# vadimkantorov/deepspeech.pytorch

Hardware: AMD Instinct MI355X
Metric: audio-seconds/sec training, DS2 5x BiGRU-800 bs32, at 1/2/4/8 MI355X (higher is better)
Workload: dtype f32

## Files before the change

### deepspeech.pytorch_amd/csrc/gru.hip

```cpp
#include "rnn_common.h"

#include <algorithm>

namespace ds2 {

constexpr int KC_FWD = 1024;
constexpr int KC_BWD = 2400;
constexpr int kTraceS0 = 100, kTraceSteps = 16;

template <int KSW>
__global__ __launch_bounds__(GT) void gru_fwd_step_kernel(
    int s, int T, int N, int H, int D, int UB, int BT, const float* __restrict__ xproj,
    const float* __restrict__ wp, const float* __restrict__ b_f, const float* __restrict__ b_r,
    const int* __restrict__ lens, float* __restrict__ h_all, float* __restrict__ gates) {
  constexpr int PITCH = KC_FWD + 2;
  __shared__ __attribute__((aligned(16))) float hs[GB * PITCH];
  int ub, d, bt;
  if (!map_work(UB * D, BT, UB, ub, d, bt)) return;
  const int n0 = bt * GB;
  const int lane = threadIdx.x & 63;
  const int wave = __builtin_amdgcn_readfirstlane(threadIdx.x >> 6);
  const int t = d == 0 ? s : T - 1 - s;
  const int tp = d == 0 ? t - 1 : t + 1;
  const int KS = (H + 3) / 4;
  const int per = (KS + GW - 1) / GW;
  const int a_ks = wave * per;
  const int b_ks = min(KS, a_ks + per);

  f32x4 acc[3];
#pragma unroll
  for (int g = 0; g < 3; ++g) acc[g] = f32x4{0.f, 0.f, 0.f, 0.f};

  if (s > 0) {
    float w[3][KSW];
    const float* wpd = wp + ((int64_t)d * UB + ub) * KS * 3 * 64 + lane;
#pragma unroll
    for (int i = 0; i < KSW; ++i) {
      const int ks = a_ks + i;
#pragma unroll
      for (int g = 0; g < 3; ++g) w[g][i] = ks < b_ks ? wpd[((int64_t)ks * 3 + g) * 64] : 0.f;
    }
    const float* hprev = h_all + ((int64_t)tp * N * D + d) * H;
    stage_rows(hprev, (int64_t)D * H, N, n0, 0, H, hs, PITCH);
    __syncthreads();
    const float* hrow = hs + (lane & 15) * PITCH + (lane >> 4);
#pragma unroll
    for (int i = 0; i < KSW; ++i) {
      const int ks = a_ks + i;
      if (ks < b_ks) {
        const int k = 4 * ks;
        const float a = (k + (lane >> 4) < H) ? hrow[k] : 0.f;
        acc[0] = __builtin_amdgcn_mfma_f32_16x16x4f32(a, w[0][i], acc[0], 0, 0, 0);
        acc[1] = __builtin_amdgcn_mfma_f32_16x16x4f32(a, w[1][i], acc[1], 0, 0, 0);
        acc[2] = __builtin_amdgcn_mfma_f32_16x16x4f32(a, w[2][i], acc[2], 0, 0, 0);
      }
    }
    __syncthreads();
  }
  float* red = hs;
  constexpr int RP = 3 * GU + 1;
#pragma unroll
  for (int g = 0; g < 3; ++g)
#pragma unroll
    for (int r = 0; r < 4; ++r)
      red[(wave * GB + (lane >> 4) * 4 + r) * RP + g * GU + (lane & 15)] = acc[g][r];
  __syncthreads();
  if (threadIdx.x >= GB * GU) return;

  const int m = threadIdx.x >> 4;
  const int u = threadIdx.x & 15;
  const int n = n0 + m;
  const int j = ub * GU + u;
  if (n >= N || j >= H) return;
  float gh[3];
#pragma unroll
  for (int g = 0; g < 3; ++g) {
    float v = 0.f;
#pragma unroll
    for (int w8 = 0; w8 < GW; ++w8) v += red[(w8 * GB + m) * RP + g * GU + u];
    gh[g] = v;
  }
  const float* bh = d == 0 ? b_f : b_r;
  const float ghr = gh[0] + bh[j];
  const float ghz = gh[1] + bh[H + j];
  float ghn = gh[2] + bh[2 * H + j];
  const int64_t row = ((int64_t)t * N + n) * D + d;
  const bool active = t < lens[n];
  float hout = 0.f, r = 0.f, z = 0.f, nn = 0.f;
  if (active) {
    const float* xp = xproj + row * 3 * H;
    const float hp = s > 0 ? h_all[(((int64_t)tp * N + n) * D + d) * H + j] : 0.f;
    r = sigmoidf_(ghr + xp[j]);
    z = sigmoidf_(ghz + xp[H + j]);
    nn = tanhf(xp[2 * H + j] + r * ghn);
    hout = (hp - nn) * z + nn;
  } else {
    ghn = 0.f;
  }
  h_all[row * H + j] = hout;
  if (gates != nullptr) {
    float* gp = gates + row * 4 * H;
    gp[j] = r;
    gp[H + j] = z;
    gp[2 * H + j] = nn;
    gp[3 * H + j] = ghn;
  }
}

template <int KSW>
__global__ __launch_bounds__(GT) void gru_bwd_step_kernel(
    int s, int T, int N, int H, int D, int UB, int BT, const float* __restrict__ dy, int dyd,
    const float* __restrict__ wpt, const float* __restrict__ h_all,
    const float* __restrict__ gates, const int* __restrict__ lens, float* __restrict__ dgx,
    float* __restrict__ dgh, float* __restrict__ dhs) {
  constexpr int PITCH = KC_BWD + 2;
  __shared__ __attribute__((aligned(16))) float hs[GB * PITCH];
  int ub, d, bt;
  if (!map_work(UB * D, BT, UB, ub, d, bt)) return;
  const int n0 = bt * GB;
  const int lane = threadIdx.x & 63;
  const int wave = __builtin_amdgcn_readfirstlane(threadIdx.x >> 6);
  const int t = d == 0 ? T - 1 - s : s;
  const int tq = d == 0 ? t + 1 : t - 1;
  const int H3 = 3 * H;
  const int KS = (H3 + 3) / 4;

  f32x4 acc0 = f32x4{0.f, 0.f, 0.f, 0.f};
  f32x4 acc1 = f32x4{0.f, 0.f, 0.f, 0.f};
  if (s > 0) {
    const float* dghq = dgh + ((int64_t)tq * N * D + d) * H3;
    const float* wpd = wpt + ((int64_t)d * UB + ub) * KS * 64 + lane;
    for (int kc0 = 0; kc0 < H3; kc0 += KC_BWD) {
      const int kc1 = min(H3, kc0 + KC_BWD);
      const int ks0 = kc0 / 4;
      const int ks1 = (kc1 + 3) / 4;
      const int per = (ks1 - ks0 + GW - 1) / GW;
      const int a_ks = ks0 + wave * per;
      const int b_ks = min(ks1, a_ks + per);
      float w[KSW];
#pragma unroll
      for (int i = 0; i < KSW; ++i) {
        const int ks = a_ks + i;
        w[i] = ks < b_ks ? wpd[(int64_t)ks * 64] : 0.f;
      }
      if (kc0 > 0) __syncthreads();
      stage_rows(dghq, (int64_t)D * H3, N, n0, kc0, kc1, hs, PITCH);
      __syncthreads();
      const float* hrow = hs + (lane & 15) * PITCH + (lane >> 4) - kc0;
#pragma unroll
      for (int i = 0; i < KSW; i += 2) {
        const int ks = a_ks + i;
        if (ks < b_ks) {
          const int k = 4 * ks;
          const float a0 = (k + (lane >> 4) < kc1) ? hrow[k] : 0.f;
          acc0 = __builtin_amdgcn_mfma_f32_16x16x4f32(a0, w[i], acc0, 0, 0, 0);
        }
        if (i + 1 < KSW && ks + 1 < b_ks) {
          const int k = 4 * (ks + 1);
          const float a1 = (k + (lane >> 4) < kc1) ? hrow[k] : 0.f;
          acc1 = __builtin_amdgcn_mfma_f32_16x16x4f32(a1, w[i + 1], acc1, 0, 0, 0);
        }
      }
    }
    __syncthreads();
  }
  float* red = hs;
  constexpr int RP = GU + 1;
#pragma unroll
  for (int r = 0; r < 4; ++r)
    red[(wave * GB + (lane >> 4) * 4 + r) * RP + (lane & 15)] = acc0[r] + acc1[r];
  __syncthreads();
  if (threadIdx.x >= GB * GU) return;

  const int m = threadIdx.x >> 4;
  const int u = threadIdx.x & 15;
  const int n = n0 + m;
  const int j = ub * GU + u;
  if (n >= N || j >= H) return;
  const int len = lens[n];
  const int64_t row = ((int64_t)t * N + n) * D + d;
  float* dhcur = dhs + ((int64_t)(s & 1) * N * D + (int64_t)n * D + d) * H;
  const float* dhprv = dhs + ((int64_t)((s + 1) & 1) * N * D + (int64_t)n * D + d) * H;
  float dh = 0.f;
  if (t < len) {
    float carry = 0.f;
    if (s > 0) {
      float rec = 0.f;
#pragma unroll
      for (int w8 = 0; w8 < GW; ++w8) rec += red[(w8 * GB + m) * RP + u];
      const float zq = gates[(((int64_t)tq * N + n) * D + d) * 4 * H + H + j];
      carry = dhprv[j] * zq + rec;
    }
    dh = dy[(((int64_t)t * N + n) * dyd + (dyd > 1 ? d : 0)) * H + j] + carry;
  }
  float dar = 0.f, daz = 0.f, dan = 0.f, dghn = 0.f;
  if (t < len) {
    const float* gp = gates + row * 4 * H;
    const float r = gp[j], z = gp[H + j], nn = gp[2 * H + j], ghn = gp[3 * H + j];
    float hp = 0.f;
    const int tp = d == 0 ? t - 1 : t + 1;
    if (tp >= 0 && tp < T) hp = h_all[(((int64_t)tp * N + n) * D + d) * H + j];
    dan = dh * (1.f - z) * (1.f - nn * nn);
    daz = dh * (hp - nn) * z * (1.f - z);
    dar = dan * ghn * r * (1.f - r);
    dghn = dan * r;
  }
  float* gx = dgx + row * H3;
  float* gh = dgh + row * H3;
  gx[j] = dar;
  gx[H + j] = daz;
  gx[2 * H + j] = dan;
  gh[j] = dar;
  gh[H + j] = daz;
  gh[2 * H + j] = dghn;
  dhcur[j] = dh;
}

template <int KSW>
__global__ __launch_bounds__(GT) void gru_fwd_persist_kernel(
    int T, int N, int H, int D, int UB, int BT, const float* __restrict__ xproj,
    const float* __restrict__ wp, const float* __restrict__ b_f, const float* __restrict__ b_r,
    const int* __restrict__ lens, float* __restrict__ h_all, float* __restrict__ gates,
    unsigned* __restrict__ counters, unsigned* __restrict__ err,
    unsigned long long* __restrict__ stamps, int trace) {
  constexpr int PITCH = KC_FWD + 4;
  __shared__ __attribute__((aligned(16))) float hs[GB * PITCH];
  __shared__ int flag;
  int ub, d, bt;
  if (!map_work(UB * D, BT, UB, ub, d, bt)) return;
  const int n0 = bt * GB;
  const int lane = threadIdx.x & 63;
  const int wave = __builtin_amdgcn_readfirstlane(threadIdx.x >> 6);
  const int KS = (H + 3) / 4;
  const int a_ks = wave * KSW;
  const int b_ks = min(KS, a_ks + KSW);
  unsigned* gflags = counters + (D * BT + 1) + (d * BT + bt) * UB;
  const __amdgpu_buffer_rsrc_t h_rs = __builtin_amdgcn_make_buffer_rsrc(
      h_all, (short)0, T * N * D * H * 4, 0x00020000);
  const bool stamping = stamps != nullptr && !trace && blockIdx.x == 0 && threadIdx.x == 0;
  const bool tracing = stamps != nullptr && trace && threadIdx.x == 0;
  auto trace_at = [&](int s, int p) {
    if (tracing && s >= kTraceS0 && s < kTraceS0 + kTraceSteps)
      stamps[((int64_t)(s - kTraceS0) * gridDim.x + blockIdx.x) * 5 + p] =
          __builtin_amdgcn_s_memrealtime();
  };
  unsigned long long acc_t[6] = {0, 0, 0, 0, 0, 0};
  unsigned long long t0 = 0, t1 = 0;

  float w[3][KSW];
  {
    const float* wpd = wp + ((int64_t)d * UB + ub) * KS * 3 * 64 + lane;
#pragma unroll
    for (int i = 0; i < KSW; ++i) {
      const int ks = a_ks + i;
#pragma unroll
      for (int g = 0; g < 3; ++g) w[g][i] = ks < b_ks ? wpd[((int64_t)ks * 3 + g) * 64] : 0.f;
    }
  }
  const float* bh = d == 0 ? b_f : b_r;
  const int m = threadIdx.x >> 4;
  const int u = threadIdx.x & 15;
  const int n = n0 + m;
  const int j = ub * GU + u;
  const bool owner = threadIdx.x < GB * GU && n < N && j < H;
  float bias_r = 0.f, bias_z = 0.f, bias_n = 0.f;
  int len = 0;
  if (owner) {
    bias_r = bh[j];
    bias_z = bh[H + j];
    bias_n = bh[2 * H + j];
    len = lens[n];
  }
  settle(bias_r);
  settle(bias_z);
  settle(bias_n);
  settle(len);
  constexpr int RP = 3 * GU + 1;
  __shared__ float red[GW * GB * RP];
  float g_r = 0.f, g_z = 0.f, g_n = 0.f, g_hn = 0.f;
  int64_t g_row = -1;
  for (int s = 0; s < T; ++s) {
    const int t = d == 0 ? s : T - 1 - s;
    const int tp = d == 0 ? t - 1 : t + 1;
    const int64_t row = ((int64_t)t * N + n) * D + d;
    float xr = 0.f, xz = 0.f, xn = 0.f;
    if (owner && t < len) {
      const float* xp = xproj + row * 3 * H;
      xr = xp[j];
      xz = xp[H + j];
      xn = xp[2 * H + j];
    }
    f32x4 acc[3];
#pragma unroll
    for (int g = 0; g < 3; ++g) acc[g] = f32x4{0.f, 0.f, 0.f, 0.f};
    float hp = 0.f;
    if (stamping) t0 = stamp_now();
    trace_at(s, 0);
    if (s > 0) {
      if (!flags_wait(gflags, UB, (unsigned)s, err, &flag)) {
        poison_rest(h_all, s, T, d != 0, N, D, n, d, H, j, H, 1, owner);
        return;
      }
      trace_at(s, 1);
      if (stamping) { t1 = stamp_now(); acc_t[0] += t1 - t0; t0 = t1; }
      const float* hprev = h_all + ((int64_t)tp * N * D + d) * H;
// ... 377 lines not shown
      const float* hrow = hs + (lane & 15) * PITCH + (lane >> 4) + 4 * a_ks;
#pragma unroll
      for (int i = 0; i < KSW; i += 2) {
        acc0 = __builtin_amdgcn_mfma_f32_16x16x4f32(hrow[4 * i], w[i], acc0, 0, 0, 0);
        if (i + 1 < KSW)
          acc1 = __builtin_amdgcn_mfma_f32_16x16x4f32(hrow[4 * i + 4], w[i + 1], acc1, 0, 0, 0);
      }
      __syncthreads();
    }
#pragma unroll
    for (int r = 0; r < 4; ++r)
      red[(wave * GB + (lane >> 4) * 4 + r) * RP + (lane & 15)] = acc0[r] + acc1[r];
    __syncthreads();
    trace_at(s, 3);
    if (owner) {
      float dh = 0.f;
      float dar = 0.f, daz = 0.f, dan = 0.f, dghn = 0.f, zc = 0.f;
      if (t < len) {
        float carry = 0.f;
        if (s > 0) {
          float rec = 0.f;
#pragma unroll
          for (int w8 = 0; w8 < GW; ++w8) rec += red[(w8 * GB + m) * RP + u];
          carry = dh_prev * z_prev + rec;
        }
        dh = dyv + carry;
        zc = g_z;
        dan = dh * (1.f - zc) * (1.f - g_n * g_n);
        daz = dh * (hp - g_n) * zc * (1.f - zc);
        dar = dan * g_hn * g_r * (1.f - g_r);
        dghn = dan * g_r;
      }
      const int go = static_cast<int>((row * H3 + j) * 4);
      __builtin_amdgcn_raw_buffer_store_b32(__builtin_bit_cast(unsigned, dar), g_rs, go, 0, kSc1);
      __builtin_amdgcn_raw_buffer_store_b32(__builtin_bit_cast(unsigned, daz), g_rs, go + 4 * H, 0,
                                            kSc1);
      __builtin_amdgcn_raw_buffer_store_b32(__builtin_bit_cast(unsigned, dghn), g_rs, go + 8 * H,
                                            0, kSc1);
      dh_prev = dh;
      z_prev = zc;
      px_dar = dar; px_daz = daz; px_dan = dan; px_row = row;
    }
    flags_arrive(gflags + ub, (unsigned)s + 1);
    trace_at(s, 4);
    if (owner) {
      float* gx = dgx + px_row * H3;
      gx[j] = px_dar;
      gx[H + j] = px_daz;
      gx[2 * H + j] = px_dan;
    }
  }
}

template <int NBW>
__global__ __launch_bounds__(GT) __attribute__((amdgpu_waves_per_eu(2, 2))) void gru_bwd_dop_kernel(
    int T, int N, int H, int D, int UB, int BT, const float* __restrict__ dy, int dyd,
    const float* __restrict__ w_f, const float* __restrict__ w_r,
    const float* __restrict__ h_all, const float* __restrict__ gates,
    const int* __restrict__ lens, float* __restrict__ dgx, float* __restrict__ dgh,
    float* __restrict__ gx, unsigned* __restrict__ counters, unsigned* __restrict__ err,
    unsigned long long* __restrict__ stamps, double* __restrict__ dbp) {
  constexpr int RP = GU + 1;
  __shared__ __attribute__((aligned(8))) float red[GW * GB * RP];
  __shared__ __attribute__((aligned(16))) float tile[3 * GB * GU];
  __shared__ int flag;
  int ub, d, bt;
  if (!map_work(UB * D, BT, UB, ub, d, bt)) return;
  const int n0 = bt * GB;
  const int lane = threadIdx.x & 63;
  const int wave = __builtin_amdgcn_readfirstlane(threadIdx.x >> 6);
  const int H3 = 3 * H;
  const int NB3 = 3 * UB;
  int b0, nb;
  simd_split(NB3, wave, b0, nb);
  const unsigned* gflags = counters + (D * BT + 1) + (d * BT + bt) * UB;
  unsigned* myflag = counters + (D * BT + 1) + (d * BT + bt) * UB + ub;
  const int slot_floats = D * BT * NB3 * 256;
  const __amdgpu_buffer_rsrc_t x_rs =
      __builtin_amdgcn_make_buffer_rsrc(gx, (short)0, 2 * slot_floats * 4, 0x00020000);
  const int grp_off = (d * BT + bt) * NB3 * 256;
  const bool tracing = stamps != nullptr && threadIdx.x == 0;
  auto trace_at = [&](int s, int p) {
    if (tracing && s >= kTraceS0 && s < kTraceS0 + kTraceSteps)
      stamps[((int64_t)(s - kTraceS0) * gridDim.x + blockIdx.x) * 5 + p] =
          __builtin_amdgcn_s_memrealtime();
  };

  f32x4 w[NBW];
  {
    const float* W = d == 0 ? w_f : w_r;
    const float* wc = W + (int64_t)(16 * b0 + 4 * (lane >> 4)) * H + ub * GU + (lane & 15);
#pragma unroll
    for (int i = 0; i < NBW; ++i)
#pragma unroll
      for (int c = 0; c < 4; ++c) w[i][c] = i < nb ? wc[(int64_t)(16 * i + c) * H] : 0.f;
#pragma unroll
    for (int i = 0; i < NBW; ++i) settle(w[i]);
  }
  const int m = threadIdx.x >> 4;
  const int u = threadIdx.x & 15;
  const int n = n0 + m;
  const int j = ub * GU + u;
  const bool owner = threadIdx.x < GB * GU && n < N;
  int len = owner ? lens[n] : 0;
  settle(len);
  const int tpos = ((u >> 2) * GB + m) * 4 + (u & 3);
  float dh_prev = 0.f, z_prev = 0.f;
  float px_dar = 0.f, px_daz = 0.f, px_dan = 0.f, px_dghn = 0.f;
  int64_t px_row = -1;
  double sb_r = 0.0, sb_z = 0.0, sb_n = 0.0, sb_hn = 0.0;
  for (int s = 0; s < T; ++s) {
    const int t = d == 0 ? T - 1 - s : s;
    f32x4 acc0 = f32x4{0.f, 0.f, 0.f, 0.f};
    f32x4 acc1 = f32x4{0.f, 0.f, 0.f, 0.f};
    trace_at(s, 0);
    float dyv = 0.f, g_r = 0.f, g_z = 0.f, g_n = 0.f, g_hn = 0.f, hp = 0.f;
    const int64_t row = ((int64_t)t * N + n) * D + d;
    if (owner && t < len) {
      dyv = dy[(((int64_t)t * N + n) * dyd + (dyd > 1 ? d : 0)) * H + j];
      const float* gp = gates + row * 4 * H;
      g_r = gp[j];
      g_z = gp[H + j];
      g_n = gp[2 * H + j];
      g_hn = gp[3 * H + j];
      const int tp = d == 0 ? t - 1 : t + 1;
      if (tp >= 0 && tp < T) hp = h_all[(((int64_t)tp * N + n) * D + d) * H + j];
    }
    if (s > 0) {
      if (!flags_wait(gflags, UB, (unsigned)s, err, &flag)) {
        poison_rest(dgx, s, T, d == 0, N, D, n, d, H, j, H3, 3, owner);
        return;
      }
      trace_at(s, 1);
      const int base = (((s - 1) & 1) * slot_floats + grp_off + b0 * 256 + lane * 4) * 4;
      f32x4 gv[NBW];
#pragma unroll
      for (int i = 0; i < NBW; ++i) {
        const int off = i < nb ? base + i * 1024 : 0x7ffffff0;
        gv[i] = __builtin_bit_cast(f32x4, __builtin_amdgcn_raw_buffer_load_b128(x_rs, off, 0, kSc1));
      }
      asm volatile("" ::: "memory");
      __builtin_amdgcn_sched_barrier(0);
#pragma unroll
      for (int i = 0; i < NBW; ++i) {
        acc0 = __builtin_amdgcn_mfma_f32_16x16x4f32(gv[i][0], w[i][0], acc0, 0, 0, 0);
        acc1 = __builtin_amdgcn_mfma_f32_16x16x4f32(gv[i][1], w[i][1], acc1, 0, 0, 0);
        acc0 = __builtin_amdgcn_mfma_f32_16x16x4f32(gv[i][2], w[i][2], acc0, 0, 0, 0);
        acc1 = __builtin_amdgcn_mfma_f32_16x16x4f32(gv[i][3], w[i][3], acc1, 0, 0, 0);
      }
      trace_at(s, 2);
    }
#pragma unroll
    for (int r = 0; r < 4; ++r)
      red[(wave * GB + (lane >> 4) * 4 + r) * RP + (lane & 15)] = acc0[r] + acc1[r];
    settle(dyv);
    settle(g_r);
    settle(g_z);
    settle(g_n);
    settle(g_hn);
    settle(hp);
    __syncthreads();
    trace_at(s, 3);
    if (threadIdx.x < GB * GU) {
      float dar = 0.f, daz = 0.f, dan = 0.f, dghn = 0.f;
      if (owner) {
        float dh = 0.f, zc = 0.f;
        if (t < len) {
          float carry = 0.f;
          if (s > 0) {
            float rec = 0.f;
#pragma unroll
            for (int w8 = 0; w8 < GW; ++w8) rec += red[(w8 * GB + m) * RP + u];
            carry = dh_prev * z_prev + rec;
          }
          dh = dyv + carry;
          zc = g_z;
          dan = dh * (1.f - zc) * (1.f - g_n * g_n);
          daz = dh * (hp - g_n) * zc * (1.f - zc);
          dar = dan * g_hn * g_r * (1.f - g_r);
          dghn = dan * g_r;
        }
        dh_prev = dh;
        z_prev = zc;
        px_dar = dar; px_daz = daz; px_dan = dan; px_dghn = dghn; px_row = row;
        sb_r += dar; sb_z += daz; sb_n += dan; sb_hn += dghn;
      }
      tile[tpos] = dar;
      tile[GB * GU + tpos] = daz;
      tile[2 * GB * GU + tpos] = dghn;
    }
    __syncthreads();
    if (wave == 0) {
      const int toff = (grp_off + ub * 256 + lane * 4) * 4;
      const int so = (s & 1) * slot_floats * 4 + toff;
#pragma unroll
      for (int g = 0; g < 3; ++g) {
        const u32x4 v = *reinterpret_cast<const u32x4*>(tile + g * GB * GU + lane * 4);
        __builtin_amdgcn_raw_buffer_store_b128(v, x_rs, so + g * UB * 1024, 0, kSc1);
      }
      asm volatile("s_waitcnt vmcnt(0)" ::: "memory");
      if (lane == 0)
        __hip_atomic_store(myflag, (unsigned)s + 1, __ATOMIC_RELAXED, __HIP_MEMORY_SCOPE_AGENT);
    }
    trace_at(s, 4);
    if (owner) {
      float* gxr = dgx + px_row * H3;
      gxr[j] = px_dar;
      gxr[H + j] = px_daz;
      gxr[2 * H + j] = px_dan;
      float* ghr = dgh + px_row * H3;
      ghr[j] = px_dar;
      ghr[H + j] = px_daz;
      ghr[2 * H + j] = px_dghn;
    }
  }
  if (dbp == nullptr) return;
  double* rd = reinterpret_cast<double*>(red);
  __syncthreads();
  if (threadIdx.x < GB * GU) {
    const bool mine = owner;
    rd[(0 * GB + m) * GU + u] = mine ? sb_r : 0.0;
    rd[(1 * GB + m) * GU + u] = mine ? sb_z : 0.0;
    rd[(2 * GB + m) * GU + u] = mine ? sb_n : 0.0;
    rd[(3 * GB + m) * GU + u] = mine ? sb_hn : 0.0;
  }
  __syncthreads();
  if (threadIdx.x < 4 * GU) {
    const int g = threadIdx.x / GU, uu = threadIdx.x - (threadIdx.x / GU) * GU;
    double acc = 0.0;
#pragma unroll
    for (int mm = 0; mm < GB; ++mm) acc += rd[(g * GB + mm) * GU + uu];
    dbp[(((int64_t)bt * D + d) * 4 + g) * H + ub * GU + uu] = acc;
  }
}

__global__ void gru_db_cols_kernel(const float* __restrict__ dgx, const float* __restrict__ dgh,
                                   int rows, int D, int H, double* __restrict__ dbp) {
  const int c = blockIdx.x;
  const int d = c / (4 * H), k = c - d * 4 * H;
  const int g = k / H, j = k - g * H;
  const float* src = g < 3 ? dgx + d * 3 * H + g * H + j : dgh + d * 3 * H + 2 * H + j;
  const int64_t stride = (int64_t)D * 3 * H;
  double acc = 0.0;
  for (int r = threadIdx.x; r < rows; r += blockDim.x) acc += src[r * stride];
  __shared__ double sh[256];
  sh[threadIdx.x] = acc;
  __syncthreads();
  for (int w = 128; w > 0; w >>= 1) {
    if ((int)threadIdx.x < w) sh[threadIdx.x] += sh[threadIdx.x + w];
    __syncthreads();
  }
  if (threadIdx.x == 0) dbp[c] = sh[0];
}

__global__ void gru_db_final_kernel(const double* __restrict__ dbp, int BT, int D, int H,
                                    float* __restrict__ dbi_f, float* __restrict__ dbh_f,
                                    float* __restrict__ dbi_r, float* __restrict__ dbh_r) {
  const int total = D * 4 * H;
  for (int i = blockIdx.x * blockDim.x + threadIdx.x; i < total; i += gridDim.x * blockDim.x) {
    const int d = i / (4 * H), k = i - d * 4 * H;
    double acc = 0.0;
    for (int b = 0; b < BT; ++b) acc += dbp[(int64_t)b * total + i];
    const float v = static_cast<float>(acc);
    float* dbi = d == 0 ? dbi_f : dbi_r;
    float* dbh = d == 0 ? dbh_f : dbh_r;
    if (k < 3 * H) dbi[k] = v;
    if (k < 2 * H) dbh[k] = v;
    if (k >= 3 * H) dbh[k - H] = v;
  }
}

}

namespace ds2 {
bool launch_gru_fwd_x6(int t_max, int n, int h, int num_dirs, const float* xproj,
                       const float* w_hh_f, const float* w_hh_r, const float* b_hh_f,
                       const float* b_hh_r, const int* lens, float* h_all, float* gates,
                       float* ring, unsigned* ctrs, unsigned* err, unsigned long long* stamps,
                       size_t lds_pad, hipStream_t st);
bool launch_gru_bwd_x6(int t_max, int n, int h, int num_dirs, const float* dy, int dy_dirs,
                       const float* w_hh_f, const float* w_hh_r, const float* h_all,
                       const float* gates, const int* lens, float* dgates_x, float* dgates_h,
                       float* ring, unsigned* ctrs, unsigned* err, unsigned long long* stamps,
                       double* dbp, size_t lds_pad, hipStream_t st, unsigned* camax,
                       bool* camax_done);
int gru_bwd_x6_grid(int n, int h, int num_dirs);
bool launch_rnn_fwd_h3(int t_max, int n, int h, int num_dirs, const float* xproj,
                       const float* w_hh_f, const float* w_hh_r, const float* b_hh_f,
                       const float* b_hh_r, const int* lens, float* h_all, float* ring,
                       unsigned* ctrs, unsigned* err, unsigned long long* stamps, size_t lds_pad,
                       hipStream_t st);
bool launch_rnn_bwd_h3(int t_max, int n, int h, int num_dirs, const float* dy, int dy_dirs,
                       const float* w_hh_f, const float* w_hh_r, const float* h_all,
                       const int* lens, float* dgates, float* ring, unsigned* ctrs, unsigned* err,
                       unsigned long long* stamps, size_t lds_pad, hipStream_t st,
                       unsigned* camax);
int rnn_h3_grid(int n, int h, int num_dirs);
int gru_xl_groups(int n, int h, int num_dirs);
int gru_xl_active(int n, int h, int num_dirs);
size_t gru_xl_ctr_words();
bool launch_gru_fwd_xl(int t_max, int n, int h, int num_dirs, const float* xproj,
                       const float* w_hh_f, const float* w_hh_r, const float* b_hh_f,
                       const float* b_hh_r, const int* lens, float* h_all, float* gates,
                       float* ring, unsigned* xl, unsigned* err, unsigned long long* stamps,
                       size_t lds_pad, hipStream_t st);
bool launch_gru_bwd_xl(int t_max, int n, int h, int num_dirs, const float* dy, int dy_dirs,
                       const float* w_hh_f, const float* w_hh_r, const float* h_all,
                       const float* gates, const int* lens, float* dgates_x, float* dgates_h,
                       float* ring, unsigned* xl, unsigned* err, unsigned long long* stamps,
                       double* dbp, size_t lds_pad, hipStream_t st, unsigned* camax);
}

using namespace ds2;

extern "C" {

static inline int stamp_mode() {
  const char* e = getenv("DS2_GRU_STAMPS");
  return e == nullptr ? 0 : (e[0] == '1' ? 1 : (e[0] == '2' ? 2 : 0));
}
constexpr unsigned kDopPadLds = 80 * 1024;
static const void* bwd_dop_fn(int need) {
#define DS2_BDOP(K) \
  if (need <= K) return reinterpret_cast<const void*>(gru_bwd_dop_kernel<K>);
  DS2_BDOP(1) DS2_BDOP(2) DS2_BDOP(3) DS2_BDOP(4) DS2_BDOP(6) DS2_BDOP(8) DS2_BDOP(10)
  DS2_BDOP(13) DS2_BDOP(16) DS2_BDOP(19) DS2_BDOP(22) DS2_BDOP(24)
#undef DS2_BDOP
  return nullptr;
}
static inline size_t ctr_words(int n, int num_dirs) {
  const int groups = num_dirs * ((n + GB - 1) / GB);
  const size_t a = (size_t)groups * 128, b = gru_xl_ctr_words();
  return (size_t)groups + 1 + (a > b ? a : b);
}
static inline size_t counter_bytes(int n, int num_dirs) {
  const size_t trace = stamp_mode() == 2 ? (size_t)kTraceSteps * 1024 * 5 : 16;
  return align256(ctr_words(n, num_dirs) * sizeof(unsigned)) + trace * sizeof(unsigned long long);
}
static inline unsigned long long* stamp_slots(unsigned* ctrs, int n, int num_dirs) {
  if (stamp_mode() == 0) return nullptr;
  return reinterpret_cast<unsigned long long*>(reinterpret_cast<char*>(ctrs) +
                                               align256(ctr_words(n, num_dirs) * sizeof(unsigned)));
}

static inline size_t ring_bytes(int n, int h, int num_dirs, int tiles) {
  const size_t UB = (h + GU - 1) / GU, BT = (n + GB - 1) / GB;
  const size_t tile_floats = tiles == 3 ? 384 : 256;
  const size_t slots = tiles == 3 ? 4 : 2 * kRingSlots;
  return align256(slots * (size_t)num_dirs * BT * UB * tiles * tile_floats * sizeof(float));
}
static inline hipError_t ring_reset(float* ring, int n, int h, int num_dirs, hipStream_t st) {
  return hipMemsetAsync(ring, 0xFF, ring_bytes(n, h, num_dirs, 1), st);
}

size_t ds2_gru_cache_floats(int t_max, int n, int h, int num_dirs) {
  if (t_max <= 0 || n <= 0 || h <= 0 || num_dirs <= 0) return 0;
  return (size_t)t_max * n * num_dirs * 4 * h;
}

size_t ds2_gru_fwd_workspace_size(int n, int h, int num_dirs) {
  const int64_t UB = (h + GU - 1) / GU;
  const int64_t KS = (h + 3) / 4;
  return align256((size_t)(num_dirs * UB * KS * 3 * 64) * sizeof(float)) +
         align256(counter_bytes(n, num_dirs)) + ring_bytes(n, h, num_dirs, 1) + 256;
}

#define DS2_FWD_CASE(K)                                                                    \
  case K:                                                                                  \
    hipLaunchKernelGGL(gru_fwd_step_kernel<K>, dim3(grid), dim3(GT), 0, st, s, t_max, n, h, \
                       num_dirs, UB, BT, xproj, wp, b_hh_f, b_hh_r, lens, h_all, gates);    \
    break;

static int pick_ksw(int per) {
  const int opts[] = {8, 16, 32, 48, 64, 80, 96};
  for (int k : opts)
    if (per <= k) return k;
  return -1;
}

ds2_status_t ds2_gru_fwd(int t_max, int n, int h, int num_dirs, const float* xproj,
                         const float* w_hh_f, const float* w_hh_r, const float* b_hh_f,
                         const float* b_hh_r, const int* lens, float* h_all, float* gates,
                         unsigned* err_out, void* ws, size_t ws_bytes, ds2_stream_t stream) {
  if (t_max < 0 || n < 0 || h < 1 || (num_dirs != 1 && num_dirs != 2)) return DS2_INVALID_VALUE;
  if (h > KC_FWD) return DS2_UNSUPPORTED_SHAPE;
  if (t_max == 0 || n == 0) return DS2_OK;
  if (ws == nullptr || ws_bytes < ds2_gru_fwd_workspace_size(n, h, num_dirs))
    return DS2_WORKSPACE_TOO_SMALL;
  if (num_dirs == 1) {
    w_hh_r = w_hh_f;
    b_hh_r = b_hh_f;
  }
  hipStream_t st = as_stream(stream);
  apply_spin_limit_env();
  apply_rnn_tune_env();
  const int UB = (h + GU - 1) / GU;
  const int KS = (h + 3) / 4;
  const int BT = (n + GB - 1) / GB;
  const int ksw = pick_ksw((KS + GW - 1) / GW);
  if (ksw < 0) return DS2_UNSUPPORTED_SHAPE;
  float* wp = static_cast<float*>(ws);
  const int grid = mapped_grid(UB * num_dirs, BT);
  const bool persistent = persistent_enabled() && grid <= num_cus() &&
                          (int64_t)t_max * n * num_dirs * h * 4 < (1ll << 31);
  unsigned* ctrs = reinterpret_cast<unsigned*>(
      static_cast<char*>(ws) + align256((size_t)num_dirs * UB * KS * 3 * 64 * sizeof(float)));
  unsigned* err = ctrs + num_dirs * BT;
  if (persistent && (h % GU) == 0 && UB <= 8 * GW) {
    if (hipMemsetAsync(ctrs, 0, counter_bytes(n, num_dirs), st) != hipSuccess)
      return launch_status("ds2_gru counters");
    int T_ = t_max, N_ = n, H_ = h, D_ = num_dirs, UB_ = UB, BT_ = BT;
    unsigned long long* stamps = stamp_mode() == 2 ? stamp_slots(ctrs, n, num_dirs) : nullptr;
    float* ring = reinterpret_cast<float*>(reinterpret_cast<char*>(ctrs) +
                                           align256(counter_bytes(n, num_dirs)));
    void* args[] = {&T_, &N_, &H_, &D_, &UB_, &BT_, &xproj, &w_hh_f, &w_hh_r, &b_hh_f,
                    &b_hh_r, &lens, &h_all, &gates, &ring, &ctrs, &err, &stamps};
    if (ring_reset(ring, n, h, num_dirs, st) != hipSuccess) return launch_status("ds2_gru ring");
    if (launch_gru_fwd_xl(t_max, n, h, num_dirs, xproj, w_hh_f, w_hh_r, b_hh_f, b_hh_r, lens,
                          h_all, gates, ring, err + 1, err, stamps, kDopPadLds, st)) {
      fold_err(err, err_out, st);
      return launch_status("ds2_gru_fwd");
    }
    (void)hipGetLastError();
    if (launch_gru_fwd_x6(t_max, n, h, num_dirs, xproj, w_hh_f, w_hh_r, b_hh_f, b_hh_r, lens,
                          h_all, gates, ring, ctrs, err, stamps, kDopPadLds, st)) {
      fold_err(err, err_out, st);
      return launch_status("ds2_gru_fwd");
    }
    (void)hipGetLastError();
    const void* fn = nullptr;
#define DS2_FDOP(K) \
  case K: fn = reinterpret_cast<const void*>(gru_fwd_dop_kernel<K>); break;
    switch ((UB + GW - 1) / GW) {
      DS2_FDOP(1) DS2_FDOP(2) DS2_FDOP(3) DS2_FDOP(4) DS2_FDOP(5) DS2_FDOP(6) DS2_FDOP(7)
      DS2_FDOP(8)
      default: break;
    }
#undef DS2_FDOP
    if (fn != nullptr &&
        rnn_launch(fn, dim3(grid), dim3(GT), args, kDopPadLds, st) == hipSuccess) {
      fold_err(err, err_out, st);
      return launch_status("ds2_gru_fwd");
    }
    (void)hipGetLastError();
  }
  hipLaunchKernelGGL(pack_fwd_kernel<3>, dim3(grid_cap((int64_t)num_dirs * UB * KS * 192)),
                     dim3(256), 0, st, w_hh_f, w_hh_r, h, num_dirs, UB, KS, wp);
  if (persistent && (h % 4) == 0) {
    if (hipMemsetAsync(ctrs, 0, counter_bytes(n, num_dirs), st) != hipSuccess)
      return launch_status("ds2_gru counters");
    int T_ = t_max, N_ = n, H_ = h, D_ = num_dirs, UB_ = UB, BT_ = BT;
    unsigned long long* stamps = stamp_slots(ctrs, n, num_dirs);
    int trace_ = stamp_mode() == 2 ? 1 : 0;
    void* args[] = {&T_, &N_, &H_, &D_, &UB_, &BT_, &xproj, &wp, &b_hh_f, &b_hh_r, &lens,
                    &h_all, &gates, &ctrs, &err, &stamps, &trace_};
    const void* fn = nullptr;
    const int kp = persist_ksw((KS + GW - 1) / GW, KC_FWD);
    switch (kp) {
      case 8: fn = reinterpret_cast<const void*>(gru_fwd_persist_kernel<8>); break;
      case 16: fn = reinterpret_cast<const void*>(gru_fwd_persist_kernel<16>); break;
      case 25: fn = reinterpret_cast<const void*>(gru_fwd_persist_kernel<25>); break;
      case 32: fn = reinterpret_cast<const void*>(gru_fwd_persist_kernel<32>); break;
      default: break;
    }
    if (fn != nullptr &&
        rnn_launch(fn, dim3(grid), dim3(GT), args, 0, st) == hipSuccess) {
      fold_err(err, err_out, st);
      return launch_status("ds2_gru_fwd");
    }
    (void)hipGetLastError();
  }
  for (int s = 0; s < t_max; ++s) {
    switch (ksw) {
      DS2_FWD_CASE(8) DS2_FWD_CASE(16) DS2_FWD_CASE(32) DS2_FWD_CASE(48) DS2_FWD_CASE(64)
      DS2_FWD_CASE(80) DS2_FWD_CASE(96)
    }
  }
  return launch_status("ds2_gru_fwd");
}

static size_t gru_bwd_ws_base(int n, int h, int num_dirs) {
  const int64_t UB = (h + GU - 1) / GU;
  const int64_t KS = (3 * h + 3) / 4;
  return align256((size_t)(num_dirs * UB * KS * 64) * sizeof(float)) +
         align256((size_t)2 * n * num_dirs * h * sizeof(float)) +
         align256(counter_bytes(n, num_dirs)) + ring_bytes(n, h, num_dirs, 3) + 512;
}

static size_t gru_db_bytes(int n, int h, int num_dirs) {
  return align256((size_t)((n + 7) / 8) * num_dirs * 4 * h * sizeof(double));
}

size_t ds2_gru_bwd_workspace_size(int n, int h, int num_dirs) {
  return gru_bwd_ws_base(n, h, num_dirs) + gru_db_bytes(n, h, num_dirs);
}

#define DS2_BWD_CASE(K)                                                                     \
  case K:                                                                                   \
    hipLaunchKernelGGL(gru_bwd_step_kernel<K>, dim3(grid), dim3(GT), 0, st, s, t_max, n, h,  \
                       num_dirs, UB, BT, dy, dy_dirs, wpt, h_all, gates, lens, dgates_x,     \
                       dgates_h, dhs);                                                       \
    break;

int ds2_gru_bwd_grid(int n, int h, int num_dirs) {
  if (n < 1 || h < 1 || (num_dirs != 1 && num_dirs != 2)) return 0;
  const int UB = (h + GU - 1) / GU, BT = (n + GB - 1) / GB;
  const int grid = mapped_grid(UB * num_dirs, BT);
  if (!persistent_enabled() || grid > num_cus()) return 0;
  if ((h % GU) == 0 && UB <= 8 * GW) {
    const int g = gru_bwd_x6_grid(n, h, num_dirs);
    const int x = gru_xl_active(n, h, num_dirs);
    const int m = g > x ? g : x;
    return m > grid ? m : grid;
  }
  return (3 * h <= KC_BWD && (h % 4) == 0) ? grid : 0;
}

ds2_status_t ds2_gru_bwd(int t_max, int n, int h, int num_dirs, const float* dy, int dy_dirs,
                         const float* w_hh_f, const float* w_hh_r, const float* h_all,
                         const float* gates, const int* lens, float* dgates_x, float* dgates_h,
                         unsigned* err_out, void* ws, size_t ws_bytes, ds2_stream_t stream) {
  return ds2_gru_bwd_bias(t_max, n, h, num_dirs, dy, dy_dirs, w_hh_f, w_hh_r, h_all, gates, lens,
                          dgates_x, dgates_h, nullptr, nullptr, nullptr, nullptr, err_out, ws,
                          ws_bytes, stream);
}

static ds2_status_t gru_bwd_run(int t_max, int n, int h, int num_dirs, const float* dy, int dy_dirs,
                                const float* w_hh_f, const float* w_hh_r, const float* h_all,
                                const float* gates, const int* lens, float* dgates_x,
                                float* dgates_h, unsigned* err_out, void* ws, hipStream_t st,
                                double* dbp, bool& summed, unsigned* camax, bool& camax_done,
                                int& db_tiles);

static ds2_status_t gru_bwd_bias_impl(int t_max, int n, int h, int num_dirs, const float* dy,
                                      int dy_dirs, const float* w_hh_f, const float* w_hh_r,
                                      const float* h_all, const float* gates, const int* lens,
                                      float* dgates_x, float* dgates_h, float* db_ih_f,
                                      float* db_hh_f, float* db_ih_r, float* db_hh_r,
                                      unsigned* err_out, void* ws, size_t ws_bytes,
                                      unsigned* camax, ds2_stream_t stream);

ds2_status_t ds2_gru_bwd_bias(int t_max, int n, int h, int num_dirs, const float* dy, int dy_dirs,
                              const float* w_hh_f, const float* w_hh_r, const float* h_all,
                              const float* gates, const int* lens, float* dgates_x,
                              float* dgates_h, float* db_ih_f, float* db_hh_f, float* db_ih_r,
                              float* db_hh_r, unsigned* err_out, void* ws, size_t ws_bytes,
                              ds2_stream_t stream) {
  return gru_bwd_bias_impl(t_max, n, h, num_dirs, dy, dy_dirs, w_hh_f, w_hh_r, h_all, gates, lens,
                           dgates_x, dgates_h, db_ih_f, db_hh_f, db_ih_r, db_hh_r, err_out, ws,
                           ws_bytes, nullptr, stream);
}

ds2_status_t ds2_gru_bwd_bias_amax(int t_max, int n, int h, int num_dirs, const float* dy,
                                   int dy_dirs, const float* w_hh_f, const float* w_hh_r,
                                   const float* h_all, const float* gates, const int* lens,
                                   float* dgates_x, float* dgates_h, float* db_ih_f,
                                   float* db_hh_f, float* db_ih_r, float* db_hh_r,
                                   unsigned* col_amax, unsigned* err_out, void* ws,
                                   size_t ws_bytes, ds2_stream_t stream) {
  if (col_amax == nullptr) return DS2_INVALID_VALUE;
  return gru_bwd_bias_impl(t_max, n, h, num_dirs, dy, dy_dirs, w_hh_f, w_hh_r, h_all, gates, lens,
                           dgates_x, dgates_h, db_ih_f, db_hh_f, db_ih_r, db_hh_r, err_out, ws,
                           ws_bytes, col_amax, stream);
}

static ds2_status_t gru_bwd_bias_impl(int t_max, int n, int h, int num_dirs, const float* dy,
                                      int dy_dirs, const float* w_hh_f, const float* w_hh_r,
                                      const float* h_all, const float* gates, const int* lens,
                                      float* dgates_x, float* dgates_h, float* db_ih_f,
                                      float* db_hh_f, float* db_ih_r, float* db_hh_r,
                                      unsigned* err_out, void* ws, size_t ws_bytes,
                                      unsigned* camax, ds2_stream_t stream) {
  if (t_max < 0 || n < 0 || h < 1 || (num_dirs != 1 && num_dirs != 2)) return DS2_INVALID_VALUE;
  if (gates == nullptr) return DS2_INVALID_VALUE;
  if (dy_dirs != 1 && dy_dirs != num_dirs) return DS2_INVALID_VALUE;
  const bool want_db = db_ih_f != nullptr;
  if (want_db && (db_hh_f == nullptr || (num_dirs == 2 && (db_ih_r == nullptr || db_hh_r == nullptr))))
    return DS2_INVALID_VALUE;
  if (ws == nullptr || ws_bytes < ds2_gru_bwd_workspace_size(n, h, num_dirs))
    return DS2_WORKSPACE_TOO_SMALL;
  hipStream_t st = as_stream(stream);
  double* dbp = reinterpret_cast<double*>(static_cast<char*>(ws) + gru_bwd_ws_base(n, h, num_dirs));
  const size_t camax_bytes = (size_t)2 * num_dirs * 3 * h * sizeof(unsigned);
  if (camax != nullptr && hipMemsetAsync(camax, 0, camax_bytes, st) != hipSuccess)
    return launch_status("ds2_gru_bwd_bias_amax");
  if (t_max == 0 || n == 0) {
    if (!want_db) return DS2_OK;
    if (hipMemsetAsync(dbp, 0, gru_db_bytes(n > 0 ? n : 1, h, num_dirs), st) != hipSuccess)
      return launch_status("ds2_gru_bwd_bias");
    hipLaunchKernelGGL(gru_db_final_kernel, dim3(cdiv(num_dirs * 4 * h, 256)), dim3(256), 0, st,
                       dbp, 1, num_dirs, h, db_ih_f, db_hh_f, db_ih_r, db_hh_r);
    return launch_status("ds2_gru_bwd_bias");
  }
  bool summed = false, camax_done = false;
  int db_tiles = (n + GB - 1) / GB;
  const ds2_status_t rc = gru_bwd_run(t_max, n, h, num_dirs, dy, dy_dirs, w_hh_f, w_hh_r, h_all,
                                      gates, lens, dgates_x, dgates_h, err_out, ws, st,
                                      want_db ? dbp : nullptr, summed, camax, camax_done, db_tiles);
  if (rc != DS2_OK) return rc;
  if (camax != nullptr && !camax_done) {
    const ds2_status_t ra = ds2_amax(dgates_x, t_max * n, num_dirs * 3 * h, num_dirs * 3 * h,
                                     nullptr, camax, stream);
    const ds2_status_t rb = ra != DS2_OK ? ra
        : ds2_amax(dgates_h, t_max * n, num_dirs * 3 * h, num_dirs * 3 * h, nullptr,
                   camax + num_dirs * 3 * h, stream);
    if (rb != DS2_OK) return rb;
  }
  if (!want_db) return DS2_OK;
  int bt = db_tiles;
  if (!summed) {
    hipLaunchKernelGGL(gru_db_cols_kernel, dim3(num_dirs * 4 * h), dim3(256), 0, st, dgates_x,
                       dgates_h, t_max * n, num_dirs, h, dbp);
    bt = 1;
  }
  hipLaunchKernelGGL(gru_db_final_kernel, dim3(cdiv(num_dirs * 4 * h, 256)), dim3(256), 0, st, dbp,
                     bt, num_dirs, h, db_ih_f, db_hh_f, db_ih_r, db_hh_r);
  return launch_status("ds2_gru_bwd_bias");
}

static ds2_status_t gru_bwd_run(int t_max, int n, int h, int num_dirs, const float* dy, int dy_dirs,
                                const float* w_hh_f, const float* w_hh_r, const float* h_all,
                                const float* gates, const int* lens, float* dgates_x,
                                float* dgates_h, unsigned* err_out, void* ws, hipStream_t st,
                                double* dbp, bool& summed, unsigned* camax, bool& camax_done,
                                int& db_tiles) {
  if (num_dirs == 1) w_hh_r = w_hh_f;
  apply_spin_limit_env();
  apply_rnn_tune_env();
  const int UB = (h + GU - 1) / GU;
  const int KS = (3 * h + 3) / 4;
  const int BT = (n + GB - 1) / GB;
  const int chunk_ks = (std::min(3 * h, KC_BWD) + 3) / 4;
  const int ksw = pick_ksw((chunk_ks + GW - 1) / GW + 1);
  if (ksw < 0) return DS2_UNSUPPORTED_SHAPE;
  float* wpt = static_cast<float*>(ws);
  size_t off = align256((size_t)num_dirs * UB * KS * 64 * sizeof(float));
  float* dhs = reinterpret_cast<float*>(static_cast<char*>(ws) + off);
  const int grid = mapped_grid(UB * num_dirs, BT);
  const bool persistent = persistent_enabled() && grid <= num_cus() &&
                          (int64_t)t_max * n * num_dirs * 3 * h * 4 < (1ll << 31);
  unsigned* ctrs = reinterpret_cast<unsigned*>(
      reinterpret_cast<char*>(dhs) + align256((size_t)2 * n * num_dirs * h * sizeof(float)));
  unsigned* err = ctrs + num_dirs * BT;
  if (persistent && (h % GU) == 0 && UB <= 8 * GW) {
    if (hipMemsetAsync(ctrs, 0, counter_bytes(n, num_dirs), st) != hipSuccess)
      return launch_status("ds2_gru counters");
    int T_ = t_max, N_ = n, H_ = h, D_ = num_dirs, UB_ = UB, BT_ = BT, DYD_ = dy_dirs;
    unsigned long long* stamps = stamp_mode() == 2 ? stamp_slots(ctrs, n, num_dirs) : nullptr;
    float* ring = reinterpret_cast<float*>(reinterpret_cast<char*>(ctrs) +
                                           align256(counter_bytes(n, num_dirs)));
    void* args[] = {&T_, &N_, &H_, &D_, &UB_, &BT_, &dy, &DYD_, &w_hh_f, &w_hh_r, &h_all,
                    &gates, &lens, &dgates_x, &dgates_h, &ring, &ctrs, &err, &stamps, &dbp};
    if (launch_gru_bwd_xl(t_max, n, h, num_dirs, dy, dy_dirs, w_hh_f, w_hh_r, h_all, gates,
                          lens, dgates_x, dgates_h, ring, err + 1, err, stamps, dbp, kDopPadLds,
                          st, camax)) {
      fold_err(err, err_out, st);
      summed = dbp != nullptr;
      camax_done = camax != nullptr;
      db_tiles = (n + 7) / 8;
      return launch_status("ds2_gru_bwd");
    }
    (void)hipGetLastError();
    if (launch_gru_bwd_x6(t_max, n, h, num_dirs, dy, dy_dirs, w_hh_f, w_hh_r, h_all, gates,
                          lens, dgates_x, dgates_h, ring, ctrs, err, stamps, dbp, kDopPadLds, st,
                          camax, &camax_done)) {
      fold_err(err, err_out, st);
      summed = dbp != nullptr;
      return launch_status("ds2_gru_bwd");
    }
    (void)hipGetLastError();
    const void* fn = bwd_dop_fn((3 * UB + GW - 1) / GW);
    if (fn != nullptr &&
        rnn_launch(fn, dim3(grid), dim3(GT), args, kDopPadLds, st) == hipSuccess) {
      fold_err(err, err_out, st);
      summed = dbp != nullptr;
      return launch_status("ds2_gru_bwd");
    }
    (void)hipGetLastError();
  }
  hipLaunchKernelGGL(pack_bwd_kernel<3>, dim3(grid_cap((int64_t)num_dirs * UB * KS * 64)),
                     dim3(256), 0, st, w_hh_f, w_hh_r, h, num_dirs, UB, KS, wpt);
  if (persistent && 3 * h <= KC_BWD && (h % 4) == 0) {
    if (hipMemsetAsync(ctrs, 0, counter_bytes(n, num_dirs), st) != hipSuccess)
      return launch_status("ds2_gru counters");
    int T_ = t_max, N_ = n, H_ = h, D_ = num_dirs, UB_ = UB, BT_ = BT, DYD_ = dy_dirs;
    unsigned long long* stamps = stamp_mode() == 2 ? stamp_slots(ctrs, n, num_dirs) : nullptr;
    void* args[] = {&T_, &N_, &H_, &D_, &UB_, &BT_, &dy, &DYD_, &wpt, &h_all, &gates, &lens,
                    &dgates_x, &dgates_h, &ctrs, &err, &stamps};
    const void* fn = nullptr;
    const int kp = persist_ksw((KS + GW - 1) / GW, KC_BWD);
    switch (kp) {
      case 8: fn = reinterpret_cast<const void*>(gru_bwd_persist_kernel<8>); break;
      case 16: fn = reinterpret_cast<const void*>(gru_bwd_persist_kernel<16>); break;
      case 25: fn = reinterpret_cast<const void*>(gru_bwd_persist_kernel<25>); break;
      case 32: fn = reinterpret_cast<const void*>(gru_bwd_persist_kernel<32>); break;
      case 48: fn = reinterpret_cast<const void*>(gru_bwd_persist_kernel<48>); break;
      case 64: fn = reinterpret_cast<const void*>(gru_bwd_persist_kernel<64>); break;
      case 75: fn = reinterpret_cast<const void*>(gru_bwd_persist_kernel<75>); break;
      default: break;
    }
    if (fn != nullptr &&
        rnn_launch(fn, dim3(grid), dim3(GT), args, 0, st) == hipSuccess) {
      fold_err(err, err_out, st);
      return launch_status("ds2_gru_bwd");
    }
    (void)hipGetLastError();
  }
  for (int s = 0; s < t_max; ++s) {
    switch (ksw) {
      DS2_BWD_CASE(8) DS2_BWD_CASE(16) DS2_BWD_CASE(32) DS2_BWD_CASE(48) DS2_BWD_CASE(64)
      DS2_BWD_CASE(80) DS2_BWD_CASE(96)
    }
  }
  return launch_status("ds2_gru_bwd");
}

static bool rnn_persistent_ok(int t_max, int n, int h, int num_dirs) {
  const int g = rnn_h3_grid(n, h, num_dirs);
  return persistent_enabled() && g > 0 && g <= num_cus() &&
         (int64_t)t_max * n * num_dirs * h * 4 < (1ll << 31);
}

size_t ds2_rnn_fwd_workspace_size(int n, int h, int num_dirs) {
  if (n < 1 || h < 1 || num_dirs < 1) return 256;
  return align256(counter_bytes(n, num_dirs)) + ring_bytes(n, h, num_dirs, 1) + 256;
}

ds2_status_t ds2_rnn_fwd_ws(int t_max, int n, int h, int num_dirs, const float* xproj,
                            const float* w_hh_f, const float* w_hh_r, const float* b_hh_f,
                            const float* b_hh_r, const int* lens, float* h_all, unsigned* err_out,
                            void* ws, size_t ws_bytes, ds2_stream_t stream) {
  if (t_max < 0 || n < 0 || h < 1 || (num_dirs != 1 && num_dirs != 2)) return DS2_INVALID_VALUE;
  if (t_max == 0 || n == 0) return DS2_OK;
  if (xproj == nullptr || w_hh_f == nullptr || b_hh_f == nullptr || lens == nullptr ||
      h_all == nullptr || (num_dirs == 2 && (w_hh_r == nullptr || b_hh_r == nullptr)))
    return DS2_INVALID_VALUE;
  if (ws == nullptr || ws_bytes < ds2_rnn_fwd_workspace_size(n, h, num_dirs))
    return DS2_WORKSPACE_TOO_SMALL;
  if (num_dirs == 1) {
    w_hh_r = w_hh_f;
    b_hh_r = b_hh_f;
  }
  hipStream_t st = as_stream(stream);
  if (rnn_persistent_ok(t_max, n, h, num_dirs)) {
    unsigned* ctrs = static_cast<unsigned*>(ws);
    unsigned* err = ctrs + num_dirs * ((n + GB - 1) / GB);
    float* ring = reinterpret_cast<float*>(static_cast<char*>(ws) + align256(counter_bytes(n, num_dirs)));
    if (hipMemsetAsync(ctrs, 0, counter_bytes(n, num_dirs), st) != hipSuccess)
      return launch_status("ds2_rnn counters");
    if (ring_reset(ring, n, h, num_dirs, st) != hipSuccess) return launch_status("ds2_rnn ring");
    unsigned long long* stamps = stamp_mode() == 2 ? stamp_slots(ctrs, n, num_dirs) : nullptr;
    if (launch_rnn_fwd_h3(t_max, n, h, num_dirs, xproj, w_hh_f, w_hh_r, b_hh_f, b_hh_r, lens,
                          h_all, ring, ctrs, err, stamps, kDopPadLds, st)) {
      fold_err(err, err_out, st);
      return launch_status("ds2_rnn_fwd");
    }
    (void)hipGetLastError();
  }
  return ds2_rnn_fwd(t_max, n, h, num_dirs, xproj, w_hh_f, w_hh_r, b_hh_f, b_hh_r, lens, h_all,
                     stream);
}

size_t ds2_rnn_bwd_workspace_size(int n, int h, int num_dirs) {
  if (n < 1 || h < 1 || num_dirs < 1) return 256;
  return align256(counter_bytes(n, num_dirs)) + ring_bytes(n, h, num_dirs, 3) + 256;
}

int ds2_rnn_bwd_grid(int n, int h, int num_dirs) {
  if (n < 1 || h < 1 || (num_dirs != 1 && num_dirs != 2)) return 0;
  const int g = rnn_h3_grid(n, h, num_dirs);
  return persistent_enabled() && g > 0 && g <= num_cus() ? g : 0;
}

ds2_status_t ds2_rnn_bwd_ws(int t_max, int n, int h, int num_dirs, const float* dy, int dy_dirs,
                            const float* w_hh_f, const float* w_hh_r, const float* h_all,
                            const int* lens, float* dgates, unsigned* col_amax, unsigned* err_out,
                            void* ws, size_t ws_bytes, ds2_stream_t stream) {
  if (t_max < 0 || n < 0 || h < 1 || (num_dirs != 1 && num_dirs != 2)) return DS2_INVALID_VALUE;
  if (dy_dirs != 1 && dy_dirs != num_dirs) return DS2_INVALID_VALUE;
  if (ws == nullptr || ws_bytes < ds2_rnn_bwd_workspace_size(n, h, num_dirs))
    return DS2_WORKSPACE_TOO_SMALL;
  hipStream_t st = as_stream(stream);
  if (col_amax != nullptr &&
      hipMemsetAsync(col_amax, 0, (size_t)num_dirs * h * sizeof(unsigned), st) != hipSuccess)
    return launch_status("ds2_rnn_bwd_ws");
  if (t_max == 0 || n == 0) return DS2_OK;
  if (dy == nullptr || w_hh_f == nullptr || h_all == nullptr || lens == nullptr ||
      dgates == nullptr || (num_dirs == 2 && w_hh_r == nullptr))
    return DS2_INVALID_VALUE;
  if (num_dirs == 1) w_hh_r = w_hh_f;
  if (rnn_persistent_ok(t_max, n, h, num_dirs)) {
    unsigned* ctrs = static_cast<unsigned*>(ws);
    unsigned* err = ctrs + num_dirs * ((n + GB - 1) / GB);
    float* ring = reinterpret_cast<float*>(static_cast<char*>(ws) + align256(counter_bytes(n, num_dirs)));
    if (hipMemsetAsync(ctrs, 0, counter_bytes(n, num_dirs), st) != hipSuccess)
      return launch_status("ds2_rnn counters");
    unsigned long long* stamps = stamp_mode() == 2 ? stamp_slots(ctrs, n, num_dirs) : nullptr;
    if (launch_rnn_bwd_h3(t_max, n, h, num_dirs, dy, dy_dirs, w_hh_f, w_hh_r, h_all, lens, dgates,
                          ring, ctrs, err, stamps, kDopPadLds, st, col_amax)) {
      fold_err(err, err_out, st);
      return launch_status("ds2_rnn_bwd");
    }
    (void)hipGetLastError();
  }
  const ds2_status_t rc = ds2_rnn_bwd(t_max, n, h, num_dirs, dy, dy_dirs, w_hh_f, w_hh_r, h_all,
                                      lens, dgates, stream);
  if (rc != DS2_OK || col_amax == nullptr) return rc;
  return ds2_amax(dgates, t_max * n, num_dirs * h, num_dirs * h, nullptr, col_amax, stream);
}

}
```

### deepspeech.pytorch_amd/csrc/gru_xl.hip

```cpp
#include "rnn_common.h"

namespace ds2 {

#ifndef DS2_XL_ABL
#define DS2_XL_ABL 0
#endif
constexpr bool kAblLoads = (DS2_XL_ABL & 1) != 0;
constexpr bool kAblStores = (DS2_XL_ABL & 2) != 0;
constexpr bool kAblWait = (DS2_XL_ABL & 4) != 0;
constexpr bool kAblFixT = (DS2_XL_ABL & 8) != 0;

constexpr int LB = 8;
constexpr int LU = 32;
constexpr int LW = 4;
constexpr int LT = LW * 64;
constexpr int LSLOTS = 4;
constexpr int LRB = 784;
constexpr int kXlTraceS0 = 100, kXlTraceSteps = 16;

__device__ __forceinline__ bool xl_map(int G, int UBX, int& g, int& ub) {
  g = blockIdx.x & 7;
  ub = blockIdx.x >> 3;
  return g < G && ub < UBX;
}

__device__ __forceinline__ bool xl_group_local(unsigned* xtab, int ub, int UBX, unsigned* err,
                                               int* lds_word, unsigned* mode, int force_global) {
  const unsigned mine = xcc_id() + 1u;
  if (threadIdx.x == 0) __hip_atomic_store(xtab + ub, mine, __ATOMIC_RELAXED, __HIP_MEMORY_SCOPE_AGENT);
  if ((threadIdx.x >> 6) == 0) {
    const int lane = threadIdx.x & 63;
    unsigned v = mine;
    bool ok = true;
    for (unsigned spins = 0;; ++spins) {
      v = lane < UBX ? __hip_atomic_load(xtab + lane, __ATOMIC_RELAXED, __HIP_MEMORY_SCOPE_AGENT)
                     : mine;
      if (__ballot(v == 0u) == 0ull) break;
      if (spins > g_spin_limit) {
        if (lane == 0) __hip_atomic_fetch_or(err, 1u, __ATOMIC_RELAXED, __HIP_MEMORY_SCOPE_AGENT);
        ok = false;
        break;
      }
      __builtin_amdgcn_s_sleep(1);
    }
    const bool loc = ok && __ballot(v != mine) == 0ull && force_global == 0;
    if (lane == 0) {
      *lds_word = loc ? 1 : 0;
      __hip_atomic_fetch_or(mode, loc ? 1u : 2u, __ATOMIC_RELAXED, __HIP_MEMORY_SCOPE_AGENT);
    }
  }
  __syncthreads();
  return *lds_word != 0;
}

__device__ __forceinline__ void xl_store(u32x4 v, __amdgpu_buffer_rsrc_t rs, int off, bool local) {
  if (local)
    __builtin_amdgcn_raw_buffer_store_b128(v, rs, off, 0, 0);
  else
    __builtin_amdgcn_raw_buffer_store_b128(v, rs, off, 0, kSc1);
}

__device__ __forceinline__ int xl_frag_hi(int m, int k) { return (((k >> 3) << 4) + m) * 8 + (k & 7); }

template <int NPW>
__global__ __launch_bounds__(LT) __attribute__((amdgpu_waves_per_eu(1, 1))) void gru_fwd_xl_kernel(
    int T, int N, int H, int D, int UBX, int BTX, const float* __restrict__ xproj,
    const float* __restrict__ w_f, const float* __restrict__ w_r, const float* __restrict__ b_f,
    const float* __restrict__ b_r, const int* __restrict__ lens, float* __restrict__ h_all,
    float* __restrict__ gates, float* __restrict__ ring, unsigned* __restrict__ xl,
    unsigned* __restrict__ err, unsigned long long* __restrict__ stamps, int force_global) {
  constexpr int NCT = 6;
  constexpr int RC = 3 * LU + 1;
  __shared__ float red[LW * 16 * RC];
  __shared__ __attribute__((aligned(16))) _Float16 stg[64 * 8];
  __shared__ float unsc[3 * LU];
  __shared__ __attribute__((aligned(16))) float pin[3 * 256];
  __shared__ __attribute__((aligned(16))) float pout[5 * 256];
  __shared__ int slen[LB];
  __shared__ int sh_local;
  __shared__ int failed;
  __shared__ u32x4 wx[LW * NCT * 2 * 64];
  const int G = D * BTX;
  int g, ub;
  if (!xl_map(G, UBX, g, ub)) return;
  const int d = g / BTX, bt = g - d * BTX;
  const int lane = threadIdx.x & 63;
  const int wave = __builtin_amdgcn_readfirstlane(threadIdx.x >> 6);
  const int p0 = wave * (UBX / LW) + min(wave, UBX % LW);
  const int np = UBX / LW + (wave < UBX % LW ? 1 : 0);
  if (threadIdx.x == 0) failed = 0;
  const bool local = xl_group_local(xl + g * 32, ub, UBX, err, &sh_local, xl + 512 + g, force_global);
  const int slot_floats = G * UBX * 256;
  const __amdgpu_buffer_rsrc_t x_rs =
      __builtin_amdgcn_make_buffer_rsrc(ring, (short)0, LSLOTS * slot_floats * 4, 0x00020000);
  const int grp_off = g * UBX * 256;
  const bool tracing = stamps != nullptr && lane == 0;
  auto trace_at = [&](int s, int p) __attribute__((always_inline)) {
    if (tracing && s >= kXlTraceS0 && s < kXlTraceS0 + kXlTraceSteps)
      stamps[(((int64_t)(s - kXlTraceS0) * gridDim.x + blockIdx.x) * LW + wave) * 6 + p] =
          __builtin_amdgcn_s_memrealtime();
  };

  Duo w[NPW][NCT];
  auto wfr = [&](int p, int ct) __attribute__((always_inline)) {
    if (p < NPW) return w[p < NPW ? p : 0][ct];
    Duo r;
    r.hi = __builtin_bit_cast(f16x8, wx[((wave * NCT + ct) * 2 + 0) * 64 + lane]);
    r.lo = __builtin_bit_cast(f16x8, wx[((wave * NCT + ct) * 2 + 1) * 64 + lane]);
    return r;
  };
  {
    const float* W = d == 0 ? w_f : w_r;
    const int q8 = 8 * (lane >> 4);
    auto frag = [&](int p, int ct, f32x4& a, f32x4& b) __attribute__((always_inline)) {
      const f32x4 z4 = f32x4{0.f, 0.f, 0.f, 0.f};
      if (p < np) {
        const float* r = W + (int64_t)((ct >> 1) * H + LU * ub + 16 * (ct & 1) + (lane & 15)) * H +
                         LU * (p0 + p) + q8;
        a = *reinterpret_cast<const f32x4*>(r);
        b = *reinterpret_cast<const f32x4*>(r + 4);
      } else {
        a = z4;
        b = z4;
      }
    };
    float mx[NCT];
#pragma unroll
    for (int ct = 0; ct < NCT; ++ct) mx[ct] = 0.f;
#pragma unroll
    for (int p = 0; p < NPW + 1; ++p)
#pragma unroll
      for (int ct = 0; ct < NCT; ++ct) {
        f32x4 a, b;
        frag(p, ct, a, b);
#pragma unroll
        for (int i = 0; i < 4; ++i) mx[ct] = fmaxf(mx[ct], fmaxf(fabsf(a[i]), fabsf(b[i])));
      }
#pragma unroll
    for (int ct = 0; ct < NCT; ++ct) {
      mx[ct] = fmaxf(mx[ct], __shfl_xor(mx[ct], 16));
      mx[ct] = fmaxf(mx[ct], __shfl_xor(mx[ct], 32));
      if (lane < 16) red[wave * 96 + ct * 16 + lane] = mx[ct];
    }
    __syncthreads();
    float sc[NCT];
#pragma unroll
    for (int ct = 0; ct < NCT; ++ct) {
      float m = 0.f;
#pragma unroll
      for (int w4 = 0; w4 < LW; ++w4) m = fmaxf(m, red[w4 * 96 + ct * 16 + (lane & 15)]);
      sc[ct] = __builtin_ldexpf(1.f, h3_row_exp(m));
    }
    if (threadIdx.x < 3 * LU) {
      float m = 0.f;
#pragma unroll
      for (int w4 = 0; w4 < LW; ++w4) m = fmaxf(m, red[w4 * 96 + threadIdx.x]);
      unsc[threadIdx.x] = __builtin_ldexpf(1.f, -(h3_row_exp(m) + 14));
    }
    __syncthreads();
    asm volatile("" ::: "memory");
#pragma unroll
    for (int p = 0; p < NPW + 1; ++p)
#pragma unroll
      for (int ct = 0; ct < NCT; ++ct) {
        f32x4 a, b;
        frag(p, ct, a, b);
        const Duo dd = split2h(a, b, sc[ct]);
        if (p < NPW) {
          w[p < NPW ? p : 0][ct] = dd;
        } else {
          wx[((wave * NCT + ct) * 2 + 0) * 64 + lane] = __builtin_bit_cast(u32x4, dd.hi);
          wx[((wave * NCT + ct) * 2 + 1) * 64 + lane] = __builtin_bit_cast(u32x4, dd.lo);
        }
      }
  }
  const float* bh = d == 0 ? b_f : b_r;
  const int m = threadIdx.x >> 5;
  const int u = threadIdx.x & 31;
  const int n = bt * LB + m;
  const int j = ub * LU + u;
  const bool owner = n < N;
  float bias_r = 0.f, bias_z = 0.f, bias_n = 0.f;
  if (owner) {
    bias_r = bh[j];
    bias_z = bh[H + j];
    bias_n = bh[2 * H + j];
  }
  if (threadIdx.x < LB) slen[threadIdx.x] = bt * LB + (int)threadIdx.x < N ? lens[bt * LB + threadIdx.x] : 0;
  __syncthreads();
  const int len = slen[m];
  const float us_r = unsc[u], us_z = unsc[LU + u], us_n = unsc[2 * LU + u];
  settle(bias_r);
  settle(bias_z);
  settle(bias_n);
  const int shi = xl_frag_hi(m, u), slo = shi + 64;
  const bool io = wave != 0;
  const int q = io ? (int)threadIdx.x - 64 : 0;
  const int qm = q / 24, qg = (q % 24) >> 3, q4 = (q & 7) * 4;
  const int qn = bt * LB + qm;
  const bool qv = io && qn < N;
  const int qlen = slen[qm];
  const float* xq = xproj + ((int64_t)qn * D + d) * 3 * H + qg * H + ub * LU + q4;
  const int64_t xstep = (int64_t)N * D * 3 * H;
  const f32x4 z4v = f32x4{0.f, 0.f, 0.f, 0.f};
  auto in_ok = [&](int st) __attribute__((always_inline)) {
    const int tt = d == 0 ? st : T - 1 - st;
    return !kAblLoads && qv && tt < qlen;
  };
  auto load_in = [&](int st) __attribute__((always_inline)) {
    const int tt = d == 0 ? st : T - 1 - st;
    return *reinterpret_cast<const f32x4*>(in_ok(st) ? xq + (kAblFixT ? 0 : tt) * xstep : xproj);
  };
  float* ob[2];
  int64_t ostr[2];
  int osrc[2];
  bool ov[2];
#pragma unroll
  for (int k = 0; k < 2; ++k) {
    const int idx = q + 192 * k;
    const int sm = (idx / 40) & 7, f = (idx % 40) >> 3, o4 = (idx & 7) * 4, sn = bt * LB + sm;
    ov[k] = io && idx < 320 && sn < N && (f == 0 || gates != nullptr);
    osrc[k] = f * 256 + sm * LU + o4;
    if (f == 0) {
      ob[k] = h_all + ((int64_t)sn * D + d) * H + ub * LU + o4;
      ostr[k] = (int64_t)N * D * H;
    } else {
      ob[k] = gates + ((int64_t)sn * D + d) * 4 * H + (f - 1) * H + ub * LU + o4;
      ostr[k] = (int64_t)N * D * 4 * H;
    }
  }
  auto store_out = [&](int st) __attribute__((always_inline)) {
    const int tt = d == 0 ? st : T - 1 - st;
#pragma unroll
    for (int k = 0; k < 2; ++k)
      if (ov[k])
        *reinterpret_cast<f32x4*>(ob[k] + tt * ostr[k]) = *reinterpret_cast<const f32x4*>(pout + osrc[k]);
  };
  f32x4 xin = io ? load_in(0) : z4v;
  float h_own = 0.f;
  for (int s = 0; s < T; ++s) {
    const int t = d == 0 ? s : T - 1 - s;
    f32x4 acc[NCT];
#pragma unroll
    for (int ct = 0; ct < NCT; ++ct) acc[ct] = f32x4{0.f, 0.f, 0.f, 0.f};
    trace_at(s, 0);
    if (io) *reinterpret_cast<f32x4*>(pin + qg * 256 + qm * LU + q4) = in_ok(s) ? xin : z4v;
    if (s > 0) {
      trace_at(s, 1);
      const int base = (((s - 1) % LSLOTS) * slot_floats + grp_off + p0 * 256 + lane * 4) * 4;
      sleep_units(g_rnn_tune[7]);
      u32x4 hv[NPW + 1];
#pragma unroll
      for (int p = 0; p < NPW + 1; ++p)
        hv[p] = __builtin_amdgcn_raw_buffer_load_b128(x_rs, p < np ? base + p * 1024 : 0x7ffffff0, 0, kSc1);
      asm volatile("" ::: "memory");
      __builtin_amdgcn_sched_barrier(0);
      bool bad = false;
#pragma unroll
      for (int p = 0; p < NPW + 1; ++p) {
        if (p < np && !bad) {
          for (unsigned spins = 0;
               !kAblWait && (!wave_ready(__builtin_bit_cast(f32x4, hv[p])) || g_spin_limit == 0);
               ++spins) {
            if (spins > g_spin_limit || g_spin_limit == 0) {
              if (lane == 0) __hip_atomic_fetch_or(err, 1u, __ATOMIC_RELAXED, __HIP_MEMORY_SCOPE_AGENT);
              failed = 1;
              bad = true;
              break;
            }
            sleep_units(g_rnn_tune[0]);
            asm volatile("" ::: "memory");
#pragma unroll
            for (int q = p; q < NPW + 1; ++q)
              if (q < np && (unsigned)(q - p) < g_rnn_tune[6])
                hv[q] = __builtin_amdgcn_raw_buffer_load_b128(x_rs, base + q * 1024, 0, kSc1);
          }
          const f16x8 a = __builtin_bit_cast(f16x8, hv[p]);
#pragma unroll
          for (int ct = 0; ct < NCT; ++ct) {
            const Duo wf = wfr(p, ct);
            acc[ct] = __builtin_amdgcn_mfma_f32_16x16x32_f16(a, wf.lo, acc[ct], 0, 0, 0);
            acc[ct] = __builtin_amdgcn_mfma_f32_16x16x32_f16(a, wf.hi, acc[ct], 0, 0, 0);
          }
        }
      }
      trace_at(s, 2);
    }
    if (io) {
      if (s + 1 < T) xin = load_in(s + 1);
      if (!kAblStores && s > 0) store_out(s - 1);
    }
    trace_at(s, 3);
#pragma unroll
    for (int ct = 0; ct < NCT; ++ct)
#pragma unroll
      for (int i = 0; i < 4; ++i)
        red[(wave * 16 + (lane >> 4) * 4 + i) * RC + ct * 16 + (lane & 15)] = acc[ct][i];
    __syncthreads();
    if (failed) {
      poison_rest(h_all, s, T, d != 0, N, D, n, d, H, j, H, 1, owner);
      return;
    }
    trace_at(s, 4);
    float gh[3];
#pragma unroll
    for (int gt = 0; gt < 3; ++gt) {
      float v = 0.f;
#pragma unroll
      for (int w4 = 0; w4 < LW; ++w4)
        v += red[(w4 * 16 + m) * RC + gt * LU + u] + red[(w4 * 16 + m + 8) * RC + gt * LU + u];
      gh[gt] = v;
    }
    const float xr = pin[m * LU + u], xz = pin[256 + m * LU + u], xn = pin[512 + m * LU + u];
    float hout = 0.f, r = 0.f, z = 0.f, nn = 0.f, ghn = 0.f;
    if (owner && t < len) {
      ghn = gh[2] * us_n + bias_n;
      r = sigmoid_fast(gh[0] * us_r + bias_r + xr);
      z = sigmoid_fast(gh[1] * us_z + bias_z + xz);
      nn = tanh_fast(xn + r * ghn);
      hout = (h_own - nn) * z + nn;
    }
    h_own = owner ? hout : 0.f;
    pout[m * LU + u] = hout;
    pout[256 + m * LU + u] = r;
    pout[512 + m * LU + u] = z;
    pout[768 + m * LU + u] = nn;
    pout[1024 + m * LU + u] = ghn;
    {
      const float v = hout * 16384.f;
      const _Float16 hi = (_Float16)v;
      stg[shi] = hi;
      stg[slo] = (_Float16)(v - (float)hi);
    }
    __syncthreads();
    if (wave == 0) {
      const int toff = (grp_off + ub * 256 + lane * 4) * 4;
      const u32x4 v = desentinel(*reinterpret_cast<const u32x4*>(stg + lane * 8));
      asm volatile("s_waitcnt vmcnt(0)" ::: "memory");
      xl_store(v, x_rs, (s % LSLOTS) * slot_floats * 4 + toff, local);
      xl_store(u32x4{kSentinel, kSentinel, kSentinel, kSentinel}, x_rs,
               ((s + 2) % LSLOTS) * slot_floats * 4 + toff, local);
    }
    trace_at(s, 5);
  }
  __syncthreads();
  if (io && !kAblStores) store_out(T - 1);
}

template <int NPW>
__global__ __launch_bounds__(LT) __attribute__((amdgpu_waves_per_eu(1, 1))) void gru_bwd_xl_kernel(
    int T, int N, int H, int D, int UBX, int BTX, const float* __restrict__ dy, int dyd,
    const float* __restrict__ w_f, const float* __restrict__ w_r,
    const float* __restrict__ h_all, const float* __restrict__ gates,
    const int* __restrict__ lens, float* __restrict__ dgx, float* __restrict__ dgh,
    float* __restrict__ ring, unsigned* __restrict__ xl, unsigned* __restrict__ err,
    unsigned long long* __restrict__ stamps, double* __restrict__ dbp,
    unsigned* __restrict__ camax, int force_global) {
  constexpr int RC = LU + 1;
  constexpr int LWP = 3;
  __shared__ __attribute__((aligned(8))) float red[LW * 16 * RC > 4 * LB * LU * 2 ? LW * 16 * RC : 4 * LB * LU * 2];
  __shared__ __attribute__((aligned(16))) _Float16 stg[3 * 64 * 8];
  __shared__ __attribute__((aligned(16))) float stsc[LB];
  __shared__ float colmx[LW * LU];
  __shared__ __attribute__((aligned(16))) float pin[6 * 256];
  __shared__ __attribute__((aligned(16))) float pout[4 * 256];
  __shared__ int slen[LB];
  __shared__ int sh_local;
  __shared__ int flag;
  __shared__ u32x4 wx[LW * 6 * 2 * 64];
  const int G = D * BTX;
  int g, ub;
  if (!xl_map(G, UBX, g, ub)) return;
  const int d = g / BTX, bt = g - d * BTX;
  const int lane = threadIdx.x & 63;
  const int wave = __builtin_amdgcn_readfirstlane(threadIdx.x >> 6);
  const int p0 = wave * (UBX / LW) + min(wave, UBX % LW);
  const int np = UBX / LW + (wave < UBX % LW ? 1 : 0);
  const int H3 = 3 * H;
  const int slot_floats = G * UBX * LRB;
  const __amdgpu_buffer_rsrc_t x_rs =
      __builtin_amdgcn_make_buffer_rsrc(ring, (short)0, 2 * slot_floats * 4, 0x00020000);
  const int grp_off = g * UBX * LRB;
  const bool local = xl_group_local(xl + g * 32, ub, UBX, err, &sh_local, xl + 512 + g, force_global);
  unsigned* flags = xl + 256 + g * 32;
  const __amdgpu_buffer_rsrc_t f_rs =
      __builtin_amdgcn_make_buffer_rsrc(xl + 256, (short)0, 8 * 32 * 4, 0x00020000);
  const bool tracing = stamps != nullptr && lane == 0;
  auto trace_at = [&](int s, int p) __attribute__((always_inline)) {
    if (tracing && s >= kXlTraceS0 && s < kXlTraceS0 + kXlTraceSteps)
      stamps[(((int64_t)(s - kXlTraceS0) * gridDim.x + blockIdx.x) * LW + wave) * 6 + p] =
          __builtin_amdgcn_s_memrealtime();
  };

  Duo w[NPW][3][2];
  auto wfr = [&](int p, int gt, int c) __attribute__((always_inline)) {
    if (p < NPW) return w[p < NPW ? p : 0][gt][c];
    Duo r;
    r.hi = __builtin_bit_cast(f16x8, wx[((wave * 6 + gt * 2 + c) * 2 + 0) * 64 + lane]);
    r.lo = __builtin_bit_cast(f16x8, wx[((wave * 6 + gt * 2 + c) * 2 + 1) * 64 + lane]);
    return r;
  };
  float unscale;
  {
    const float* W = d == 0 ? w_f : w_r;
    const int q8 = 8 * (lane >> 4);
    auto col = [&](int p, int gt, int c, f32x4& a, f32x4& b) __attribute__((always_inline)) {
      if (p < np) {
        const float* wc = W + (int64_t)(gt * H + LU * (p0 + p) + q8) * H + LU * ub + 16 * c + (lane & 15);
#pragma unroll
        for (int i = 0; i < 4; ++i) {
          a[i] = wc[(int64_t)i * H];
          b[i] = wc[(int64_t)(i + 4) * H];
        }
      } else {
        a = f32x4{0.f, 0.f, 0.f, 0.f};
        b = a;
      }
    };
    float mx[2] = {0.f, 0.f};
#pragma unroll
    for (int p = 0; p < NPW + 1; ++p)
#pragma unroll
      for (int gt = 0; gt < 3; ++gt)
#pragma unroll
        for (int c = 0; c < 2; ++c) {
          f32x4 a, b;
          col(p, gt, c, a, b);
#pragma unroll
          for (int i = 0; i < 4; ++i) mx[c] = fmaxf(mx[c], fmaxf(fabsf(a[i]), fabsf(b[i])));
        }
#pragma unroll
    for (int c = 0; c < 2; ++c) {
      mx[c] = fmaxf(mx[c], __shfl_xor(mx[c], 16));
      mx[c] = fmaxf(mx[c], __shfl_xor(mx[c], 32));
      if (lane < 16) colmx[wave * LU + 16 * c + lane] = mx[c];
    }
    __syncthreads();
    float sc[2];
#pragma unroll
    for (int c = 0; c < 2; ++c) {
      float m = 0.f;
#pragma unroll
      for (int w4 = 0; w4 < LW; ++w4) m = fmaxf(m, colmx[w4 * LU + 16 * c + (lane & 15)]);
      sc[c] = __builtin_ldexpf(1.f, h3_row_exp(m));
    }
    {
      float m = 0.f;
#pragma unroll
      for (int w4 = 0; w4 < LW; ++w4) m = fmaxf(m, colmx[w4 * LU + (threadIdx.x & 31)]);
      unscale = __builtin_ldexpf(1.f, -h3_row_exp(m));
    }
    asm volatile("" ::: "memory");
#pragma unroll
    for (int p = 0; p < NPW + 1; ++p)
#pragma unroll
      for (int gt = 0; gt < 3; ++gt)
#pragma unroll
        for (int c = 0; c < 2; ++c) {
          f32x4 a, b;
          col(p, gt, c, a, b);
          const Duo dd = split2h(a, b, sc[c]);
          if (p < NPW) {
            w[p < NPW ? p : 0][gt][c] = dd;
          } else {
            wx[((wave * 6 + gt * 2 + c) * 2 + 0) * 64 + lane] = __builtin_bit_cast(u32x4, dd.hi);
            wx[((wave * 6 + gt * 2 + c) * 2 + 1) * 64 + lane] = __builtin_bit_cast(u32x4, dd.lo);
          }
        }
  }
  const int m = threadIdx.x >> 5;
  const int u = threadIdx.x & 31;
  const int n = bt * LB + m;
  const int j = ub * LU + u;
  const bool owner = n < N;
  if (threadIdx.x < LB) slen[threadIdx.x] = bt * LB + (int)threadIdx.x < N ? lens[bt * LB + threadIdx.x] : 0;
  __syncthreads();
  const int len = slen[m];
  const int shi = xl_frag_hi(m, u), slo = shi + 64;
  const bool io = wave != 0;
  const int q = io ? (int)threadIdx.x - 64 : 0;
  const f32x4 z4v = f32x4{0.f, 0.f, 0.f, 0.f};
  const int ostr = N * D * H3;
  struct IoSlot {
    const float* in;
    float* out;
    int f, len, str, pin_at, pout_at;
  };
  auto make_slot = [&](int k) __attribute__((always_inline)) {
    const int idx = q + 192 * k;
    const int sm = idx / 48, f = (idx % 48) >> 3, o4 = (idx & 7) * 4, sn = bt * LB + sm;
    IoSlot r;
    r.f = f;
    r.len = io && sn < N ? slen[sm] : -1;
    if (f == 0) {
      r.in = dy + (sn * dyd + (dyd > 1 ? d : 0)) * H + ub * LU + o4;
      r.str = N * dyd * H;
    } else if (f < 5) {
      r.in = gates + (sn * D + d) * 4 * H + (f - 1) * H + ub * LU + o4;
      r.str = N * D * 4 * H;
    } else {
      r.in = h_all + (sn * D + d) * H + ub * LU + o4;
      r.str = N * D * H;
    }
    r.out = io && sn < N ? (f < 3 ? dgx : dgh) + (sn * D + d) * H3 + (f % 3) * H + ub * LU + o4
                         : nullptr;
    r.pin_at = f * 256 + sm * LU + o4;
    r.pout_at = (f < 3 ? f : (f == 5 ? 3 : f - 3)) * 256 + sm * LU + o4;
    return r;
  };
  const IoSlot sl0 = make_slot(0), sl1 = make_slot(1);
  auto in_ok = [&](int st, const IoSlot sl) __attribute__((always_inline)) {
    const int tt = d == 0 ? T - 1 - st : st;
    const int tr = sl.f == 5 ? (d == 0 ? tt - 1 : tt + 1) : tt;
    return !kAblLoads && tt < sl.len && tr >= 0 && tr < T;
  };
  auto load_in = [&](int st, const IoSlot sl) __attribute__((always_inline)) {
    const int tt = d == 0 ? T - 1 - st : st;
    const int tr = sl.f == 5 ? (d == 0 ? tt - 1 : tt + 1) : tt;
    return *reinterpret_cast<const f32x4*>(sl.in + (in_ok(st, sl) && !kAblFixT ? tr * sl.str : 0));
  };
  auto stage_in = [&](const f32x4 v, const IoSlot sl, int st) __attribute__((always_inline)) {
    *reinterpret_cast<f32x4*>(pin + sl.pin_at) = in_ok(st, sl) ? v : z4v;
  };
  auto store_one = [&](int tt, const IoSlot sl) __attribute__((always_inline)) {
    if (sl.out != nullptr)
      *reinterpret_cast<f32x4*>(sl.out + tt * ostr) = *reinterpret_cast<const f32x4*>(pout + sl.pout_at);
  };
  auto store_out = [&](int st) __attribute__((always_inline)) {
    const int tt = d == 0 ? T - 1 - st : st;
    store_one(tt, sl0);
    store_one(tt, sl1);
  };
  f32x4 xin0 = io ? load_in(0, sl0) : z4v, xin1 = io ? load_in(0, sl1) : z4v;
  float dh_prev = 0.f, z_prev = 0.f;
  double sb_r = 0.0, sb_z = 0.0, sb_n = 0.0, sb_hn = 0.0;
  float cm_r = 0.f, cm_z = 0.f, cm_n = 0.f, cm_hn = 0.f;
  const int rsel = ((lane >> 4) & 1) * 16;
  auto io_issue = [&](int st) __attribute__((always_inline)) {
    if (!io) return;
    if (st + 1 < T) {
      xin0 = load_in(st + 1, sl0);
      xin1 = load_in(st + 1, sl1);
    }
    if (!kAblStores && st > 0) store_out(st - 1);
  };
  for (int s = 0; s < T; ++s) {
    const int t = d == 0 ? T - 1 - s : s;
    f32x4 acc[2] = {f32x4{0.f, 0.f, 0.f, 0.f}, f32x4{0.f, 0.f, 0.f, 0.f}};
    trace_at(s, 0);
    if (io) {
      stage_in(xin0, sl0, s);
      stage_in(xin1, sl1, s);
    }
    if (s == 0) io_issue(0);
    if (s > 0) {
      if (!kAblWait && !flags_wait(flags, UBX, (unsigned)s, err, &flag)) {
        poison_rest(dgx, s, T, d == 0, N, D, n, d, H, j, H3, 3, owner);
        return;
      }
      trace_at(s, 1);
      const int rb = (((s - 1) & 1) * slot_floats + grp_off + p0 * LRB) * 4;
      u32x4 r0[NPW + 1], r1[NPW + 1], r2[NPW + 1];
      f32x4 rs[NPW + 1];
      auto load_rec = [&](int p) __attribute__((always_inline)) {
        const int base = p < np ? rb + p * LRB * 4 : 0x7ffff000;
        r0[p] = __builtin_amdgcn_raw_buffer_load_b128(x_rs, base + lane * 16, 0, kSc1);
        r1[p] = __builtin_amdgcn_raw_buffer_load_b128(x_rs, base + 1024 + lane * 16, 0, kSc1);
        r2[p] = __builtin_amdgcn_raw_buffer_load_b128(x_rs, base + 2048 + lane * 16, 0, kSc1);
        rs[p] = __builtin_bit_cast(
            f32x4, __builtin_amdgcn_raw_buffer_load_b128(x_rs, base + 3072 + rsel, 0, kSc1));
      };
#pragma unroll
      for (int p = 0; p < LWP && p < NPW + 1; ++p) load_rec(p);
      if (LWP >= NPW + 1) io_issue(s);
      asm volatile("" ::: "memory");
      __builtin_amdgcn_sched_barrier(0);
#pragma unroll
      for (int p = 0; p < NPW + 1; ++p) {
        if (p + LWP < NPW + 1) load_rec(p + LWP);
        if (p + LWP == NPW) io_issue(s);
        if (p < np) {
          const f16x8 ar = __builtin_bit_cast(f16x8, r0[p]);
          const f16x8 az = __builtin_bit_cast(f16x8, r1[p]);
          const f16x8 an = __builtin_bit_cast(f16x8, r2[p]);
#pragma unroll
          for (int c = 0; c < 2; ++c) {
            const f32x4 z4 = f32x4{0.f, 0.f, 0.f, 0.f};
            const Duo w0 = wfr(p, 0, c), w1 = wfr(p, 1, c), w2 = wfr(p, 2, c);
            f32x4 c1 = __builtin_amdgcn_mfma_f32_16x16x32_f16(ar, w0.hi, z4, 0, 0, 0);
            f32x4 c2 = __builtin_amdgcn_mfma_f32_16x16x32_f16(ar, w0.lo, z4, 0, 0, 0);
            c1 = __builtin_amdgcn_mfma_f32_16x16x32_f16(az, w1.hi, c1, 0, 0, 0);
            c2 = __builtin_amdgcn_mfma_f32_16x16x32_f16(az, w1.lo, c2, 0, 0, 0);
            c1 = __builtin_amdgcn_mfma_f32_16x16x32_f16(an, w2.hi, c1, 0, 0, 0);
            c2 = __builtin_amdgcn_mfma_f32_16x16x32_f16(an, w2.lo, c2, 0, 0, 0);
            acc[c] += (c1 + c2) * rs[p];
          }
        }
      }
      trace_at(s, 2);
    }
    trace_at(s, 3);
#pragma unroll
    for (int c = 0; c < 2; ++c)
#pragma unroll
      for (int i = 0; i < 4; ++i)
        red[(wave * 16 + (lane >> 4) * 4 + i) * RC + 16 * c + (lane & 15)] = acc[c][i];
    __syncthreads();
    const float dyv = pin[m * LU + u], g_r = pin[256 + m * LU + u], g_z = pin[512 + m * LU + u];
    const float g_n = pin[768 + m * LU + u], g_hn = pin[1024 + m * LU + u];
    const float hp = pin[1280 + m * LU + u];
    trace_at(s, 4);
    float dar = 0.f, daz = 0.f, dan = 0.f, dghn = 0.f;
    if (owner) {
      float dh = 0.f, zc = 0.f;
      if (t < len) {
        float carry = 0.f;
        if (s > 0) {
          float rec = 0.f;
#pragma unroll
          for (int w4 = 0; w4 < LW; ++w4)
            rec += red[(w4 * 16 + m) * RC + u] + red[(w4 * 16 + m + 8) * RC + u];
          carry = dh_prev * z_prev + rec * unscale;
        }
        dh = dyv + carry;
        zc = g_z;
        dan = dh * (1.f - zc) * (1.f - g_n * g_n);
        daz = dh * (hp - g_n) * zc * (1.f - zc);
        dar = dan * g_hn * g_r * (1.f - g_r);
        dghn = dan * g_r;
      }
      dh_prev = dh;
      z_prev = zc;
      sb_r += dar; sb_z += daz; sb_n += dan; sb_hn += dghn;
      cm_r = fmaxf(cm_r, fabsf(dar));
      cm_z = fmaxf(cm_z, fabsf(daz));
      cm_n = fmaxf(cm_n, fabsf(dan));
      cm_hn = fmaxf(cm_hn, fabsf(dghn));
    }
    pout[m * LU + u] = dar;
    pout[256 + m * LU + u] = daz;
    pout[512 + m * LU + u] = dan;
    pout[768 + m * LU + u] = dghn;
    {
      float mx = fmaxf(fmaxf(fabsf(dar), fabsf(daz)), fabsf(dghn));
#pragma unroll
      for (int o = 1; o < 32; o <<= 1) mx = fmaxf(mx, __shfl_xor(mx, o));
      const int e = h3_row_exp(mx);
      const float sc = __builtin_ldexpf(1.f, e);
      const float vr = dar * sc, vz = daz * sc, vn = dghn * sc;
      const _Float16 hr = (_Float16)vr, hz = (_Float16)vz, hn = (_Float16)vn;
      stg[shi] = hr;
      stg[slo] = (_Float16)(vr - (float)hr);
      stg[512 + shi] = hz;
      stg[512 + slo] = (_Float16)(vz - (float)hz);
      stg[1024 + shi] = hn;
      stg[1024 + slo] = (_Float16)(vn - (float)hn);
      if (u == 0) stsc[m] = __builtin_ldexpf(1.f, -e);
    }
    __syncthreads();
    if (wave == 0) {
      const int so = ((s & 1) * slot_floats + grp_off + ub * LRB) * 4;
#pragma unroll
      for (int k = 0; k < 3; ++k)
        xl_store(*reinterpret_cast<const u32x4*>(stg + k * 512 + lane * 8), x_rs,
                 so + k * 1024 + lane * 16, local);
      if (lane < 2) xl_store(*reinterpret_cast<const u32x4*>(stsc + lane * 4), x_rs, so + 3072 + lane * 16, local);
      asm volatile("s_waitcnt vmcnt(0)" ::: "memory");
      if (lane == 0) {
        const unsigned fv = (unsigned)s + 1;
        if (local)
          __builtin_amdgcn_raw_buffer_store_b32(fv, f_rs, (g * 32 + ub) * 4, 0, 0);
        else
          __builtin_amdgcn_raw_buffer_store_b32(fv, f_rs, (g * 32 + ub) * 4, 0, kSc1);
      }
    }
    trace_at(s, 5);
  }
  __syncthreads();
  if (io && !kAblStores) store_out(T - 1);
  if (camax != nullptr) {
    __syncthreads();
    red[(0 * LB + m) * LU + u] = cm_r;
    red[(1 * LB + m) * LU + u] = cm_z;
    red[(2 * LB + m) * LU + u] = cm_n;
    red[(3 * LB + m) * LU + u] = cm_hn;
    __syncthreads();
    if (threadIdx.x < 4 * LU) {
      const int gq = threadIdx.x / LU, uu = threadIdx.x - gq * LU;
      float a = 0.f;
#pragma unroll
      for (int mm = 0; mm < LB; ++mm) a = fmaxf(a, red[(gq * LB + mm) * LU + uu]);
      const unsigned bits = __float_as_uint(a);
      const int cl = d * H3 + ub * LU + uu;
      if (bits != 0u) {
        if (gq < 2) {
          atomicMax(camax + cl + gq * H, bits);
          atomicMax(camax + D * H3 + cl + gq * H, bits);
        } else if (gq == 2) {
          atomicMax(camax + cl + 2 * H, bits);
        } else {
          atomicMax(camax + D * H3 + cl + 2 * H, bits);
        }
      }
    }
  }
  if (dbp == nullptr) return;
  double* rd = reinterpret_cast<double*>(red);
  __syncthreads();
  rd[(0 * LB + m) * LU + u] = owner ? sb_r : 0.0;
  rd[(1 * LB + m) * LU + u] = owner ? sb_z : 0.0;
  rd[(2 * LB + m) * LU + u] = owner ? sb_n : 0.0;
  rd[(3 * LB + m) * LU + u] = owner ? sb_hn : 0.0;
  __syncthreads();
  if (threadIdx.x < 4 * LU) {
    const int gq = threadIdx.x / LU, uu = threadIdx.x - gq * LU;
    double a = 0.0;
#pragma unroll
    for (int mm = 0; mm < LB; ++mm) a += rd[(gq * LB + mm) * LU + uu];
    dbp[(((int64_t)bt * D + d) * 4 + gq) * H + ub * LU + uu] = a;
  }
}


static inline bool env_off(const char* name) {
  const char* e = getenv(name);
  return e != nullptr && e[0] == '0';
}
static inline bool xl_enabled() { return !env_off("DS2_GRU_XL") && !env_off("DS2_GRU_X6"); }
static inline int xl_force_global() {
  const char* e = getenv("DS2_GRU_XL");
  return (e != nullptr && e[0] == '2') ? 1 : 0;
}

int gru_xl_groups(int n, int h, int num_dirs) {
  if (!xl_enabled() || n < 1 || h < LU || (h % LU) != 0) return 0;
  const int UBX = h / LU, BTX = (n + LB - 1) / LB, G = num_dirs * BTX;
  if (UBX > 32 || G > 8 || (UBX + LW - 1) / LW > 7) return 0;
  return G;
}

int gru_xl_active(int n, int h, int num_dirs) {
  const int G = gru_xl_groups(n, h, num_dirs);
  return G > 0 ? G * (h / LU) : 0;
}

size_t gru_xl_ctr_words() { return 520; }

static const void* fwd_xl_fn(int UBX) {
  const int need = (UBX + LW - 1) / LW;
#define DS2_FXL(K) \
  if (need <= K + 1) return reinterpret_cast<const void*>(gru_fwd_xl_kernel<K>);
  DS2_FXL(1) DS2_FXL(3) DS2_FXL(6)
#undef DS2_FXL
  return nullptr;
}

static const void* bwd_xl_fn(int UBX) {
  const int need = (UBX + LW - 1) / LW;
#define DS2_BXL(K) \
  if (need <= K + 1) return reinterpret_cast<const void*>(gru_bwd_xl_kernel<K>);
  DS2_BXL(1) DS2_BXL(3) DS2_BXL(6)
#undef DS2_BXL
  return nullptr;
}

size_t gru_xl_ring_bytes(int n, int h, int num_dirs, bool bwd) {
  const size_t UBX = h / LU, G = (size_t)num_dirs * ((n + LB - 1) / LB);
  return bwd ? 2 * G * UBX * LRB * sizeof(float) : LSLOTS * G * UBX * 256 * sizeof(float);
}

bool launch_gru_fwd_xl(int t_max, int n, int h, int num_dirs, const float* xproj,
                       const float* w_hh_f, const float* w_hh_r, const float* b_hh_f,
                       const float* b_hh_r, const int* lens, float* h_all, float* gates,
                       float* ring, unsigned* xl, unsigned* err, unsigned long long* stamps,
                       size_t lds_pad, hipStream_t st) {
  if (gru_xl_groups(n, h, num_dirs) == 0 || env_off("DS2_GRU_H3")) return false;
  apply_spin_limit_env();
  apply_rnn_tune_env();
  const int UBX = h / LU, BTX = (n + LB - 1) / LB;
  const void* fn = fwd_xl_fn(UBX);
  if (fn == nullptr) return false;
  int T_ = t_max, N_ = n, H_ = h, D_ = num_dirs, UB_ = UBX, BT_ = BTX, FG_ = xl_force_global();
  void* args[] = {&T_, &N_, &H_, &D_, &UB_, &BT_, &xproj, &w_hh_f, &w_hh_r, &b_hh_f,
                  &b_hh_r, &lens, &h_all, &gates, &ring, &xl, &err, &stamps, &FG_};
  return rnn_launch(fn, dim3(8 * UBX), dim3(LT), args, lds_pad, st) == hipSuccess;
}

bool launch_gru_bwd_xl(int t_max, int n, int h, int num_dirs, const float* dy, int dy_dirs,
                       const float* w_hh_f, const float* w_hh_r, const float* h_all,
                       const float* gates, const int* lens, float* dgates_x, float* dgates_h,
                       float* ring, unsigned* xl, unsigned* err, unsigned long long* stamps,
                       double* dbp, size_t lds_pad, hipStream_t st, unsigned* camax) {
  if (gru_xl_groups(n, h, num_dirs) == 0 || env_off("DS2_GRU_H3_BWD")) return false;
  apply_spin_limit_env();
  apply_rnn_tune_env();
  const int UBX = h / LU, BTX = (n + LB - 1) / LB;
  const void* fn = bwd_xl_fn(UBX);
  if (fn == nullptr) return false;
  int T_ = t_max, N_ = n, H_ = h, D_ = num_dirs, UB_ = UBX, BT_ = BTX, DYD_ = dy_dirs;
  int FG_ = xl_force_global();
  void* args[] = {&T_, &N_, &H_, &D_, &UB_, &BT_, &dy, &DYD_, &w_hh_f, &w_hh_r, &h_all,
                  &gates, &lens, &dgates_x, &dgates_h, &ring, &xl, &err, &stamps, &dbp, &camax,
                  &FG_};
  return rnn_launch(fn, dim3(8 * UBX), dim3(LT), args, lds_pad, st) == hipSuccess;
}

}
```

### deepspeech.pytorch_amd/csrc/rnn_common.h

```cpp
#pragma once

#include "common.h"

#include <cstdlib>

namespace ds2 {

constexpr int GU = 16;
constexpr int GB = 16;
constexpr int GW = 8;
constexpr int GT = GW * 64;

template <int G>
__global__ void pack_fwd_kernel(const float* __restrict__ w_f, const float* __restrict__ w_r,
                                int H, int D, int UB, int KS, float* __restrict__ wp) {
  const int64_t total = (int64_t)D * UB * KS * G * 64;
  for (int64_t i = blockIdx.x * (int64_t)blockDim.x + threadIdx.x; i < total;
       i += (int64_t)gridDim.x * blockDim.x) {
    int64_t r = i;
    const int l = r % 64; r /= 64;
    const int g = r % G; r /= G;
    const int ks = r % KS; r /= KS;
    const int ub = r % UB; r /= UB;
    const int d = static_cast<int>(r);
    const float* w = d == 0 ? w_f : w_r;
    const int u = ub * GU + (l & 15);
    const int k = 4 * ks + (l >> 4);
    wp[i] = (u < H && k < H) ? w[(int64_t)(g * H + u) * H + k] : 0.f;
  }
}

template <int G>
__global__ void pack_bwd_kernel(const float* __restrict__ w_f, const float* __restrict__ w_r,
                                int H, int D, int UB, int KS, float* __restrict__ wp) {
  const int64_t total = (int64_t)D * UB * KS * 64;
  for (int64_t i = blockIdx.x * (int64_t)blockDim.x + threadIdx.x; i < total;
       i += (int64_t)gridDim.x * blockDim.x) {
    int64_t r = i;
    const int l = r % 64; r /= 64;
    const int ks = r % KS; r /= KS;
    const int ub = r % UB; r /= UB;
    const int d = static_cast<int>(r);
    const float* w = d == 0 ? w_f : w_r;
    const int u = ub * GU + (l & 15);
    const int k = 4 * ks + (l >> 4);
    wp[i] = (u < H && k < G * H) ? w[(int64_t)k * H + u] : 0.f;
  }
}

__device__ __forceinline__ void stage_rows(const float* __restrict__ src, int64_t ld, int N,
                                           int n0, int kc0, int kc1, float* __restrict__ hs,
                                           int pitch) {
  const int width = kc1 - kc0;
  const int pairs = (width + 1) >> 1;
  for (int i = threadIdx.x; i < GB * pairs; i += blockDim.x) {
    const int m = i / pairs;
    const int kp = (i - m * pairs) * 2;
    const int n = n0 + m;
    float2 v = make_float2(0.f, 0.f);
    if (n < N) {
      const float* p = src + (int64_t)n * ld + kc0 + kp;
      v.x = p[0];
      v.y = (kp + 1 < width) ? p[1] : 0.f;
    }
    *reinterpret_cast<float2*>(hs + m * pitch + kp) = v;
  }
}

__device__ __forceinline__ bool map_work(int P, int BT, int UB, int& ub, int& d, int& bt) {
  const int wg = blockIdx.x;
  const int xcd = wg & 7;
  const int slot = wg >> 3;
  const int pair = xcd + 8 * (slot / BT);
  bt = slot - (slot / BT) * BT;
  if (pair >= P) return false;
  ub = pair % UB;
  d = pair / UB;
  return true;
}

static inline int mapped_grid(int P, int BT) { return 8 * ((P + 7) / 8) * BT; }

static inline bool xgrp_fits(int UB, int BT, int D) {
  const int G = D * BT;
  return G >= 1 && G <= 8 && 8 % G == 0 && UB % (8 / G) == 0;
}
static inline int xgrp_grid(int UB, int BT, int D) { return 8 * (UB / (8 / (D * BT))); }
static inline bool xcd_groups_on() {
  const char* xe = getenv("DS2_GRU_XCD");
  return !(xe != nullptr && xe[0] == '0');
}
__device__ __forceinline__ bool map_work_xgrp(int UB, int BT, int D, int& ub, int& d, int& bt) {
  const int wg = blockIdx.x;
  const int xcd = wg & 7, slot = wg >> 3;
  const int G = D * BT, xpg = 8 / G, per = UB / xpg;
  const int q = xcd / xpg, part = xcd - q * xpg;
  if (slot >= per || q >= G) return false;
  ub = part * per + slot;
  d = q / BT;
  bt = q - d * BT;
  return true;
}
__device__ __forceinline__ unsigned xcc_id() {
  return __builtin_amdgcn_s_getreg(20 | (0 << 6) | ((4 - 1) << 11)) & 15u;
}


constexpr unsigned kSpinLimit = 1u << 21;

static __constant__ unsigned g_spin_limit = kSpinLimit;

static void apply_spin_limit_env() {
  static unsigned applied = kSpinLimit;
  const char* e = getenv("DS2_RNN_SPIN_LIMIT");
  const unsigned v = (e == nullptr || e[0] == 0) ? kSpinLimit
                                                 : static_cast<unsigned>(strtoul(e, nullptr, 10));
  if (v == applied) return;
  if (hipMemcpyToSymbol(HIP_SYMBOL(g_spin_limit), &v, sizeof(v)) == hipSuccess) applied = v;
}

constexpr unsigned kRepollSleep = 1u, kFirstPollDelay = 7u, kFirstPollDelayBwd = 14u,
                   kFlagPollSleep = 1u, kFlagPollGap = 0u, kFlagFirstDelay = 0u, kXlRepoll = 8u,
                   kXlFirstDelay = 0u;
constexpr int kTuneN = 8;
static __constant__ unsigned g_rnn_tune[kTuneN] = {kRepollSleep, kFirstPollDelay,
                                                   kFirstPollDelayBwd, kFlagPollSleep,
                                                   kFlagPollGap, kFlagFirstDelay, kXlRepoll,
                                                   kXlFirstDelay};

static void apply_rnn_tune_env() {
  static unsigned applied[kTuneN] = {kRepollSleep, kFirstPollDelay, kFirstPollDelayBwd,
                                     kFlagPollSleep, kFlagPollGap, kFlagFirstDelay, kXlRepoll,
                                     kXlFirstDelay};
  unsigned v[kTuneN] = {kRepollSleep, kFirstPollDelay, kFirstPollDelayBwd, kFlagPollSleep,
                        kFlagPollGap, kFlagFirstDelay, kXlRepoll, kXlFirstDelay};
  const char* e = getenv("DS2_RNN_TUNE");
  for (int i = 0; e != nullptr && e[0] != 0 && i < kTuneN; ++i) {
    char* end = nullptr;
    v[i] = static_cast<unsigned>(strtoul(e, &end, 10));
    e = (end != nullptr && *end == ',') ? end + 1 : nullptr;
  }
  bool same = true;
  for (int i = 0; i < kTuneN; ++i) same = same && v[i] == applied[i];
  if (same) return;
  if (hipMemcpyToSymbol(HIP_SYMBOL(g_rnn_tune), v, sizeof(v)) == hipSuccess)
    for (int i = 0; i < kTuneN; ++i) applied[i] = v[i];
}

__device__ __forceinline__ void sleep_units(unsigned k) {
  for (unsigned i = 0; i < k; ++i) __builtin_amdgcn_s_sleep(1);
}

static __global__ void err_fold_kernel(const unsigned* __restrict__ err, unsigned* __restrict__ out) {
  if (threadIdx.x == 0) {
    const unsigned v = __hip_atomic_load(err, __ATOMIC_RELAXED, __HIP_MEMORY_SCOPE_AGENT);
    if (v != 0u) __hip_atomic_fetch_or(out, v, __ATOMIC_RELAXED, __HIP_MEMORY_SCOPE_AGENT);
  }
}

static inline void fold_err(const unsigned* err, unsigned* err_out, hipStream_t st) {
  if (err_out != nullptr) hipLaunchKernelGGL(err_fold_kernel, dim3(1), dim3(64), 0, st, err, err_out);
}

__device__ __forceinline__ void st_sc1(float* p, float v) {
  __hip_atomic_store(p, v, __ATOMIC_RELAXED, __HIP_MEMORY_SCOPE_AGENT);
}

__device__ __forceinline__ unsigned long long ld_sc1_u64(const float* p) {
  return __hip_atomic_load(reinterpret_cast<const unsigned long long*>(p), __ATOMIC_RELAXED,
                           __HIP_MEMORY_SCOPE_AGENT);
}

__device__ __forceinline__ float ld_sc1(const float* p) {
  return __hip_atomic_load(p, __ATOMIC_RELAXED, __HIP_MEMORY_SCOPE_AGENT);
}

__device__ __forceinline__ bool flags_wait(const unsigned* flags, int count, unsigned target,
                                           unsigned* err, int* lds_flag, int poll_wave = 0) {
  if ((threadIdx.x >> 6) == poll_wave) {
    const int lane = threadIdx.x & 63;
    unsigned spins = 0;
    int ok = 1;
    if (g_spin_limit == 0) {
      if (lane == 0) __hip_atomic_fetch_or(err, 1u, __ATOMIC_RELAXED, __HIP_MEMORY_SCOPE_AGENT);
      ok = 0;
    }
    auto poll = [&]() {
      return lane < count ? __hip_atomic_load(flags + lane, __ATOMIC_RELAXED,
                                              __HIP_MEMORY_SCOPE_AGENT)
                          : target;
    };
    const unsigned gap = g_rnn_tune[4];
    sleep_units(g_rnn_tune[5]);
    if (gap != 0u && ok) {
      unsigned a = poll();
      sleep_units(gap);
      unsigned b = poll();
      for (;;) {
        if (__ballot(a < target) == 0ull) break;
        a = poll();
        if (__ballot(b < target) == 0ull) break;
        b = poll();
        if (++spins > g_spin_limit) {
          if (lane == 0) __hip_atomic_fetch_or(err, 1u, __ATOMIC_RELAXED, __HIP_MEMORY_SCOPE_AGENT);
          ok = 0;
          break;
        }
      }
      asm volatile("s_waitcnt vmcnt(0)" ::: "memory");
    }
    for (; ok && gap == 0u;) {
      const unsigned v = poll();
      if (__ballot(v < target) == 0ull) break;
      sleep_units(g_rnn_tune[3]);
      if (++spins > g_spin_limit) {
        if (lane == 0) __hip_atomic_fetch_or(err, 1u, __ATOMIC_RELAXED, __HIP_MEMORY_SCOPE_AGENT);
        ok = 0;
        break;
      }
    }
    if (lane == 0) *lds_flag = ok;
  }
  __syncthreads();
  return *lds_flag != 0;
}

__device__ __forceinline__ void poison_rest(float* out, int s, int T, bool rev, int N, int D,
                                            int n, int d, int H, int j, int width, int groups,
                                            bool owner) {
  if (!owner || out == nullptr) return;
  for (int q = s; q < T; ++q) {
    const int t = rev ? T - 1 - q : q;
    float* o = out + (((int64_t)t * N + n) * D + d) * width + j;
    for (int g = 0; g < groups; ++g) o[(int64_t)g * H] = __builtin_nanf("");
  }
}

__device__ __forceinline__ void simd_split(int nblk, int wave, int& b0, int& nb) {
  auto simd_lo = [&](int s) { return (nblk * s) / 4; };
  auto wave_cnt = [&](int w) {
    const int s = w & 3;
    const int c = simd_lo(s + 1) - simd_lo(s);
    return w < 4 ? (c + 1) / 2 : c / 2;
  };
  int start = 0;
  for (int w = 0; w < wave; ++w) start += wave_cnt(w);
  b0 = start;
  nb = wave_cnt(wave);
}

__device__ __forceinline__ void flags_arrive(unsigned* flag, unsigned value) {
  asm volatile("s_waitcnt vmcnt(0)" ::: "memory");
  __syncthreads();
  if (threadIdx.x == 0) __hip_atomic_store(flag, value, __ATOMIC_RELAXED, __HIP_MEMORY_SCOPE_AGENT);
}

typedef unsigned int u32x4 __attribute__((ext_vector_type(4)));
constexpr int kSc1 = 16;

template <typename T>
__device__ __forceinline__ void settle(T& v) { asm volatile("" : "+v"(v)); }

constexpr unsigned kSentinel = 0xFFFFFFFFu;
constexpr int kRingSlots = 4;

__device__ __forceinline__ bool tile_ready(f32x4 v) {
  const u32x4 b = __builtin_bit_cast(u32x4, v);
  return (b.x != kSentinel) & (b.y != kSentinel) & (b.z != kSentinel) & (b.w != kSentinel);
}

__device__ __forceinline__ u32x4 desentinel(u32x4 v) {
  const unsigned qnan = 0x7FC00000u;
  return u32x4{v.x == kSentinel ? qnan : v.x, v.y == kSentinel ? qnan : v.y,
               v.z == kSentinel ? qnan : v.z, v.w == kSentinel ? qnan : v.w};
}

__device__ __forceinline__ bool wave_ready(f32x4 v) { return __ballot(!tile_ready(v)) == 0ull; }

__device__ __forceinline__ bool spin_tile(f32x4& v, __amdgpu_buffer_rsrc_t rs, int off,
                                          unsigned* err) {
  for (unsigned spins = 0; g_spin_limit == 0 || !wave_ready(v); ++spins) {
    if (spins > g_spin_limit || g_spin_limit == 0) {
      if ((threadIdx.x & 63) == 0)
        __hip_atomic_fetch_or(err, 1u, __ATOMIC_RELAXED, __HIP_MEMORY_SCOPE_AGENT);
      return false;
    }
    __builtin_amdgcn_s_sleep(1);
    asm volatile("" ::: "memory");
    v = __builtin_bit_cast(f32x4, __builtin_amdgcn_raw_buffer_load_b128(rs, off, 0, kSc1));
  }
  return true;
}

template <int MAXI, int ROWS = GB>
__device__ __forceinline__ void stage_rows_sc1(const float* src, int ld, int N, int n0,
                                               int width, int cols, float* __restrict__ hs,
                                               int pitch) {
  const __amdgpu_buffer_rsrc_t rs =
      __builtin_amdgcn_make_buffer_rsrc(const_cast<float*>(src), (short)0, N * ld * 4, 0x00020000);
  const int q = cols >> 2;
  const int total = ROWS * q;
  u32x4 v[MAXI];
#pragma unroll
  for (int r = 0; r < MAXI; ++r) {
    const int i = threadIdx.x + r * GT;
    int off = 0x7ffffff0;
    if (i < total) {
      const int m = i / q;
      const int k = (i - m * q) * 4;
      if (k < width) off = ((n0 + m) * ld + k) * 4;
    }
    v[r] = __builtin_amdgcn_raw_buffer_load_b128(rs, off, 0, kSc1);
  }
#pragma unroll
  for (int r = 0; r < MAXI; ++r) {
    const int i = threadIdx.x + r * GT;
    if (i < total) {
      const int m = i / q;
      const int k = (i - m * q) * 4;
      *reinterpret_cast<u32x4*>(hs + m * pitch + k) = v[r];
    }
  }
}

__device__ __forceinline__ unsigned long long stamp_now() { return __builtin_amdgcn_s_memtime(); }

static int g_num_cus = -1;
static int num_cus() {
  if (g_num_cus < 0) {
    int dev = 0, v = 0;
    if (hipGetDevice(&dev) != hipSuccess) dev = 0;
    if (hipDeviceGetAttribute(&v, hipDeviceAttributeMultiprocessorCount, dev) != hipSuccess) v = 0;
    g_num_cus = v;
  }
  return g_num_cus;
}

static int persist_ksw(int per, int kc) {
  const int opts[] = {8, 16, 25, 32, 48, 64, 75};
  for (int k : opts)
    if (per <= k && 4 * GW * k <= kc) return k;
  return -1;
}

static bool persistent_enabled() {
  const char* e = getenv("DS2_RNN_PERSISTENT");
  return !(e != nullptr && e[0] == '0');
}

static inline hipError_t rnn_launch(const void* fn, dim3 grid, dim3 block, void** args,
                                    size_t lds, hipStream_t st) {
  constexpr size_t max_lds = 160 * 1024;
  hipFuncAttributes fa;
  if (hipFuncGetAttributes(&fa, fn) != hipSuccess) return hipErrorInvalidDeviceFunction;
  const size_t stat = fa.sharedSizeBytes;
  if (stat > max_lds) return hipErrorInvalidValue;
  if (stat + lds > max_lds) lds = max_lds - stat;
  return hipLaunchKernel(fn, grid, block, args, lds, st);
}

static inline int grid_cap(int64_t work) {
  int64_t g = (work + 255) / 256;
  return static_cast<int>(g > 2048 ? 2048 : (g < 1 ? 1 : g));
}

static inline size_t align256(size_t x) { return (x + 255) & ~(size_t)255; }

typedef _Float16 f16x8 __attribute__((ext_vector_type(8)));
typedef _Float16 f16x2h __attribute__((ext_vector_type(2)));
struct Duo {
  f16x8 hi, lo;
};

__device__ __forceinline__ Duo split2h(const f32x4 a, const f32x4 b, float sc) {
  typedef float f32x2v __attribute__((ext_vector_type(2)));
  Duo t;
#pragma unroll
  for (int j = 0; j < 4; ++j) {
    const f32x2v x = (j < 2 ? f32x2v{a[2 * j], a[2 * j + 1]} : f32x2v{b[2 * j - 4], b[2 * j - 3]}) * sc;
    const f16x2h h = __builtin_convertvector(x, f16x2h);
    const f16x2h l = __builtin_convertvector(x - __builtin_convertvector(h, f32x2v), f16x2h);
    t.hi[2 * j] = h[0];
    t.hi[2 * j + 1] = h[1];
    t.lo[2 * j] = l[0];
    t.lo[2 * j + 1] = l[1];
  }
  return t;
}

__device__ __forceinline__ f32x4 mma3h(const Duo& a, const Duo& b, f32x4 c) {
  c = __builtin_amdgcn_mfma_f32_16x16x32_f16(a.lo, b.hi, c, 0, 0, 0);
  c = __builtin_amdgcn_mfma_f32_16x16x32_f16(a.hi, b.lo, c, 0, 0, 0);
  c = __builtin_amdgcn_mfma_f32_16x16x32_f16(a.hi, b.hi, c, 0, 0, 0);
  return c;
}

__device__ __forceinline__ int h3_row_exp(float m) {
  const unsigned u = __float_as_uint(m);
  const int E = (int)(u >> 23);
  if (u == 0u || E >= 255) return 0;
  const int e = 14 - ((E == 0 ? 1 : E) - 127);
  return e > 127 ? 127 : e;
}

}
```

### deepspeech.pytorch_amd/ds2amd/_lib.py

```python
from __future__ import annotations

import ctypes
import os
import threading

_HERE = os.path.dirname(os.path.abspath(__file__))
LIB_PATH = os.environ.get("DS2_LIB_PATH") or os.path.join(_HERE, "libds2hip.so")

_c_int = ctypes.c_int
_c_i64 = ctypes.c_int64
_c_f = ctypes.c_float
_vp = ctypes.c_void_p
_sz = ctypes.c_size_t

_PROTOS = {
    "ds2_status_string": (ctypes.c_char_p, [_c_int]),
    "ds2_last_error": (ctypes.c_char_p, []),
    "ds2_version": (ctypes.c_char_p, []),
    "ds2_stft_workspace_size": (_sz, [_c_int, _c_int, _c_int]),
    "ds2_stft_logmag": (_c_int, [_vp, _vp, _c_int, _c_int, _c_int, _c_int, _vp, _c_int, _vp,
                                 _c_int, _vp, _c_int, _vp, _sz, _vp]),
    "ds2_stft_logmag_masked": (_c_int, [_vp, _vp, _c_int, _c_int, _c_int, _c_int, _vp, _c_int,
                                        _vp, _c_int, _vp, _vp, _c_int, _vp, _sz, _vp]),
    "ds2_wave_aug_workspace_size": (_sz, [_c_int, _c_i64]),
    "ds2_wave_aug": (_c_int, [_vp, _c_i64, _vp, _c_int, _vp, _vp, _c_int, _vp, _c_i64, _vp,
                              _c_i64, _vp, _c_i64, _vp, _vp, _sz, _vp]),
    "ds2_time_stretch_workspace_size": (_sz, [_c_int, _c_int, _c_int]),
    "ds2_time_stretch": (_c_int, [_vp, _c_i64, _vp, _c_int, _vp, _vp, _vp, _vp, _vp, _vp, _c_i64,
                                  _c_int, _c_int, _vp, _sz, _vp]),
    "ds2_resample_workspace_size": (_sz, [_c_int, _c_i64]),
    "ds2_resample": (_c_int, [_vp, _c_i64, _vp, _c_int, _vp, _vp, _vp, _c_int, _c_int, _vp,
                              _c_i64, _vp, _sz, _vp]),
    "ds2_sgemm": (_c_int, [_c_int, _c_int, _c_int, _c_int, _c_int, _c_f, _vp, _c_i64, _c_i64,
                           _vp, _c_i64, _c_i64, _c_f, _vp, _c_i64, _c_i64, _c_int, _vp, _vp]),
    "ds2_sgemm_workspace_size": (_sz, [_c_int, _c_int, _c_int, _c_int]),
    "ds2_sgemm_ws": (_c_int, [_c_int, _c_int, _c_int, _c_int, _c_int, _c_f, _vp, _c_i64, _c_i64,
                              _vp, _c_i64, _c_i64, _c_f, _vp, _c_i64, _c_i64, _c_int, _vp, _vp,
                              _sz, _vp]),
    "ds2_sgemm_bf16_workspace_size": (_sz, [_c_int, _c_int, _c_int, _c_int]),
    "ds2_sgemm_bf16_ws": (_c_int, [_c_int, _c_int, _c_int, _c_int, _c_int, _c_f, _vp, _c_i64,
                                   _c_i64, _vp, _c_i64, _c_i64, _c_f, _vp, _c_i64, _c_i64, _c_int,
                                   _vp, _vp, _sz, _vp]),
    "ds2_conv2d_workspace_size": (_sz, [_c_int] * 11),
    "ds2_conv2d_fwd": (_c_int, [_vp, _vp, _vp, _vp] + [_c_int] * 11 + [_vp, _vp, _sz, _vp]),
    "ds2_conv2d_dgrad": (_c_int, [_vp, _vp, _vp] + [_c_int] * 11 + [_vp, _sz, _vp]),
    "ds2_conv2d_wgrad_workspace_size": (_sz, [_c_int] * 11),
    "ds2_conv2d_wgrad": (_c_int, [_vp, _vp, _vp, _vp] + [_c_int] * 11 + [_vp, _sz, _vp]),
    "ds2_bn_workspace_size": (_sz, [_c_int, _c_int, _c_int]),
    "ds2_bn_train_stats": (_c_int, [_vp, _c_int, _c_int, _c_int, _c_f, _c_f, _vp, _vp, _vp, _vp,
                                    _vp, _sz, _vp]),
    "ds2_bn_eval_stats": (_c_int, [_vp, _vp, _c_int, _c_f, _vp, _vp, _vp]),
    "ds2_bn_apply": (_c_int, [_vp, _c_int, _c_int, _c_int, _vp, _vp, _vp, _vp, _vp, _vp]),
    "ds2_bn_apply_amax": (_c_int, [_vp, _c_int, _c_int, _vp, _vp, _vp, _vp, _vp, _vp, _vp, _vp]),
    "ds2_bn_apply_mask_htanh": (_c_int, [_vp, _c_int, _c_int, _c_int, _c_int, _vp, _vp, _vp, _vp,
                                         _vp, _c_f, _c_f, _vp, _c_int, _vp]),
    "ds2_bn_backward": (_c_int, [_vp, _c_int, _vp, _c_int, _c_int, _c_int, _c_int, _vp, _vp, _vp,
                                 _vp, _c_int, _vp, _c_f, _c_f, _vp, _vp, _vp, _vp, _vp, _sz,
                                 _vp]),
    "ds2_gru_fwd_workspace_size": (_sz, [_c_int, _c_int, _c_int]),
    "ds2_gru_cache_floats": (_sz, [_c_int, _c_int, _c_int, _c_int]),
    "ds2_gru_fwd": (_c_int, [_c_int, _c_int, _c_int, _c_int, _vp, _vp, _vp, _vp, _vp, _vp, _vp,
                             _vp, _vp, _vp, _sz, _vp]),
    "ds2_gru_bwd_workspace_size": (_sz, [_c_int, _c_int, _c_int]),
    "ds2_gru_bwd_grid": (_c_int, [_c_int, _c_int, _c_int]),
    "ds2_lstm_bwd_grid": (_c_int, [_c_int, _c_int, _c_int]),
    "ds2_bgemm_workspace_size": (_sz, [_c_int, _c_int, _c_int]),
    "ds2_bgemm_nt": (_c_int, [_c_int, _c_int, _c_int, _c_f, _vp, _c_i64, _vp, _c_i64, _c_f, _vp,
                              _c_i64, _vp, _vp, _sz, _vp]),
    "ds2_cvt_bf16": (_c_int, [_vp, _c_int, _c_int, _c_i64, _vp, _c_i64, _c_int, _vp]),
    "ds2_rnn_fwd": (_c_int, [_c_int, _c_int, _c_int, _c_int, _vp, _vp, _vp, _vp, _vp, _vp, _vp,
                             _vp]),
    "ds2_rnn_bwd": (_c_int, [_c_int, _c_int, _c_int, _c_int, _vp, _c_int, _vp, _vp, _vp, _vp,
                             _vp, _vp]),
    "ds2_rnn_fwd_workspace_size": (_sz, [_c_int, _c_int, _c_int]),
    "ds2_rnn_fwd_ws": (_c_int, [_c_int, _c_int, _c_int, _c_int, _vp, _vp, _vp, _vp, _vp, _vp, _vp,
                                _vp, _vp, _sz, _vp]),
    "ds2_rnn_bwd_workspace_size": (_sz, [_c_int, _c_int, _c_int]),
    "ds2_rnn_bwd_grid": (_c_int, [_c_int, _c_int, _c_int]),
    "ds2_rnn_bwd_ws": (_c_int, [_c_int, _c_int, _c_int, _c_int, _vp, _c_int, _vp, _vp, _vp, _vp,
                                _vp, _vp, _vp, _vp, _sz, _vp]),
    "ds2_test_occupy": (_c_int, [_c_int, _c_int, _c_int, _vp, _vp]),
    "ds2_test_rnn_launch_lds": (_c_int, [_c_int, _c_int, _vp, _vp]),
    "ds2_test_timestamp": (_c_int, [_vp, _vp]),
    "ds2_amax": (_c_int, [_vp, _c_int, _c_int, _c_i64, _vp, _vp, _vp]),
    "ds2_sgemm_amax_ws": (_c_int, [_c_int, _c_int, _c_int, _c_int, _c_int, _c_f, _vp, _c_i64, _vp,
                                   _c_i64, _c_f, _vp, _c_i64, _vp, _vp, _vp, _vp, _sz, _vp]),
    "ds2_test_ring_traffic": (_c_int, [_vp, _c_i64, _c_int, _vp, _c_int, ctypes.c_double, _vp]),
    "ds2_test_beam_stamps": (_c_int, [_vp]),
    "ds2_gru_bwd": (_c_int, [_c_int, _c_int, _c_int, _c_int, _vp, _c_int, _vp, _vp, _vp, _vp,
                             _vp, _vp, _vp, _vp, _vp, _sz, _vp]),
    "ds2_gru_bwd_bias": (_c_int, [_c_int, _c_int, _c_int, _c_int, _vp, _c_int, _vp, _vp, _vp,
                                  _vp, _vp, _vp, _vp, _vp, _vp, _vp, _vp, _vp, _vp, _sz, _vp]),
    "ds2_gru_bwd_bias_amax": (_c_int, [_c_int, _c_int, _c_int, _c_int, _vp, _c_int, _vp, _vp,
                                       _vp, _vp, _vp, _vp, _vp, _vp, _vp, _vp, _vp, _vp, _vp, _vp,
                                       _sz, _vp]),
    "ds2_lstm_fwd_workspace_size": (_sz, [_c_int, _c_int, _c_int]),
    "ds2_lstm_fwd": (_c_int, [_c_int, _c_int, _c_int, _c_int, _vp, _vp, _vp, _vp, _vp, _vp, _vp,
                              _vp, _vp, _vp, _vp, _sz, _vp]),
    "ds2_lstm_bwd_workspace_size": (_sz, [_c_int, _c_int, _c_int]),
    "ds2_lstm_bwd": (_c_int, [_c_int, _c_int, _c_int, _c_int, _vp, _c_int, _vp, _vp, _vp, _vp,
                              _vp, _vp, _vp, _vp, _sz, _vp]),
    "ds2_lstm_bwd_half_grid": (_c_int, [_c_int, _c_int, _c_int]),
    "ds2_lstm_bwd_half": (_c_int, [_c_int, _c_int, _c_int, _c_int, _vp, _c_int, _vp, _vp, _vp,
                                   _vp, _vp, _vp, _vp, _vp, _sz, _vp]),
    "ds2_lookahead_fwd": (_c_int, [_vp, _c_int, _c_int, _c_int, _vp, _c_int, _c_int, _c_f,
                                   _c_f, _vp, _vp]),
    "ds2_lookahead_bwd_workspace_size": (_sz, [_c_int, _c_int, _c_int, _c_int]),
    "ds2_lookahead_bwd": (_c_int, [_vp, _vp, _c_f, _c_f, _vp, _c_int, _c_int, _c_int, _vp,
                                   _c_int, _vp, _vp, _vp, _sz, _vp]),
    "ds2_dirsum": (_c_int, [_vp, _c_int, _c_int, _c_int, _vp, _vp]),
    "ds2_colsum_workspace_size": (_sz, [_c_int, _c_int]),
    "ds2_colsum": (_c_int, [_vp, _c_int, _c_int, _c_i64, _vp, _c_int, _vp, _sz, _vp]),
    "ds2_softmax_tnc": (_c_int, [_vp, _c_int, _c_int, _c_int, _vp, _vp]),
    "ds2_softmax_tnc_bwd": (_c_int, [_vp, _vp, _c_int, _c_int, _c_int, _vp, _c_int, _vp]),
    "ds2_ctc_workspace_size": (_sz, [_c_int, _c_int, _c_int]),
    "ds2_ctc_loss": (_c_int, [_vp, _c_int, _c_int, _c_int, _vp, _vp, _vp, _c_int, _c_int, _c_int,
                              _vp, _vp, _vp, _sz, _vp]),
    "ds2_greedy_decode": (_c_int, [_vp, _c_int, _c_int, _c_int, _c_i64, _c_i64, _vp, _c_int, _vp,
                                   _vp, _vp, _vp, _vp]),
    "ds2_edit_distance": (_c_int, [_vp, _c_i64, _vp, _vp, _vp, _vp, _c_int, _c_int, _vp, _vp,
                                   _vp]),
    "ds2_ctc_beam_workspace_size": (_sz, [_c_int, _c_int, _c_int]),
    "ds2_ctc_beam_decode": (_c_int, [_vp, _c_int, _c_int, _c_int, _c_i64, _c_i64, _vp, _c_int,
                                     _c_int, _c_int, ctypes.c_double, _c_int, _vp, _vp, _vp, _vp,
                                     _vp, _sz, _vp]),
    "ds2_ctc_beam_decode_lm": (_c_int, [_vp, _c_int, _c_int, _c_int, _c_i64, _c_i64, _vp, _c_int,
                                        _c_int, _c_int, ctypes.c_double, _c_int, _c_int, _c_int,
                                        _c_int, _c_int, ctypes.c_double, ctypes.c_double, _vp, _vp,
                                        _vp, _c_int, _c_int, _vp, _c_i64, _vp, _vp, _vp, _vp, _vp,
                                        _sz, _vp]),
    "ds2_comm_id_bytes": (_sz, []),
    "ds2_comm_get_unique_id": (_c_int, [_vp]),
    "ds2_comm_init": (_c_int, [_vp, _vp, _c_int, _c_int, _c_int]),
    "ds2_allreduce_bucket": (_c_int, [_vp, _vp, _c_i64, _vp]),
    "ds2_comm_destroy": (_c_int, [_vp]),
    "ds2_optim_workspace_size": (_sz, [_c_i64]),
    "ds2_grad_norm": (_c_int, [_vp, _c_i64, _vp, _vp, _sz, _vp]),
    "ds2_clip_sgd_nesterov": (_c_int, [_vp, _vp, _vp, _c_i64, _c_f, _c_f, _c_f, _vp, _vp, _vp]),
    "ds2_clip_sgd_nesterov_wd": (_c_int, [_vp, _vp, _vp, _c_i64, _c_f, _c_f, _c_f, _c_f, _vp, _vp,
                                          _vp]),
    "ds2_clip_adam": (_c_int, [_vp, _vp, _vp, _vp, _c_i64] + [ctypes.c_double] * 5
                      + [_c_f, _vp, _vp, _vp, _vp]),
    "ds2_nan_guard": (_c_int, [_vp, _c_i64, _c_int, _vp, _vp, _vp]),
    "ds2_zero_masked": (_c_int, [_vp, _vp, _c_i64, _vp, _vp]),
    "ds2_scale_by_device_scalar": (_c_int, [_vp, _c_i64, _vp, _vp]),
}

EXPORTED_SYMBOLS = tuple(_PROTOS)

_lock = threading.Lock()
_lib = None


class Ds2Error(RuntimeError):
    pass


def load() -> ctypes.CDLL:
    global _lib
    if _lib is not None:
        return _lib
    with _lock:
        if _lib is not None:
            return _lib
        if not os.path.exists(LIB_PATH):
            raise Ds2Error(
                f"libds2hip.so not found at {LIB_PATH}; build it with "
                "`make -C deepspeech.pytorch_amd/csrc` (or __graft_entry__.build()). "
                "There is no CPU fallback for the product path.")
        lib = ctypes.CDLL(LIB_PATH)
        for name, (res, args) in _PROTOS.items():
            fn = getattr(lib, name)
            fn.restype = res
            fn.argtypes = args
        _lib = lib
    return _lib


def check(status: int, what: str) -> None:
    if status != 0:
        lib = load()
        msg = lib.ds2_status_string(status).decode()
        last = lib.ds2_last_error().decode()
        raise Ds2Error(f"{what} failed: {msg}" + (f" ({last})" if last else ""))


def call(name: str, *args) -> None:
    lib = load()
    check(getattr(lib, name)(*args), name)


def size(name: str, *args) -> int:
    return int(getattr(load(), name)(*args))
```

### deepspeech.pytorch_amd/ds2amd/ops.py

```python
from __future__ import annotations

from typing import Optional, Tuple

import os
import numpy as np
import torch

from . import _lib

_F32 = torch.float32
_I32 = torch.int32


def _stream() -> int:
    return torch.cuda.current_stream().cuda_stream


def _p(t: Optional[torch.Tensor]) -> Optional[int]:
    return None if t is None else t.data_ptr()


def _need(t: torch.Tensor, name: str, dtype=_F32) -> torch.Tensor:
    if not t.is_cuda:
        raise _lib.Ds2Error(f"{name}: expected a device tensor (got {t.device}); "
# ... 451 lines not shown


_FX_CONST = {}


def _fx_window(dev):
    key = ('hann', dev)
    if key not in _FX_CONST:
        _FX_CONST[key] = torch.from_numpy(hann_periodic(FX_N_FFT)).to(dev)
    return _FX_CONST[key]


def kaiser_best_filter() -> tuple:
    from scipy.signal.windows import kaiser
    num_zeros, num_bits, beta, rolloff = 64, 2 ** 9, 14.769656459379492, 0.9475937167399596
    n = num_bits * num_zeros
    sinc_win = rolloff * np.sinc(rolloff * np.linspace(0, num_zeros, num=n + 1, endpoint=True))
    taper = kaiser(2 * n + 1, beta)[n:]
    return taper * sinc_win, num_bits


def _fx_filter(dev):
    key = ('kaiser_best', dev)
    if key not in _FX_CONST:
        win, nb = kaiser_best_filter()
        _FX_CONST[key] = (torch.from_numpy(np.ascontiguousarray(win)).to(dev), nb)
    return _FX_CONST[key]


def stretch_plan(in_len: int, rate: float) -> tuple:
    import math
    frames = 1 + in_len // FX_HOP
    out_len = int(round(in_len / rate))
    out_frames = int(math.ceil((frames - 0) / rate))
    used = min(out_frames, int(math.ceil((out_len + FX_N_FFT) / FX_HOP)))
    return out_len, out_frames, used


def time_stretch(pcm: torch.Tensor, lens, rates) -> tuple:
    pcm = _need(pcm, "time_stretch.pcm")
    n = pcm.shape[0]
    dev = pcm.device
    plans = [stretch_plan(int(l), float(r)) for l, r in zip(lens, rates)]
    out_lens = [p[0] for p in plans]
    stride = max(1, max(out_lens) if out_lens else 1)
    max_in = max([1 + int(l) // FX_HOP for l in lens] or [1])
    max_out = max([p[1] for p in plans] or [1])
    i32 = lambda v: torch.tensor(v, dtype=_I32).to(dev)
    out = torch.empty(n, stride, device=dev, dtype=_F32)
    ws = _ws(_lib.size("ds2_time_stretch_workspace_size", n, max_in, max_out), dev)
    lens_d, rate_d = i32([int(l) for l in lens]), torch.tensor([float(r) for r in rates],
                                                               dtype=torch.float64).to(dev)
    of_d, uf_d, ol_d = i32([p[1] for p in plans]), i32([p[2] for p in plans]), i32(out_lens)
    _lib.call("ds2_time_stretch", pcm.data_ptr(), pcm.stride(0), lens_d.data_ptr(), n,
              rate_d.data_ptr(), of_d.data_ptr(), uf_d.data_ptr(), ol_d.data_ptr(),
              _fx_window(dev).data_ptr(), out.data_ptr(), stride, max_in, max_out, ws.data_ptr(),
              ws.numel(), _stream())
    return out, out_lens


def resample(pcm: torch.Tensor, lens, ratios, out_lens=None) -> tuple:
    pcm = _need(pcm, "resample.pcm")
    n = pcm.shape[0]
    dev = pcm.device
    valid = [int(int(l) * float(r)) for l, r in zip(lens, ratios)]
    if out_lens is None:
        out_lens = valid
    stride = max(1, max(out_lens) if len(out_lens) else 1)
    out = torch.empty(n, stride, device=dev, dtype=_F32)
    win, nb = _fx_filter(dev)
    ws = _ws(_lib.size("ds2_resample_workspace_size", n, stride), dev)
    lens_d = torch.tensor([int(l) for l in lens], dtype=_I32).to(dev)
    valid_d = torch.tensor([min(v, o) for v, o in zip(valid, out_lens)], dtype=_I32).to(dev)
    ratio_d = torch.tensor([float(r) for r in ratios], dtype=torch.float64).to(dev)
    _lib.call("ds2_resample", pcm.data_ptr(), pcm.stride(0), lens_d.data_ptr(), n,
              ratio_d.data_ptr(), valid_d.data_ptr(), win.data_ptr(), win.numel(), nb,
              out.data_ptr(), stride, ws.data_ptr(), ws.numel(), _stream())
    return out, list(out_lens)


SPECT_ROWS = 161


def stft_logmag(pcm: torch.Tensor, n_samples: torch.Tensor, n_fft: int, hop: int,
                window: torch.Tensor, normalize: int, gauss_taps: Optional[torch.Tensor],
                max_frames: int, masks: Optional[torch.Tensor] = None) -> torch.Tensor:
    pcm = _need(pcm, "stft.pcm")
    n_samples = _need(n_samples, "stft.n_samples", _I32)
    window = _need(window, "stft.window", torch.float64)
    b, max_samples = pcm.shape
    out = torch.empty(b, SPECT_ROWS, max_frames, device=pcm.device, dtype=_F32)
    ws = _ws(_lib.size("ds2_stft_workspace_size", b, max_frames, n_fft), pcm.device)
    radius = 0 if gauss_taps is None else (gauss_taps.numel() - 1) // 2
    if masks is not None:
        masks = _need(masks, "stft.masks", _I32)
        if tuple(masks.shape) != (b, 9):
            raise _lib.Ds2Error(f"stft masks must be [batch, 9], got {tuple(masks.shape)}")
    _lib.call("ds2_stft_logmag_masked", pcm.data_ptr(), n_samples.data_ptr(), b, max_samples,
              n_fft, hop, window.data_ptr(), int(normalize), _p(gauss_taps), radius, _p(masks),
              out.data_ptr(), max_frames, ws.data_ptr(), ws.numel(), _stream())
    return out


class ConvBlockFn(torch.autograd.Function):

    @staticmethod
    def forward(ctx, x, lens, weight, bias, gamma, beta, running_mean, running_var, training,
                momentum, eps, stride, padding, lo, hi, out_layout):
        z = conv2d_fwd(x, weight, bias, stride, padding, out_lens=lens)
        n, c, d, t = z.shape
        mean, invstd = bn_stats(z, n, c, d * t, eps, momentum, running_mean, running_var, training)
        if out_layout == 1:
            y = torch.empty(t, n, c * d, device=z.device, dtype=_F32)
        else:
            y = torch.empty_like(z)
        _lib.call("ds2_bn_apply_mask_htanh", z.data_ptr(), n, c, d, t, mean.data_ptr(),
                  invstd.data_ptr(), gamma.data_ptr(), beta.data_ptr(), _p(lens), float(lo),
                  float(hi), y.data_ptr(), int(out_layout), _stream())
        ctx.save_for_backward(x, z, lens, weight, gamma, beta, mean, invstd)
        ctx.bias = bias
        ctx.cfg = (stride, padding, lo, hi, out_layout, bias is not None, training)
        return y

    @staticmethod
    def backward(ctx, dy):
        x, z, lens, weight, gamma, beta, mean, invstd = ctx.saved_tensors
        stride, padding, lo, hi, out_layout, has_bias, training = ctx.cfg
        if not training:
            raise _lib.Ds2Error("ConvBlockFn backward in eval mode is not supported")
        dy = dy.contiguous()
        n, c, d, t = z.shape
        dz, dgamma, dbeta, dbias = bn_backward(dy, out_layout, z, n, c, d, t, mean, invstd, gamma,
                                               beta, masked=True, lens=lens, lo=lo, hi=hi,
                                               want_dbias=has_bias, bias=ctx.bias)
        dx = None
        if ctx.needs_input_grad[0]:
            dx = conv2d_dgrad(dz, weight, x.shape, stride, padding)
        dw, _ = conv2d_wgrad(dz, x, weight.shape, stride, padding, with_bias=False,
                             out_dw=grad_like(weight))
        return (dx, None, dw, dbias, dgamma, dbeta) + (None,) * 10


class SeqBatchNormFn(torch.autograd.Function):

    @staticmethod
    def forward(ctx, x2d, gamma, beta, running_mean, running_var, training, momentum, eps):
        x2d = x2d.contiguous()
        r, c = x2d.shape
        mean, invstd = bn_stats(x2d, r, c, 1, eps, momentum, running_mean, running_var, training)
        y = (bn_apply_amax(x2d, r, c, mean, invstd, gamma, beta) if h3_enabled()
             else bn_apply(x2d, r, c, 1, mean, invstd, gamma, beta))
        ctx.save_for_backward(x2d, gamma, beta, mean, invstd)
        ctx.training = training
        return y

    @staticmethod
    def backward(ctx, dy):
        x2d, gamma, beta, mean, invstd = ctx.saved_tensors
        if not ctx.training:
            raise _lib.Ds2Error("SeqBatchNormFn backward in eval mode is not supported")
        r, c = x2d.shape
        dx, dgamma, dbeta, _ = bn_backward(dy.contiguous(), 0, x2d, r, c, 1, 1, mean, invstd,
                                           gamma, beta)
        return dx.view(r, c), dgamma, dbeta, None, None, None, None, None


class LinearFn(torch.autograd.Function):

    @staticmethod
    def forward(ctx, x2d, weight):
        x2d = x2d.contiguous()
        ctx.save_for_backward(x2d, weight)
        m, k = x2d.shape
        x_r, ctx.x_c = _take_amax(x2d, m, k) if h3_enabled() else (None, None)
        out = torch.empty(m, weight.shape[0], device=x2d.device, dtype=_F32)
        return sgemm(x2d, weight, out, m=m, n=weight.shape[0], k=k, trans_b=True, lda=k, ldb=k,
                     ldc=weight.shape[0], a_amax=x_r)

    @staticmethod
    def backward(ctx, dy):
        x2d, weight = ctx.saved_tensors
        dy = dy.contiguous()
        m, k = x2d.shape
        n = weight.shape[0]
        dx = None
        if ctx.needs_input_grad[0]:
            dx = torch.empty_like(x2d)
            sgemm(dy, weight, dx, m=m, n=k, k=n, lda=n, ldb=k, ldc=k)
        dw = grad_like(weight)
        sgemm(dy, x2d, dw, m=n, n=k, k=m, trans_a=True, lda=n, ldb=k, ldc=k, b_amax=ctx.x_c)
        return dx, dw


_RNN_GEMM_BF16 = [False]


class rnn_gemm_precision:

    def __init__(self, precision: str):
        if precision not in ('fp32', 'bf16'):
            raise ValueError(f"rnn GEMM precision must be 'fp32' or 'bf16', got {precision!r}")
        self.bf16 = precision == 'bf16'

    def __enter__(self):
        self.prev = _RNN_GEMM_BF16[0]
        _RNN_GEMM_BF16[0] = self.bf16
        return self

    def __exit__(self, *exc):
        _RNN_GEMM_BF16[0] = self.prev
        return False


def _stacked_rows(a: torch.Tensor, b: torch.Tensor):
    if a.dim() != 2 or tuple(b.shape) != tuple(a.shape) or not (a.is_contiguous() and
                                                                   b.is_contiguous()):
        return None
    if a.untyped_storage().data_ptr() != b.untyped_storage().data_ptr():
        return None
    if b.data_ptr() != a.data_ptr() + a.numel() * a.element_size():
        return None
    return a.as_strided((2 * a.shape[0], a.shape[1]), (a.shape[1], 1))


def _rnn_input_proj(x, weights, nd, g, bf16=False, need_dx=False):
    t, n, inp = x.shape
    x2d = x.view(t * n, inp)
    xproj = torch.empty(t, n, nd, g, device=x.device, dtype=_F32)
    ws = _stacked_rows(weights[0], weights[4]) if nd == 2 else None
    pre = {}
    x_r = w_r = None
    if h3_enabled() and not bf16:
        x_r, pre["x_c"] = _take_amax(x2d, t * n, inp)
        if pre["x_c"] is None:
            del pre["x_c"]
        elif ws is not None:
            w_r, w_c = amax(ws, 2 * g, inp, inp, want_cols=need_dx)
            if w_c is not None:
                pre["w_c"] = w_c
    if ws is not None:
        bias = torch.cat([weights[2], weights[6]])
        sgemm(x2d, ws, xproj, m=t * n, n=2 * g, k=inp, trans_b=True, lda=inp, ldb=inp,
              ldc=2 * g, bias=bias, bf16=bf16, a_amax=x_r, b_amax=w_r)
        return xproj, pre
    for d in range(nd):
        w_ih, _, b_ih, _ = weights[4 * d: 4 * d + 4]
        sgemm(x2d, w_ih, xproj, m=t * n, n=g, k=inp, trans_b=True, lda=inp, ldb=inp,
              ldc=nd * g, bias=b_ih, c_off=d * g, bf16=bf16, a_amax=x_r)
    return xproj, pre


def _rnn_output(h_all, sum_dirs, nd):
    t, n, _, h = h_all.shape
    if sum_dirs and nd == 2:
        y = torch.empty(t, n, h, device=h_all.device, dtype=_F32)
        _lib.call("ds2_dirsum", h_all.data_ptr(), t * n, nd, h, y.data_ptr(), _stream())
        return y
    return h_all.view(t, n, nd * h)


def _rnn_param_grads_bf16(x2d, h_all, dgx, dgh, weights, nd, g, t, n, inp, h, need_dx, dbias):
    dev = x2d.device
    tn = t * n
    ld = nd * g
    dgx2 = dgx.view(tn, ld)
    dgx_t = to_bf16(dgx2, transpose=True)
    dgh_t = dgx_t if dgh is dgx else to_bf16(dgh.view(tn, ld), transpose=True)
    x_t = to_bf16(x2d, transpose=True)
    h_t = to_bf16(h_all.view(tn, nd * h), transpose=True)
    dx = torch.empty(t, n, inp, device=dev, dtype=_F32) if need_dx else None
    grads = []
    if dx is not None:
        dgx_b = to_bf16(dgx2)
        w_all = torch.cat([weights[4 * d] for d in range(nd)], 0) if nd > 1 else weights[0]
        w_t = to_bf16(w_all, transpose=True)
        bgemm_nt(dgx_b, w_t, dx.view(tn, inp))
    for d in range(nd):
        w_ih, w_hh, b_ih, b_hh = weights[4 * d: 4 * d + 4]
        dw_ih = grad_like(w_ih)
        bgemm_nt(dgx_t[d * g:(d + 1) * g], x_t, dw_ih)
        if dbias is not None:
            db_ih, db_hh = dbias[2 * d], dbias[2 * d + 1]
        else:
            db_ih = grad_like(b_ih)
            colsum(dgx, tn, g, ld, db_ih, off=d * g)
        k = (t - 1) * n
        ka, kb = (n, 0) if d == 0 else (0, n)
        dw_hh = grad_like(w_hh)
        bgemm_nt(dgh_t[d * g:(d + 1) * g, ka:ka + k], h_t[d * h:(d + 1) * h, kb:kb + k], dw_hh)
        if dbias is None:
            db_hh = grad_like(b_hh)
            if dgh is dgx:
                db_hh.copy_(db_ih)
            elif g == 3 * h:
                db_hh[:2 * h].copy_(db_ih[:2 * h])
                colsum(dgh, tn, h, ld, db_hh[2 * h:], off=d * g + 2 * h)
            else:
                colsum(dgh, tn, g, ld, db_hh, off=d * g)
        grads += [dw_ih, dw_hh, db_ih, db_hh]
    return dx, grads


def _rnn_param_grads(x, h_all, dgx, dgh, weights, nd, g, need_dx, bf16=False, pre=None,
                     dbias=None, shared_bf16=True, col_amax=None):
    t, n, inp = x.shape
    h = h_all.shape[-1]
    dev = x.device
    x2d = x.view(t * n, inp)
    tn = t * n
    ld = nd * g
    if bf16 and shared_bf16 and t > 1 and all(v % 8 == 0 for v in (n, inp, h, g)):
        return _rnn_param_grads_bf16(x2d, h_all, dgx, dgh, weights, nd, g, t, n, inp, h,
                                     need_dx, dbias)
    grads = []
    dx = torch.empty(t, n, inp, device=dev, dtype=_F32) if need_dx else None
    w_st = _stacked_rows(weights[0], weights[4]) if nd == 2 else None
    dw_ih_all = [grad_like(weights[4 * d]) for d in range(nd)]
    dw_st = _stacked_rows(dw_ih_all[0], dw_ih_all[1]) if w_st is not None else None
    am = {}
    if h3_enabled() and not bf16:
        if col_amax is not None:
            am["dgx_c"] = col_amax[:ld]
            am["dgh_c"] = col_amax[ld:] if col_amax.numel() == 2 * ld else am["dgx_c"]
            if need_dx:
                am["dgx_r"] = amax(dgx, tn, ld, ld, want_cols=False)[0]
        else:
            am["dgx_r"], am["dgx_c"] = amax(dgx, tn, ld, ld, want_rows=need_dx)
            am["dgh_c"] = am["dgx_c"] if dgh is dgx else amax(dgh, tn, ld, ld, want_rows=False)[1]
        pre = pre or {}
        am["x_c"] = pre["x_c"] if "x_c" in pre else amax(x2d, tn, inp, inp, want_rows=False)[1]
        am["h"] = unit_bound(nd * h, dev)
        if need_dx:
            if w_st is not None:
                am["w_c"] = (pre["w_c"] if "w_c" in pre
                             else amax(w_st, 2 * g, inp, inp, want_rows=False)[1])
            else:
                am["w_c"] = [amax(weights[4 * d], g, inp, inp, want_rows=False)[1]
                             for d in range(nd)]

    def sl(key, lo, hi):
        v = am.get(key)
        return None if v is None else v[lo:hi]

    if dw_st is not None:
        sgemm(dgx, x2d, dw_st, m=2 * g, n=inp, k=tn, trans_a=True, lda=ld, ldb=inp, ldc=inp,
              bf16=bf16, a_amax=am.get("dgx_c"), b_amax=am.get("x_c"))
    if dx is not None and w_st is not None:
        sgemm(dgx, w_st, dx, m=tn, n=inp, k=2 * g, lda=ld, ldb=inp, ldc=inp, bf16=bf16,
              a_amax=am.get("dgx_r"), b_amax=am.get("w_c"))
    for d in range(nd):
        w_ih, w_hh, b_ih, b_hh = weights[4 * d: 4 * d + 4]
        dw_ih = dw_ih_all[d]
        if dw_st is None:
            sgemm(dgx, x2d, dw_ih, m=g, n=inp, k=tn, trans_a=True, lda=ld, ldb=inp, ldc=inp,
                  a_off=d * g, bf16=bf16, a_amax=sl("dgx_c", d * g, (d + 1) * g),
                  b_amax=am.get("x_c"))
        if dbias is not None:
            db_ih, db_hh = dbias[2 * d], dbias[2 * d + 1]
        else:
            db_ih = grad_like(b_ih)
            colsum(dgx, tn, g, ld, db_ih, off=d * g)
        dw_hh = grad_like(w_hh)
        if t > 1:
            a_off = (n * ld if d == 0 else 0) + d * g
            b_off = (0 if d == 0 else n * nd * h) + d * h
            sgemm(dgh, h_all, dw_hh, m=g, n=h, k=(t - 1) * n, trans_a=True, lda=ld,
                  ldb=nd * h, ldc=h, a_off=a_off, b_off=b_off, bf16=bf16,
                  a_amax=sl("dgh_c", d * g, (d + 1) * g), b_amax=sl("h", d * h, (d + 1) * h))
        else:
            dw_hh.zero_()
        if dbias is None:
            db_hh = grad_like(b_hh)
            if dgh is dgx:
                db_hh.copy_(db_ih)
            elif g == 3 * h:
                db_hh[:2 * h].copy_(db_ih[:2 * h])
                colsum(dgh, tn, h, ld, db_hh[2 * h:], off=d * g + 2 * h)
            else:
                colsum(dgh, tn, g, ld, db_hh, off=d * g)
        if dx is not None and w_st is None:
            sgemm(dgx, w_ih, dx, m=tn, n=inp, k=g, lda=ld, ldb=inp, ldc=inp,
                  beta=0.0 if d == 0 else 1.0, a_off=d * g, bf16=bf16,
                  a_amax=am.get("dgx_r"), b_amax=None if "w_c" not in am else am["w_c"][d])
        grads += [dw_ih, dw_hh, db_ih, db_hh]
    return dx, grads


_COOP_GUARD = [None]


def set_cooperative_guard(fn) -> None:
    _COOP_GUARD[0] = fn


def persistent_bwd_grid(cell: str, n: int, h: int, nd: int) -> int:
    fn = {"gru": "ds2_gru_bwd_grid", "lstm": "ds2_lstm_bwd_grid", "rnn": "ds2_rnn_bwd_grid",
          "lstm_half": "ds2_lstm_bwd_half_grid"}[cell]
    return _lib.size(fn, n, h, nd)


def _guard_cooperative(cell, n, h, nd):
    g = _COOP_GUARD[0]
    if g is not None:
        grid = persistent_bwd_grid(cell, n, h, nd)
        if grid > 0:
            g(grid)


class GRULayerFn(torch.autograd.Function):

    @staticmethod
    def forward(ctx, x, lens, sum_dirs, hidden, *weights):
        x = x.contiguous()
        t, n, _ = x.shape
        h = hidden
        nd = len(weights) // 4
        dev = x.device
        bf16 = _RNN_GEMM_BF16[0]
        xproj, ctx.pre = _rnn_input_proj(x, weights, nd, 3 * h, bf16, ctx.needs_input_grad[0])
        h_all = torch.empty(t, n, nd, h, device=dev, dtype=_F32)
        need_grad = any(ctx.needs_input_grad)
        gates = (torch.empty(_lib.size("ds2_gru_cache_floats", t, n, h, nd), device=dev,
                             dtype=_F32) if need_grad else None)
        w_hh_f, b_hh_f = weights[1], weights[3]
        w_hh_r = weights[5] if nd == 2 else None
        b_hh_r = weights[7] if nd == 2 else None
        ws = _ws(_lib.size("ds2_gru_fwd_workspace_size", n, h, nd), dev)
        _lib.call("ds2_gru_fwd", t, n, h, nd, xproj.data_ptr(), w_hh_f.data_ptr(), _p(w_hh_r),
                  b_hh_f.data_ptr(), _p(b_hh_r), lens.data_ptr(), h_all.data_ptr(), _p(gates),
                  rnn_status_word(dev).data_ptr(), ws.data_ptr(), ws.numel(), _stream())
        ctx.save_for_backward(x, lens, h_all, gates, *weights)
        ctx.cfg = (sum_dirs, h, nd, bf16)
        return _rnn_output(h_all, sum_dirs, nd)

    @staticmethod
    def backward(ctx, dy):
        x, lens, h_all, gates, *weights = ctx.saved_tensors
        sum_dirs, h, nd, bf16 = ctx.cfg
        t, n, _ = x.shape
        dev = x.device
        h3 = 3 * h
        dy = dy.contiguous()
        dy_dirs = 1 if (sum_dirs and nd == 2) else nd
        dgx = torch.empty(t, n, nd, h3, device=dev, dtype=_F32)
        dgh = torch.empty(t, n, nd, h3, device=dev, dtype=_F32)
        w_hh_f = weights[1]
        w_hh_r = weights[5] if nd == 2 else None
        ws = _ws(_lib.size("ds2_gru_bwd_workspace_size", n, h, nd), dev)
        _guard_cooperative("gru", n, h, nd)
        dbias = [grad_like(weights[4 * d + k]) for d in range(nd) for k in (2, 3)]
        common = (t, n, h, nd, dy.data_ptr(), dy_dirs, w_hh_f.data_ptr(), _p(w_hh_r),
                  h_all.data_ptr(), gates.data_ptr(), lens.data_ptr(), dgx.data_ptr(),
                  dgh.data_ptr(), dbias[0].data_ptr(), dbias[1].data_ptr(),
                  _p(dbias[2] if nd == 2 else None), _p(dbias[3] if nd == 2 else None))
        col_amax = None
        if h3_enabled() and not bf16:
            col_amax = torch.empty(2 * nd * h3, dtype=_I32, device=dev)
            _lib.call("ds2_gru_bwd_bias_amax", *common, col_amax.data_ptr(),
                      rnn_status_word(dev).data_ptr(), ws.data_ptr(), ws.numel(), _stream())
        else:
            _lib.call("ds2_gru_bwd_bias", *common, rnn_status_word(dev).data_ptr(),
                      ws.data_ptr(), ws.numel(), _stream())
        dx, grads = _rnn_param_grads(x, h_all, dgx, dgh, weights, nd, h3,
                                     ctx.needs_input_grad[0], bf16, ctx.pre, dbias=dbias,
                                     col_amax=col_amax)
        return (dx, None, None, None, *grads)


class RNNLayerFn(torch.autograd.Function):

    @staticmethod
    def forward(ctx, x, lens, sum_dirs, hidden, *weights):
        x = x.contiguous()
        t, n, _ = x.shape
        h = hidden
        nd = len(weights) // 4
        dev = x.device
        bf16 = _RNN_GEMM_BF16[0]
        xproj, ctx.pre = _rnn_input_proj(x, weights, nd, h, bf16, ctx.needs_input_grad[0])
        h_all = torch.empty(t, n, nd, h, device=dev, dtype=_F32)
        ws = _ws(_lib.size("ds2_rnn_fwd_workspace_size", n, h, nd), dev)
        _lib.call("ds2_rnn_fwd_ws", t, n, h, nd, xproj.data_ptr(), weights[1].data_ptr(),
                  _p(weights[5] if nd == 2 else None), weights[3].data_ptr(),
                  _p(weights[7] if nd == 2 else None), lens.data_ptr(), h_all.data_ptr(),
                  rnn_status_word(dev).data_ptr(), ws.data_ptr(), ws.numel(), _stream())
        ctx.save_for_backward(x, lens, h_all, *weights)
        ctx.cfg = (sum_dirs, h, nd, bf16)
        return _rnn_output(h_all, sum_dirs, nd)

    @staticmethod
    def backward(ctx, dy):
        x, lens, h_all, *weights = ctx.saved_tensors
        sum_dirs, h, nd, bf16 = ctx.cfg
        t, n, _ = x.shape
        dy = dy.contiguous()
        dy_dirs = 1 if (sum_dirs and nd == 2) else nd
        dev = x.device
        dg = torch.empty(t, n, nd, h, device=dev, dtype=_F32)
        ws = _ws(_lib.size("ds2_rnn_bwd_workspace_size", n, h, nd), dev)
        _guard_cooperative("rnn", n, h, nd)
        col_amax = (torch.empty(nd * h, dtype=_I32, device=dev)
                    if h3_enabled() and not bf16 else None)
        _lib.call("ds2_rnn_bwd_ws", t, n, h, nd, dy.data_ptr(), dy_dirs, weights[1].data_ptr(),
                  _p(weights[5] if nd == 2 else None), h_all.data_ptr(), lens.data_ptr(),
                  dg.data_ptr(), _p(col_amax), rnn_status_word(dev).data_ptr(), ws.data_ptr(),
                  ws.numel(), _stream())
        dx, grads = _rnn_param_grads(x, h_all, dg, dg, weights, nd, h,
                                     ctx.needs_input_grad[0], bf16, ctx.pre, col_amax=col_amax)
        return (dx, None, None, None, *grads)


class LSTMLayerFn(torch.autograd.Function):

    @staticmethod
    def forward(ctx, x, lens, sum_dirs, hidden, *weights):
        x = x.contiguous()
        t, n, _ = x.shape
        h = hidden
        nd = len(weights) // 4
        dev = x.device
        bf16 = _RNN_GEMM_BF16[0]
        xproj, ctx.pre = _rnn_input_proj(x, weights, nd, 4 * h, bf16, ctx.needs_input_grad[0])
        h_all = torch.empty(t, n, nd, h, device=dev, dtype=_F32)
        need_grad = any(ctx.needs_input_grad)
        c_all = torch.empty(t, n, nd, h, device=dev, dtype=_F32) if need_grad else None
        gates = torch.empty(t, n, nd, 4 * h, device=dev, dtype=_F32) if need_grad else None
        w_hh_f, b_hh_f = weights[1], weights[3]
        w_hh_r = weights[5] if nd == 2 else None
        b_hh_r = weights[7] if nd == 2 else None
        ws = _ws(_lib.size("ds2_lstm_fwd_workspace_size", n, h, nd), dev)
        _lib.call("ds2_lstm_fwd", t, n, h, nd, xproj.data_ptr(), w_hh_f.data_ptr(), _p(w_hh_r),
                  b_hh_f.data_ptr(), _p(b_hh_r), lens.data_ptr(), h_all.data_ptr(), _p(c_all),
                  _p(gates), rnn_status_word(dev).data_ptr(), ws.data_ptr(), ws.numel(), _stream())
        ctx.save_for_backward(x, lens, h_all, c_all, gates, *weights)
        ctx.cfg = (sum_dirs, h, nd, bf16)
        return _rnn_output(h_all, sum_dirs, nd)

    @staticmethod
    def backward(ctx, dy):
        x, lens, h_all, c_all, gates, *weights = ctx.saved_tensors
        sum_dirs, h, nd, bf16 = ctx.cfg
        t, n, _ = x.shape
        dev = x.device
        dy = dy.contiguous()
        dy_dirs = 1 if (sum_dirs and nd == 2) else nd
        dg = torch.empty(t, n, nd, 4 * h, device=dev, dtype=_F32)
        w_hh_f = weights[1]
        w_hh_r = weights[5] if nd == 2 else None
        ws = _ws(_lib.size("ds2_lstm_bwd_workspace_size", n, h, nd), dev)
        half = bf16 and os.environ.get("DS2_LSTM_HALF", "1")[:1] != "0"
        _guard_cooperative("lstm_half" if half else "lstm", n, h, nd)
        _lib.call("ds2_lstm_bwd_half" if half else "ds2_lstm_bwd", t, n, h, nd, dy.data_ptr(),
                  dy_dirs, w_hh_f.data_ptr(),
                  _p(w_hh_r), c_all.data_ptr(), gates.data_ptr(), lens.data_ptr(), dg.data_ptr(),
                  rnn_status_word(dev).data_ptr(), ws.data_ptr(), ws.numel(), _stream())
        dx, grads = _rnn_param_grads(x, h_all, dg, dg, weights, nd, 4 * h,
                                     ctx.needs_input_grad[0], bf16, ctx.pre)
        return (dx, None, None, None, *grads)


class LookaheadFn(torch.autograd.Function):

    @staticmethod
    def forward(ctx, x, weight, clamp):
        x = _need(x, "lookahead x").contiguous()
        w = _need(weight, "lookahead weight").contiguous()
        t, n, h = x.shape
        context = w.shape[1] - 1
        y = torch.empty_like(x)
        lo, hi = clamp if clamp is not None else (0.0, 0.0)
        _lib.call("ds2_lookahead_fwd", x.data_ptr(), t, n, h, w.data_ptr(), context,
                  int(clamp is not None), lo, hi, y.data_ptr(), _stream())
        ctx.save_for_backward(x, w, y if clamp is not None else None)
        ctx.clamp = clamp
        return y

    @staticmethod
    def backward(ctx, dy):
        x, w, y = ctx.saved_tensors
        t, n, h = x.shape
        context = w.shape[1] - 1
        lo, hi = ctx.clamp if ctx.clamp is not None else (0.0, 0.0)
        dy = dy.contiguous()
        dx = torch.empty_like(x) if ctx.needs_input_grad[0] else None
        dw = grad_like(w) if ctx.needs_input_grad[1] else None
        ws = _ws(_lib.size("ds2_lookahead_bwd_workspace_size", t, n, h, context), x.device)
        _lib.call("ds2_lookahead_bwd", dy.data_ptr(), _p(y), lo, hi, x.data_ptr(), t, n, h,
                  w.data_ptr(), context, _p(dx), _p(dw), ws.data_ptr(), ws.numel(), _stream())
        return dx, dw, None


class CTCLossFn(torch.autograd.Function):

    @staticmethod
    def forward(ctx, acts, labels, act_lens, label_lens, max_label_len, blank, zero_infinity,
                size_average):
        costs, grads = ctc_loss_raw(acts, labels, act_lens, label_lens, max_label_len, blank,
                                    zero_infinity, want_grad=True)
        loss = costs.sum()
        if size_average:
            n = acts.shape[1]
            loss = loss / n
            grads.mul_(1.0 / n)
        ctx.save_for_backward(grads)
        return loss

    @staticmethod
    def backward(ctx, grad_out):
        (grads,) = ctx.saved_tensors
        g = grads.clone()
        go = grad_out.reshape(1).to(dtype=_F32).contiguous()
        _lib.call("ds2_scale_by_device_scalar", g.data_ptr(), g.numel(), go.data_ptr(), _stream())
        return g, None, None, None, None, None, None, None


class SoftmaxTNCFn(torch.autograd.Function):
    @staticmethod
    def forward(ctx, logits_tnc):
        probs = softmax_tnc(logits_tnc)
        ctx.save_for_backward(probs)
        return probs

    @staticmethod
    def backward(ctx, dprobs):
        (probs,) = ctx.saved_tensors
        n, t, c = probs.shape
        d = torch.empty(t, n, c, device=probs.device, dtype=_F32)
        _lib.call("ds2_softmax_tnc_bwd", probs.data_ptr(), dprobs.contiguous().data_ptr(), t, n, c,
                  d.data_ptr(), 0, _stream())
        return d
```

### include/ds2hip.h

```cpp
#ifndef DS2HIP_H
#define DS2HIP_H

#include <stddef.h>
#include <stdint.h>

#ifdef __cplusplus
extern "C" {
#endif

typedef enum ds2_status_t {
  DS2_OK = 0,
  DS2_INVALID_VALUE = 1,
  DS2_UNSUPPORTED_SHAPE = 2,
  DS2_HIP_ERROR = 3,
  DS2_RCCL_ERROR = 4,
  DS2_WORKSPACE_TOO_SMALL = 5
} ds2_status_t;

typedef void* ds2_stream_t;

const char* ds2_status_string(ds2_status_t status);
const char* ds2_last_error(void);
const char* ds2_version(void);

size_t ds2_stft_workspace_size(int batch, int max_frames, int n_fft);
ds2_status_t ds2_stft_logmag(const float* pcm, const int* n_samples, int batch, int max_samples,
                             int n_fft, int hop, const double* window, int normalize,
                             const float* gauss_taps, int gauss_radius,
                             float* out, int max_frames, void* ws, size_t ws_bytes,
                             ds2_stream_t stream);
ds2_status_t ds2_stft_logmag_masked(const float* pcm, const int* n_samples, int batch,
                                    int max_samples, int n_fft, int hop, const double* window,
                                    int normalize, const float* gauss_taps, int gauss_radius,
                                    const int* masks, float* out, int max_frames, void* ws,
                                    size_t ws_bytes, ds2_stream_t stream);

size_t ds2_wave_aug_workspace_size(int n, int64_t cap);
ds2_status_t ds2_wave_aug(const float* in, int64_t in_stride, const int* in_lens, int n,
                          const int* op_i, const double* op_f, int max_ops, const double* noise,
                          int64_t noise_stride, float* out, int64_t out_stride,
                          const int* out_lens, int64_t cap, int* err, void* ws, size_t ws_bytes,
                          ds2_stream_t stream);

size_t ds2_time_stretch_workspace_size(int n, int max_in_frames, int max_out_frames);
ds2_status_t ds2_time_stretch(const float* x, int64_t x_stride, const int* in_lens, int n,
                              const double* rate, const int* out_frames, const int* used_frames,
                              const int* out_lens, const double* window, float* out,
                              int64_t out_stride, int max_in_frames, int max_out_frames, void* ws,
                              size_t ws_bytes, ds2_stream_t stream);
size_t ds2_resample_workspace_size(int n, int64_t max_out);
ds2_status_t ds2_resample(const float* x, int64_t x_stride, const int* in_lens, int n,
                          const double* ratio, const int* n_valid, const double* win, int nwin,
                          int num_table, float* out, int64_t out_stride, void* ws,
                          size_t ws_bytes, ds2_stream_t stream);

ds2_status_t ds2_sgemm(int trans_a, int trans_b, int m, int n, int k, float alpha,
                       const float* a, int64_t lda, int64_t stride_a,
                       const float* b, int64_t ldb, int64_t stride_b, float beta,
                       float* c, int64_t ldc, int64_t stride_c, int batch,
                       const float* bias, ds2_stream_t stream);
size_t ds2_sgemm_workspace_size(int m, int n, int k, int batch);
ds2_status_t ds2_sgemm_ws(int trans_a, int trans_b, int m, int n, int k, float alpha,
                          const float* a, int64_t lda, int64_t stride_a,
                          const float* b, int64_t ldb, int64_t stride_b, float beta,
                          float* c, int64_t ldc, int64_t stride_c, int batch,
                          const float* bias, void* ws, size_t ws_bytes, ds2_stream_t stream);
ds2_status_t ds2_amax(const float* x, int rows, int cols, int64_t ld, unsigned* row_amax,
                      unsigned* col_amax, ds2_stream_t stream);
ds2_status_t ds2_sgemm_amax_ws(int trans_a, int trans_b, int m, int n, int k, float alpha,
                               const float* a, int64_t lda, const float* b, int64_t ldb,
                               float beta, float* c, int64_t ldc, const float* bias,
                               const unsigned* a_amax, const unsigned* b_amax, void* ws,
                               size_t ws_bytes, ds2_stream_t stream);
size_t ds2_sgemm_bf16_workspace_size(int m, int n, int k, int batch);
ds2_status_t ds2_sgemm_bf16_ws(int trans_a, int trans_b, int m, int n, int k, float alpha,
                               const float* a, int64_t lda, int64_t stride_a,
                               const float* b, int64_t ldb, int64_t stride_b, float beta,
                               float* c, int64_t ldc, int64_t stride_c, int batch,
                               const float* bias, void* ws, size_t ws_bytes,
                               ds2_stream_t stream);

size_t ds2_conv2d_workspace_size(int n, int c_in, int h_in, int w_in, int c_out, int kh, int kw,
                                 int sh, int sw, int ph, int pw);
ds2_status_t ds2_conv2d_fwd(const float* x, const float* w, const float* bias, float* y,
                            int n, int c_in, int h_in, int w_in, int c_out, int kh, int kw,
                            int sh, int sw, int ph, int pw, const int* out_lens, void* ws,
                            size_t ws_bytes, ds2_stream_t stream);
ds2_status_t ds2_conv2d_dgrad(const float* dy, const float* w, float* dx,
                              int n, int c_in, int h_in, int w_in, int c_out, int kh, int kw,
                              int sh, int sw, int ph, int pw, void* ws, size_t ws_bytes,
                              ds2_stream_t stream);
size_t ds2_conv2d_wgrad_workspace_size(int n, int c_in, int h_in, int w_in, int c_out, int kh,
                                       int kw, int sh, int sw, int ph, int pw);
ds2_status_t ds2_conv2d_wgrad(const float* dy, const float* x, float* dw, float* dbias,
                              int n, int c_in, int h_in, int w_in, int c_out, int kh, int kw,
                              int sh, int sw, int ph, int pw, void* ws, size_t ws_bytes,
                              ds2_stream_t stream);

size_t ds2_bn_workspace_size(int outer, int c, int inner);
ds2_status_t ds2_bn_train_stats(const float* x, int outer, int c, int inner, float eps,
                                float momentum, float* save_mean, float* save_invstd,
                                float* running_mean, float* running_var, void* ws,
                                size_t ws_bytes, ds2_stream_t stream);
ds2_status_t ds2_bn_eval_stats(const float* running_mean, const float* running_var, int c,
                               float eps, float* save_mean, float* save_invstd,
                               ds2_stream_t stream);
ds2_status_t ds2_bn_apply(const float* x, int outer, int c, int inner, const float* mean,
                          const float* invstd, const float* gamma, const float* beta, float* y,
                          ds2_stream_t stream);
ds2_status_t ds2_bn_apply_amax(const float* x, int rows, int c, const float* mean,
                               const float* invstd, const float* gamma, const float* beta,
                               float* y, unsigned* row_amax, unsigned* col_amax,
                               ds2_stream_t stream);
ds2_status_t ds2_bn_apply_mask_htanh(const float* x, int n, int c, int d, int t,
                                     const float* mean, const float* invstd, const float* gamma,
                                     const float* beta, const int* lens, float lo, float hi,
                                     float* y, int out_layout, ds2_stream_t stream);
ds2_status_t ds2_bn_backward(const float* dy, int dy_layout, const float* x, int outer, int c,
                             int d, int t, const float* mean, const float* invstd,
                             const float* gamma, const float* beta, int masked,
                             const int* lens, float lo, float hi, float* dx, float* dgamma,
                             float* dbeta, float* dbias_in, void* ws, size_t ws_bytes,
                             ds2_stream_t stream);

#define DS2_RNN_ERR_HANDOFF_TIMEOUT 1u
size_t ds2_gru_cache_floats(int t_max, int n, int h, int num_dirs);
size_t ds2_gru_fwd_workspace_size(int n, int h, int num_dirs);
ds2_status_t ds2_gru_fwd(int t_max, int n, int h, int num_dirs, const float* xproj,
                         const float* w_hh_f, const float* w_hh_r, const float* b_hh_f,
                         const float* b_hh_r, const int* lens, float* h_all, float* gates,
                         unsigned* err_out, void* ws, size_t ws_bytes, ds2_stream_t stream);
size_t ds2_gru_bwd_workspace_size(int n, int h, int num_dirs);
ds2_status_t ds2_gru_bwd(int t_max, int n, int h, int num_dirs, const float* dy, int dy_dirs,
                         const float* w_hh_f, const float* w_hh_r, const float* h_all,
                         const float* gates, const int* lens, float* dgates_x, float* dgates_h,
                         unsigned* err_out, void* ws, size_t ws_bytes, ds2_stream_t stream);
int ds2_gru_bwd_grid(int n, int h, int num_dirs);
int ds2_lstm_bwd_grid(int n, int h, int num_dirs);
ds2_status_t ds2_gru_bwd_bias(int t_max, int n, int h, int num_dirs, const float* dy, int dy_dirs,
                              const float* w_hh_f, const float* w_hh_r, const float* h_all,
                              const float* gates, const int* lens, float* dgates_x,
                              float* dgates_h, float* db_ih_f, float* db_hh_f, float* db_ih_r,
                              float* db_hh_r, unsigned* err_out, void* ws, size_t ws_bytes,
                              ds2_stream_t stream);
ds2_status_t ds2_gru_bwd_bias_amax(int t_max, int n, int h, int num_dirs, const float* dy,
                                   int dy_dirs, const float* w_hh_f, const float* w_hh_r,
                                   const float* h_all, const float* gates, const int* lens,
                                   float* dgates_x, float* dgates_h, float* db_ih_f,
                                   float* db_hh_f, float* db_ih_r, float* db_hh_r,
                                   unsigned* col_amax, unsigned* err_out, void* ws,
                                   size_t ws_bytes, ds2_stream_t stream);

size_t ds2_lstm_fwd_workspace_size(int n, int h, int num_dirs);
ds2_status_t ds2_lstm_fwd(int t_max, int n, int h, int num_dirs, const float* xproj,
                          const float* w_hh_f, const float* w_hh_r, const float* b_hh_f,
                          const float* b_hh_r, const int* lens, float* h_all, float* c_all,
                          float* gates, unsigned* err_out, void* ws, size_t ws_bytes,
                          ds2_stream_t stream);
size_t ds2_lstm_bwd_workspace_size(int n, int h, int num_dirs);
ds2_status_t ds2_lstm_bwd(int t_max, int n, int h, int num_dirs, const float* dy, int dy_dirs,
                          const float* w_hh_f, const float* w_hh_r, const float* c_all,
                          const float* gates, const int* lens, float* dgates, unsigned* err_out,
                          void* ws, size_t ws_bytes, ds2_stream_t stream);
int ds2_lstm_bwd_half_grid(int n, int h, int num_dirs);
ds2_status_t ds2_lstm_bwd_half(int t_max, int n, int h, int num_dirs, const float* dy, int dy_dirs,
                               const float* w_hh_f, const float* w_hh_r, const float* c_all,
                               const float* gates, const int* lens, float* dgates,
                               unsigned* err_out, void* ws, size_t ws_bytes, ds2_stream_t stream);

ds2_status_t ds2_lookahead_fwd(const float* x, int t, int n, int h, const float* w, int context,
                               int clamp, float lo, float hi, float* y, ds2_stream_t stream);
size_t ds2_lookahead_bwd_workspace_size(int t, int n, int h, int context);
ds2_status_t ds2_lookahead_bwd(const float* dy, const float* y, float lo, float hi,
                               const float* x, int t, int n, int h, const float* w, int context,
                               float* dx, float* dw, void* ws, size_t ws_bytes,
                               ds2_stream_t stream);

ds2_status_t ds2_dirsum(const float* h_all, int rows, int num_dirs, int h, float* y,
                        ds2_stream_t stream);
size_t ds2_colsum_workspace_size(int rows, int cols);
ds2_status_t ds2_colsum(const float* x, int rows, int cols, int64_t ld, float* out,
                        int accumulate, void* ws, size_t ws_bytes, ds2_stream_t stream);

ds2_status_t ds2_softmax_tnc(const float* logits, int t_max, int n, int c, float* probs,
                             ds2_stream_t stream);
ds2_status_t ds2_softmax_tnc_bwd(const float* probs, const float* dprobs, int t_max, int n,
                                 int c, float* dlogits, int accumulate, ds2_stream_t stream);

size_t ds2_ctc_workspace_size(int t_max, int n, int max_label_len);
ds2_status_t ds2_ctc_loss(const float* acts, int t_max, int n, int c, const int* labels,
                          const int* label_lens, const int* act_lens, int max_label_len,
                          int blank, int zero_infinity, float* costs, float* grads, void* ws,
                          size_t ws_bytes, ds2_stream_t stream);

ds2_status_t ds2_greedy_decode(const float* probs, int n, int t_max, int c, int64_t stride_n,
                               int64_t stride_t, const int* sizes, int blank, int* out_ids,
                               int* out_offsets, int* out_counts, int* argmax_out,
                               ds2_stream_t stream);

ds2_status_t ds2_edit_distance(const int* a_ids, int64_t a_stride, const int* a_lens,
                               const int* b_ids, const int* b_offsets, const int* b_lens, int n,
                               int space_id, int* out, int* err, ds2_stream_t stream);

size_t ds2_ctc_beam_workspace_size(int n, int t_max, int beam_width);
ds2_status_t ds2_ctc_beam_decode(const float* probs, int n, int t_max, int c, int64_t stride_n,
                                 int64_t stride_t, const int* sizes, int blank, int beam_width,
                                 int cutoff_top_n, double cutoff_prob, int top_paths,
                                 int* out_ids, int* out_offsets, int* out_lens,
                                 float* out_scores, void* ws, size_t ws_bytes,
                                 ds2_stream_t stream);

ds2_status_t ds2_ctc_beam_decode_lm(const float* probs, int n, int t_max, int c, int64_t stride_n,
                                    int64_t stride_t, const int* sizes, int blank, int beam_width,
                                    int cutoff_top_n, double cutoff_prob, int top_paths,
                                    int space_id, int lm_order, int start_id, int lm_vocab,
                                    double alpha, double beta, const int* dict_next,
                                    const void* dict_mask, const int* dict_word, int dict_states,
                                    int dict_cols, const int* lm_table, int64_t lm_slots,
                                    int* out_ids, int* out_offsets, int* out_lens,
                                    float* out_scores, void* ws, size_t ws_bytes,
                                    ds2_stream_t stream);

size_t ds2_bgemm_workspace_size(int m, int n, int k);
ds2_status_t ds2_bgemm_nt(int m, int n, int k, float alpha, const void* a, int64_t lda,
                          const void* b, int64_t ldb, float beta, float* c, int64_t ldc,
                          const float* bias, void* ws, size_t ws_bytes, ds2_stream_t stream);
ds2_status_t ds2_cvt_bf16(const float* src, int rows, int cols, int64_t ld_src, void* dst,
                          int64_t ld_dst, int transpose, ds2_stream_t stream);

ds2_status_t ds2_rnn_fwd(int t_max, int n, int h, int num_dirs, const float* xproj,
                         const float* w_hh_f, const float* w_hh_r, const float* b_hh_f,
                         const float* b_hh_r, const int* lens, float* h_all,
                         ds2_stream_t stream);
ds2_status_t ds2_rnn_bwd(int t_max, int n, int h, int num_dirs, const float* dy, int dy_dirs,
                         const float* w_hh_f, const float* w_hh_r, const float* h_all,
                         const int* lens, float* dgates, ds2_stream_t stream);
size_t ds2_rnn_fwd_workspace_size(int n, int h, int num_dirs);
ds2_status_t ds2_rnn_fwd_ws(int t_max, int n, int h, int num_dirs, const float* xproj,
                            const float* w_hh_f, const float* w_hh_r, const float* b_hh_f,
                            const float* b_hh_r, const int* lens, float* h_all, unsigned* err_out,
                            void* ws, size_t ws_bytes, ds2_stream_t stream);
size_t ds2_rnn_bwd_workspace_size(int n, int h, int num_dirs);
int ds2_rnn_bwd_grid(int n, int h, int num_dirs);
ds2_status_t ds2_rnn_bwd_ws(int t_max, int n, int h, int num_dirs, const float* dy, int dy_dirs,
                            const float* w_hh_f, const float* w_hh_r, const float* h_all,
                            const int* lens, float* dgates, unsigned* col_amax, unsigned* err_out,
                            void* ws, size_t ws_bytes, ds2_stream_t stream);

typedef struct ds2_comm* ds2_comm_t;
size_t ds2_comm_id_bytes(void);
ds2_status_t ds2_comm_get_unique_id(void* id_out);
ds2_status_t ds2_comm_init(ds2_comm_t* comm, const void* id, int nranks, int rank, int device);
ds2_status_t ds2_allreduce_bucket(ds2_comm_t comm, float* bucket, int64_t count,
                                  ds2_stream_t stream);
ds2_status_t ds2_comm_destroy(ds2_comm_t comm);

size_t ds2_optim_workspace_size(int64_t numel);
ds2_status_t ds2_grad_norm(const float* grads, int64_t numel, float* out_norm, void* ws,
                           size_t ws_bytes, ds2_stream_t stream);
ds2_status_t ds2_clip_sgd_nesterov(float* params, const float* grads, float* momentum_buf,
                                   int64_t numel, float lr, float momentum, float max_norm,
                                   const float* norm, const int* skip_flag,
                                   ds2_stream_t stream);
ds2_status_t ds2_clip_sgd_nesterov_wd(float* params, const float* grads, float* momentum_buf,
                                      int64_t numel, float lr, float momentum,
                                      float weight_decay, float max_norm, const float* norm,
                                      const int* skip_flag, ds2_stream_t stream);
ds2_status_t ds2_clip_adam(float* params, const float* grads, float* exp_avg, float* exp_avg_sq,
                           int64_t numel, double lr, double beta1, double beta2, double eps,
                           double weight_decay, float max_norm, const float* norm, int* step,
                           const int* skip_flag, ds2_stream_t stream);
ds2_status_t ds2_nan_guard(float* x, int64_t numel, int zero_nans, int* flag,
                           unsigned char* mask, ds2_stream_t stream);
ds2_status_t ds2_zero_masked(float* x, const unsigned char* mask, int64_t numel, const int* flag,
                             ds2_stream_t stream);
ds2_status_t ds2_scale_by_device_scalar(float* x, int64_t numel, const float* scalar,
                                        ds2_stream_t stream);

#ifdef __cplusplus
}
#endif

#endif
```

Before: 9160.

## Fuse row-amax partials into GRU xl backward and defer fallback memsets

```diff
diff --git a/deepspeech.pytorch_amd/csrc/gru.hip b/deepspeech.pytorch_amd/csrc/gru.hip
--- a/deepspeech.pytorch_amd/csrc/gru.hip
+++ b/deepspeech.pytorch_amd/csrc/gru.hip
@@ -1,6 +1,7 @@
 #include "rnn_common.h"
 
 #include <algorithm>
+#include <mutex>
 
 namespace ds2 {
 
@@ -984,13 +985,18 @@
 bool launch_gru_fwd_xl(int t_max, int n, int h, int num_dirs, const float* xproj,
                        const float* w_hh_f, const float* w_hh_r, const float* b_hh_f,
                        const float* b_hh_r, const int* lens, float* h_all, float* gates,
-                       float* ring, unsigned* xl, unsigned* err, unsigned long long* stamps,
-                       size_t lds_pad, hipStream_t st);
+                       float* ring, unsigned* ctrs, size_t ctr_bytes, unsigned* xl, unsigned* err,
+                       unsigned* err_out, unsigned long long* stamps, size_t lds_pad,
+                       hipStream_t st);
 bool launch_gru_bwd_xl(int t_max, int n, int h, int num_dirs, const float* dy, int dy_dirs,
                        const float* w_hh_f, const float* w_hh_r, const float* h_all,
                        const float* gates, const int* lens, float* dgates_x, float* dgates_h,
-                       float* ring, unsigned* xl, unsigned* err, unsigned long long* stamps,
-                       double* dbp, size_t lds_pad, hipStream_t st, unsigned* camax);
+                       float* ring, unsigned* ctrs, size_t ctr_bytes, unsigned* xl, unsigned* err,
+                       unsigned* err_out, unsigned long long* stamps, double* dbp, size_t lds_pad,
+                       hipStream_t st, unsigned* camax, float* rowp);
+size_t gru_xl_rowp_bytes(int t_max, int n, int h, int num_dirs);
+void launch_gru_xl_row_amax(int t_max, int n, int h, int num_dirs, const float* rowp,
+                            unsigned* out, hipStream_t st);
 }
 
 using namespace ds2;
@@ -1089,21 +1095,20 @@
       static_cast<char*>(ws) + align256((size_t)num_dirs * UB * KS * 3 * 64 * sizeof(float)));
   unsigned* err = ctrs + num_dirs * BT;
   if (persistent && (h % GU) == 0 && UB <= 8 * GW) {
-    if (hipMemsetAsync(ctrs, 0, counter_bytes(n, num_dirs), st) != hipSuccess)
-      return launch_status("ds2_gru counters");
     int T_ = t_max, N_ = n, H_ = h, D_ = num_dirs, UB_ = UB, BT_ = BT;
     unsigned long long* stamps = stamp_mode() == 2 ? stamp_slots(ctrs, n, num_dirs) : nullptr;
     float* ring = reinterpret_cast<float*>(reinterpret_cast<char*>(ctrs) +
                                            align256(counter_bytes(n, num_dirs)));
     void* args[] = {&T_, &N_, &H_, &D_, &UB_, &BT_, &xproj, &w_hh_f, &w_hh_r, &b_hh_f,
                     &b_hh_r, &lens, &h_all, &gates, &ring, &ctrs, &err, &stamps};
+    if (launch_gru_fwd_xl(t_max, n, h, num_dirs, xproj, w_hh_f, w_hh_r, b_hh_f, b_hh_r, lens,
+                          h_all, gates, ring, ctrs, counter_bytes(n, num_dirs), err + 1, err,
+                          err_out, stamps, kDopPadLds, st))
+      return launch_status("ds2_gru_fwd");
+    (void)hipGetLastError();
+    if (hipMemsetAsync(ctrs, 0, counter_bytes(n, num_dirs), st) != hipSuccess)
+      return launch_status("ds2_gru counters");
     if (ring_reset(ring, n, h, num_dirs, st) != hipSuccess) return launch_status("ds2_gru ring");
-    if (launch_gru_fwd_xl(t_max, n, h, num_dirs, xproj, w_hh_f, w_hh_r, b_hh_f, b_hh_r, lens,
-                          h_all, gates, ring, err + 1, err, stamps, kDopPadLds, st)) {
-      fold_err(err, err_out, st);
-      return launch_status("ds2_gru_fwd");
-    }
-    (void)hipGetLastError();
     if (launch_gru_fwd_x6(t_max, n, h, num_dirs, xproj, w_hh_f, w_hh_r, b_hh_f, b_hh_r, lens,
                           h_all, gates, ring, ctrs, err, stamps, kDopPadLds, st)) {
       fold_err(err, err_out, st);
@@ -1177,6 +1182,45 @@
   return gru_bwd_ws_base(n, h, num_dirs) + gru_db_bytes(n, h, num_dirs);
 }
 
+size_t ds2_gru_row_amax_workspace_size(int t_max, int n, int h, int num_dirs) {
+  if (t_max < 0 || n < 0 || h < 1 || (num_dirs != 1 && num_dirs != 2)) return 0;
+  return ds2_gru_bwd_workspace_size(n, h, num_dirs) +
+         align256(gru_xl_rowp_bytes(t_max, n, h, num_dirs));
+}
+
+struct RowRec {
+  const void* ws;
+  int t, n, h, d;
+};
+static std::mutex g_row_mu;
+static RowRec g_row_rec = {nullptr, 0, 0, 0, 0};
+static void row_rec_clear(const void* ws) {
+  std::lock_guard<std::mutex> lk(g_row_mu);
+  if (g_row_rec.ws == ws) g_row_rec.ws = nullptr;
+}
+static void row_rec_set(const void* ws, int t, int n, int h, int d) {
+  std::lock_guard<std::mutex> lk(g_row_mu);
+  g_row_rec = RowRec{ws, t, n, h, d};
+}
+
+ds2_status_t ds2_gru_row_amax(int t_max, int n, int h, int num_dirs, const void* ws,
+                                  size_t ws_bytes, unsigned* row_amax, ds2_stream_t stream) {
+  if (t_max < 0 || n < 0 || h < 1 || (num_dirs != 1 && num_dirs != 2)) return DS2_INVALID_VALUE;
+  if (t_max == 0 || n == 0) return DS2_OK;
+  if (ws == nullptr || row_amax == nullptr) return DS2_INVALID_VALUE;
+  {
+    std::lock_guard<std::mutex> lk(g_row_mu);
+    const RowRec r = g_row_rec;
+    if (r.ws != ws || r.t != t_max || r.n != n || r.h != h || r.d != num_dirs ||
+        ws_bytes < ds2_gru_row_amax_workspace_size(t_max, n, h, num_dirs))
+      return DS2_UNSUPPORTED_SHAPE;
+  }
+  const float* rowp = reinterpret_cast<const float*>(static_cast<const char*>(ws) +
+                                                     ds2_gru_bwd_workspace_size(n, h, num_dirs));
+  launch_gru_xl_row_amax(t_max, n, h, num_dirs, rowp, row_amax, as_stream(stream));
+  return launch_status("ds2_gru_row_amax");
+}
+
 #define DS2_BWD_CASE(K)                                                                     \
   case K:                                                                                   \
     hipLaunchKernelGGL(gru_bwd_step_kernel<K>, dim3(grid), dim3(GT), 0, st, s, t_max, n, h,  \
@@ -1212,7 +1256,7 @@
                                 const float* gates, const int* lens, float* dgates_x,
                                 float* dgates_h, unsigned* err_out, void* ws, hipStream_t st,
                                 double* dbp, bool& summed, unsigned* camax, bool& camax_done,
-                                int& db_tiles);
+                                int& db_tiles, float* rowp, bool& rowp_done);
 
 static ds2_status_t gru_bwd_bias_impl(int t_max, int n, int h, int num_dirs, const float* dy,
                                       int dy_dirs, const float* w_hh_f, const float* w_hh_r,
@@ -1264,9 +1308,10 @@
   hipStream_t st = as_stream(stream);
   double* dbp = reinterpret_cast<double*>(static_cast<char*>(ws) + gru_bwd_ws_base(n, h, num_dirs));
   const size_t camax_bytes = (size_t)2 * num_dirs * 3 * h * sizeof(unsigned);
-  if (camax != nullptr && hipMemsetAsync(camax, 0, camax_bytes, st) != hipSuccess)
-    return launch_status("ds2_gru_bwd_bias_amax");
+  row_rec_clear(ws);
   if (t_max == 0 || n == 0) {
+    if (camax != nullptr && hipMemsetAsync(camax, 0, camax_bytes, st) != hipSuccess)
+      return launch_status("ds2_gru_bwd_bias_amax");
     if (!want_db) return DS2_OK;
     if (hipMemsetAsync(dbp, 0, gru_db_bytes(n > 0 ? n : 1, h, num_dirs), st) != hipSuccess)
       return launch_status("ds2_gru_bwd_bias");
@@ -1274,12 +1319,18 @@
                        dbp, 1, num_dirs, h, db_ih_f, db_hh_f, db_ih_r, db_hh_r);
     return launch_status("ds2_gru_bwd_bias");
   }
-  bool summed = false, camax_done = false;
+  bool summed = false, camax_done = false, rowp_done = false;
   int db_tiles = (n + GB - 1) / GB;
+  float* rowp = nullptr;
+  if (camax != nullptr && ws_bytes >= ds2_gru_row_amax_workspace_size(t_max, n, h, num_dirs))
+    rowp = reinterpret_cast<float*>(static_cast<char*>(ws) +
+                                    ds2_gru_bwd_workspace_size(n, h, num_dirs));
   const ds2_status_t rc = gru_bwd_run(t_max, n, h, num_dirs, dy, dy_dirs, w_hh_f, w_hh_r, h_all,
                                       gates, lens, dgates_x, dgates_h, err_out, ws, st,
-                                      want_db ? dbp : nullptr, summed, camax, camax_done, db_tiles);
+                                      want_db ? dbp : nullptr, summed, camax, camax_done, db_tiles,
+                                      rowp, rowp_done);
   if (rc != DS2_OK) return rc;
+  if (rowp_done) row_rec_set(ws, t_max, n, h, num_dirs);
   if (camax != nullptr && !camax_done) {
     const ds2_status_t ra = ds2_amax(dgates_x, t_max * n, num_dirs * 3 * h, num_dirs * 3 * h,
                                      nullptr, camax, stream);
@@ -1305,7 +1356,7 @@
                                 const float* gates, const int* lens, float* dgates_x,
                                 float* dgates_h, unsigned* err_out, void* ws, hipStream_t st,
                                 double* dbp, bool& summed, unsigned* camax, bool& camax_done,
-                                int& db_tiles) {
+                                int& db_tiles, float* rowp, bool& rowp_done) {
   if (num_dirs == 1) w_hh_r = w_hh_f;
   apply_spin_limit_env();
   apply_rnn_tune_env();
@@ -1324,7 +1375,26 @@
   unsigned* ctrs = reinterpret_cast<unsigned*>(
       reinterpret_cast<char*>(dhs) + align256((size_t)2 * n * num_dirs * h * sizeof(float)));
   unsigned* err = ctrs + num_dirs * BT;
-  if (persistent && (h % GU) == 0 && UB <= 8 * GW) {
+  const size_t camax_bytes = (size_t)2 * num_dirs * 3 * h * sizeof(unsigned);
+  const bool dop = persistent && (h % GU) == 0 && UB <= 8 * GW;
+  if (dop) {
+    unsigned long long* stamps = stamp_mode() == 2 ? stamp_slots(ctrs, n, num_dirs) : nullptr;
+    float* ring = reinterpret_cast<float*>(reinterpret_cast<char*>(ctrs) +
+                                           align256(counter_bytes(n, num_dirs)));
+    if (launch_gru_bwd_xl(t_max, n, h, num_dirs, dy, dy_dirs, w_hh_f, w_hh_r, h_all, gates,
+                          lens, dgates_x, dgates_h, ring, ctrs, counter_bytes(n, num_dirs),
+                          err + 1, err, err_out, stamps, dbp, kDopPadLds, st, camax, rowp)) {
+      summed = dbp != nullptr;
+      camax_done = camax != nullptr;
+      rowp_done = rowp != nullptr;
+      db_tiles = (n + 7) / 8;
+      return launch_status("ds2_gru_bwd");
+    }
+    (void)hipGetLastError();
+  }
+  if (camax != nullptr && hipMemsetAsync(camax, 0, camax_bytes, st) != hipSuccess)
+    return launch_status("ds2_gru_bwd_bias_amax");
+  if (dop) {
     if (hipMemsetAsync(ctrs, 0, counter_bytes(n, num_dirs), st) != hipSuccess)
       return launch_status("ds2_gru counters");
     int T_ = t_max, N_ = n, H_ = h, D_ = num_dirs, UB_ = UB, BT_ = BT, DYD_ = dy_dirs;
@@ -1333,16 +1403,6 @@
                                            align256(counter_bytes(n, num_dirs)));
     void* args[] = {&T_, &N_, &H_, &D_, &UB_, &BT_, &dy, &DYD_, &w_hh_f, &w_hh_r, &h_all,
                     &gates, &lens, &dgates_x, &dgates_h, &ring, &ctrs, &err, &stamps, &dbp};
-    if (launch_gru_bwd_xl(t_max, n, h, num_dirs, dy, dy_dirs, w_hh_f, w_hh_r, h_all, gates,
-                          lens, dgates_x, dgates_h, ring, err + 1, err, stamps, dbp, kDopPadLds,
-                          st, camax)) {
-      fold_err(err, err_out, st);
-      summed = dbp != nullptr;
-      camax_done = camax != nullptr;
-      db_tiles = (n + 7) / 8;
-      return launch_status("ds2_gru_bwd");
-    }
-    (void)hipGetLastError();
     if (launch_gru_bwd_x6(t_max, n, h, num_dirs, dy, dy_dirs, w_hh_f, w_hh_r, h_all, gates,
                           lens, dgates_x, dgates_h, ring, ctrs, err, stamps, dbp, kDopPadLds, st,
                           camax, &camax_done)) {
diff --git a/deepspeech.pytorch_amd/csrc/gru_xl.hip b/deepspeech.pytorch_amd/csrc/gru_xl.hip
--- a/deepspeech.pytorch_amd/csrc/gru_xl.hip
+++ b/deepspeech.pytorch_amd/csrc/gru_xl.hip
@@ -1,4 +1,6 @@
 #include "rnn_common.h"
+
+#include <algorithm>
 
 namespace ds2 {
 
@@ -25,7 +27,8 @@
 }
 
 __device__ __forceinline__ bool xl_group_local(unsigned* xtab, int ub, int UBX, unsigned* err,
-                                               int* lds_word, unsigned* mode, int force_global) {
+                                               unsigned* err_out, int* lds_word, unsigned* mode,
+                                               int force_global) {
   const unsigned mine = xcc_id() + 1u;
   if (threadIdx.x == 0) __hip_atomic_store(xtab + ub, mine, __ATOMIC_RELAXED, __HIP_MEMORY_SCOPE_AGENT);
   if ((threadIdx.x >> 6) == 0) {
@@ -37,7 +40,7 @@
                      : mine;
       if (__ballot(v == 0u) == 0ull) break;
       if (spins > g_spin_limit) {
-        if (lane == 0) __hip_atomic_fetch_or(err, 1u, __ATOMIC_RELAXED, __HIP_MEMORY_SCOPE_AGENT);
+        if (lane == 0) raise_err(err, err_out);
         ok = false;
         break;
       }
@@ -58,6 +61,41 @@
     __builtin_amdgcn_raw_buffer_store_b128(v, rs, off, 0, 0);
   else
     __builtin_amdgcn_raw_buffer_store_b128(v, rs, off, 0, kSc1);
+}
+
+#define DS2_DPP_MAX(v, ctrl)                                                               \
+  v = fmaxf(v, __builtin_bit_cast(float, __builtin_amdgcn_update_dpp(                      \
+                   0, __builtin_bit_cast(int, v), ctrl, 0xf, 0xf, true)))
+__device__ __forceinline__ float half_wave_max(float v) {
+  DS2_DPP_MAX(v, 0xB1);
+  DS2_DPP_MAX(v, 0x4E);
+  DS2_DPP_MAX(v, 0x141);
+  DS2_DPP_MAX(v, 0x140);
+  const int b = __builtin_bit_cast(int, v);
+  const float r0 = __builtin_bit_cast(float, __builtin_amdgcn_readlane(b, 0));
+  const float r1 = __builtin_bit_cast(float, __builtin_amdgcn_readlane(b, 16));
+  const float r2 = __builtin_bit_cast(float, __builtin_amdgcn_readlane(b, 32));
+  const float r3 = __builtin_bit_cast(float, __builtin_amdgcn_readlane(b, 48));
+  return (threadIdx.x & 32) ? fmaxf(r2, r3) : fmaxf(r0, r1);
+}
+#undef DS2_DPP_MAX
+
+__device__ __forceinline__ bool xl_wave_flags_wait(const unsigned* flags, int count,
+                                                   unsigned target, unsigned* err,
+                                                   unsigned* err_out) {
+  const int lane = threadIdx.x & 63;
+  if (count == 0) return true;
+  for (unsigned spins = 0;; ++spins) {
+    if (spins > g_spin_limit || g_spin_limit == 0) {
+      if (lane == 0) raise_err(err, err_out);
+      return false;
+    }
+    const unsigned v = lane < count ? __hip_atomic_load(flags + lane, __ATOMIC_RELAXED,
+                                                        __HIP_MEMORY_SCOPE_AGENT)
+                                    : target;
+    if (__ballot(v < target) == 0ull) return true;
+    sleep_units(g_rnn_tune[3]);
+  }
 }
 
 __device__ __forceinline__ int xl_frag_hi(int m, int k) { return (((k >> 3) << 4) + m) * 8 + (k & 7); }
@@ -68,7 +106,8 @@
     const float* __restrict__ w_f, const float* __restrict__ w_r, const float* __restrict__ b_f,
     const float* __restrict__ b_r, const int* __restrict__ lens, float* __restrict__ h_all,
     float* __restrict__ gates, float* __restrict__ ring, unsigned* __restrict__ xl,
-    unsigned* __restrict__ err, unsigned long long* __restrict__ stamps, int force_global) {
+    unsigned* __restrict__ err, unsigned* __restrict__ err_out,
+    unsigned long long* __restrict__ stamps, int force_global) {
   constexpr int NCT = 6;
   constexpr int RC = 3 * LU + 1;
   __shared__ float red[LW * 16 * RC];
@@ -89,7 +128,8 @@
   const int p0 = wave * (UBX / LW) + min(wave, UBX % LW);
   const int np = UBX / LW + (wave < UBX % LW ? 1 : 0);
   if (threadIdx.x == 0) failed = 0;
-  const bool local = xl_group_local(xl + g * 32, ub, UBX, err, &sh_local, xl + 512 + g, force_global);
+  const bool local =
+      xl_group_local(xl + g * 32, ub, UBX, err, err_out, &sh_local, xl + 512 + g, force_global);
   const int slot_floats = G * UBX * 256;
   const __amdgpu_buffer_rsrc_t x_rs =
       __builtin_amdgcn_make_buffer_rsrc(ring, (short)0, LSLOTS * slot_floats * 4, 0x00020000);
@@ -263,7 +303,7 @@
                !kAblWait && (!wave_ready(__builtin_bit_cast(f32x4, hv[p])) || g_spin_limit == 0);
                ++spins) {
             if (spins > g_spin_limit || g_spin_limit == 0) {
-              if (lane == 0) __hip_atomic_fetch_or(err, 1u, __ATOMIC_RELAXED, __HIP_MEMORY_SCOPE_AGENT);
+              if (lane == 0) raise_err(err, err_out);
               failed = 1;
               bad = true;
               break;
@@ -347,15 +387,16 @@
   if (io && !kAblStores) store_out(T - 1);
 }
 
-template <int NPW>
+template <int NPW, bool ROWS>
 __global__ __launch_bounds__(LT) __attribute__((amdgpu_waves_per_eu(1, 1))) void gru_bwd_xl_kernel(
     int T, int N, int H, int D, int UBX, int BTX, const float* __restrict__ dy, int dyd,
     const float* __restrict__ w_f, const float* __restrict__ w_r,
     const float* __restrict__ h_all, const float* __restrict__ gates,
     const int* __restrict__ lens, float* __restrict__ dgx, float* __restrict__ dgh,
     float* __restrict__ ring, unsigned* __restrict__ xl, unsigned* __restrict__ err,
-    unsigned long long* __restrict__ stamps, double* __restrict__ dbp,
-    unsigned* __restrict__ camax, int force_global) {
+    unsigned* __restrict__ err_out, unsigned long long* __restrict__ stamps,
+    double* __restrict__ dbp, unsigned* __restrict__ camax, float* __restrict__ rowp,
+    int force_global) {
   constexpr int RC = LU + 1;
   constexpr int LWP = 3;
   __shared__ __attribute__((aligned(8))) float red[LW * 16 * RC > 4 * LB * LU * 2 ? LW * 16 * RC : 4 * LB * LU * 2];
@@ -367,6 +408,7 @@
   __shared__ int slen[LB];
   __shared__ int sh_local;
   __shared__ int flag;
+  __shared__ float rowmx[2 * LB];
   __shared__ u32x4 wx[LW * 6 * 2 * 64];
   const int G = D * BTX;
   int g, ub;
@@ -377,11 +419,13 @@
   const int p0 = wave * (UBX / LW) + min(wave, UBX % LW);
   const int np = UBX / LW + (wave < UBX % LW ? 1 : 0);
   const int H3 = 3 * H;
+  if (threadIdx.x == 0) flag = 1;
   const int slot_floats = G * UBX * LRB;
   const __amdgpu_buffer_rsrc_t x_rs =
       __builtin_amdgcn_make_buffer_rsrc(ring, (short)0, 2 * slot_floats * 4, 0x00020000);
   const int grp_off = g * UBX * LRB;
-  const bool local = xl_group_local(xl + g * 32, ub, UBX, err, &sh_local, xl + 512 + g, force_global);
+  const bool local =
+      xl_group_local(xl + g * 32, ub, UBX, err, err_out, &sh_local, xl + 512 + g, force_global);
   unsigned* flags = xl + 256 + g * 32;
   const __amdgpu_buffer_rsrc_t f_rs =
       __builtin_amdgcn_make_buffer_rsrc(xl + 256, (short)0, 8 * 32 * 4, 0x00020000);
@@ -531,6 +575,15 @@
     store_one(tt, sl0);
     store_one(tt, sl1);
   };
+  const int rpo = ROWS && wave == 1 && lane < LB && bt * LB + lane < N
+                      ? ((bt * LB + lane) * D + d) * UBX + ub
+                      : -1;
+  const int rpstr = N * D * UBX;
+  auto store_rmx = [&](int st) __attribute__((always_inline)) {
+    if (!ROWS || wave != 1) return;
+    const int tt = d == 0 ? T - 1 - st : st;
+    if (rpo >= 0) rowp[rpo + tt * rpstr] = rowmx[(st & 1) * LB + lane];
+  };
   f32x4 xin0 = io ? load_in(0, sl0) : z4v, xin1 = io ? load_in(0, sl1) : z4v;
   float dh_prev = 0.f, z_prev = 0.f;
   double sb_r = 0.0, sb_z = 0.0, sb_n = 0.0, sb_hn = 0.0;
@@ -543,6 +596,7 @@
       xin1 = load_in(st + 1, sl1);
     }
     if (!kAblStores && st > 0) store_out(st - 1);
+    if (!kAblStores && st > 1) store_rmx(st - 2);
   };
   for (int s = 0; s < T; ++s) {
     const int t = d == 0 ? T - 1 - s : s;
@@ -554,10 +608,9 @@
     }
     if (s == 0) io_issue(0);
     if (s > 0) {
-      if (!kAblWait && !flags_wait(flags, UBX, (unsigned)s, err, &flag)) {
-        poison_rest(dgx, s, T, d == 0, N, D, n, d, H, j, H3, 3, owner);
-        return;
-      }
+      if (!kAblWait && !xl_wave_flags_wait(flags + p0, np, (unsigned)s, err, err_out) && lane == 0)
+        flag = 0;
+      asm volatile("" ::: "memory");
       trace_at(s, 1);
       const int rb = (((s - 1) & 1) * slot_floats + grp_off + p0 * LRB) * 4;
       u32x4 r0[NPW + 1], r1[NPW + 1], r2[NPW + 1];
@@ -606,6 +659,10 @@
       for (int i = 0; i < 4; ++i)
         red[(wave * 16 + (lane >> 4) * 4 + i) * RC + 16 * c + (lane & 15)] = acc[c][i];
     __syncthreads();
+    if (flag == 0) {
+      poison_rest(dgx, s, T, d == 0, N, D, n, d, H, j, H3, 3, owner);
+      return;
+    }
     const float dyv = pin[m * LU + u], g_r = pin[256 + m * LU + u], g_z = pin[512 + m * LU + u];
     const float g_n = pin[768 + m * LU + u], g_hn = pin[1024 + m * LU + u];
     const float hp = pin[1280 + m * LU + u];
@@ -642,9 +699,7 @@
     pout[512 + m * LU + u] = dan;
     pout[768 + m * LU + u] = dghn;
     {
-      float mx = fmaxf(fmaxf(fabsf(dar), fabsf(daz)), fabsf(dghn));
-#pragma unroll
-      for (int o = 1; o < 32; o <<= 1) mx = fmaxf(mx, __shfl_xor(mx, o));
+      const float mx = half_wave_max(fmaxf(fmaxf(fabsf(dar), fabsf(daz)), fabsf(dghn)));
       const int e = h3_row_exp(mx);
       const float sc = __builtin_ldexpf(1.f, e);
       const float vr = dar * sc, vz = daz * sc, vn = dghn * sc;
@@ -675,9 +730,17 @@
       }
     }
     trace_at(s, 5);
+    if (ROWS) {
+      const float rm = half_wave_max(fmaxf(fmaxf(fabsf(dar), fabsf(daz)), fabsf(dan)));
+      if (u == 0) rowmx[(s & 1) * LB + m] = rm;
+    }
   }
   __syncthreads();
   if (io && !kAblStores) store_out(T - 1);
+  if (!kAblStores) {
+    if (T > 1) store_rmx(T - 2);
+    store_rmx(T - 1);
+  }
   if (camax != nullptr) {
     __syncthreads();
     red[(0 * LB + m) * LU + u] = cm_r;
@@ -721,6 +784,28 @@
   }
 }
 
+__global__ __launch_bounds__(256) void gru_xl_prep_kernel(unsigned* __restrict__ za, size_t na,
+                                                          unsigned* __restrict__ zb, size_t nb,
+                                                          u32x4* __restrict__ ff, size_t ff16) {
+  const size_t i0 = blockIdx.x * (size_t)blockDim.x + threadIdx.x;
+  const size_t step = (size_t)gridDim.x * blockDim.x;
+  for (size_t i = i0; i < na; i += step) za[i] = 0u;
+  for (size_t i = i0; i < nb; i += step) zb[i] = 0u;
+  for (size_t i = i0; i < ff16; i += step) ff[i] = u32x4{kSentinel, kSentinel, kSentinel, kSentinel};
+}
+
+__global__ __launch_bounds__(256) void gru_xl_row_amax_kernel(const float* __restrict__ rowp,
+                                                              int rows, int parts,
+                                                              unsigned* __restrict__ out) {
+  const int r = (blockIdx.x * 256 + (int)threadIdx.x) >> 3, k = threadIdx.x & 7;
+  float m = 0.f;
+  if (r < rows)
+    for (int i = k; i < parts; i += 8) m = fmaxf(m, rowp[(int64_t)r * parts + i]);
+#pragma unroll
+  for (int o = 1; o < 8; o <<= 1) m = fmaxf(m, __shfl_xor(m, o));
+  if (r < rows && k == 0) out[r] = __float_as_uint(m);
+}
+
 
 static inline bool env_off(const char* name) {
   const char* e = getenv(name);
@@ -755,10 +840,12 @@
   return nullptr;
 }
 
-static const void* bwd_xl_fn(int UBX) {
+static const void* bwd_xl_fn(int UBX, bool rows) {
   const int need = (UBX + LW - 1) / LW;
-#define DS2_BXL(K) \
-  if (need <= K + 1) return reinterpret_cast<const void*>(gru_bwd_xl_kernel<K>);
+#define DS2_BXL(K)                                                                    \
+  if (need <= K + 1)                                                                  \
+    return rows ? reinterpret_cast<const void*>(gru_bwd_xl_kernel<K, true>)           \
+                : reinterpret_cast<const void*>(gru_bwd_xl_kernel<K, false>);
   DS2_BXL(1) DS2_BXL(3) DS2_BXL(6)
 #undef DS2_BXL
   return nullptr;
@@ -769,40 +856,68 @@
   return bwd ? 2 * G * UBX * LRB * sizeof(float) : LSLOTS * G * UBX * 256 * sizeof(float);
 }
 
+static bool xl_prepare(unsigned* ctrs, size_t ctr_bytes, unsigned* zb, size_t nb, float* ring,
+                       size_t ff_bytes, hipStream_t st) {
+  const size_t na = ctr_bytes / sizeof(unsigned), ff16 = ff_bytes / 16;
+  const size_t most = std::max(std::max(na, nb), ff16);
+  const unsigned grid = (unsigned)std::min<size_t>(1024, std::max<size_t>(1, (most + 255) / 256));
+  hipLaunchKernelGGL(gru_xl_prep_kernel, dim3(grid), dim3(256), 0, st, ctrs, na, zb, nb,
+                     reinterpret_cast<u32x4*>(ring), ff16);
+  return hipGetLastError() == hipSuccess;
+}
+
 bool launch_gru_fwd_xl(int t_max, int n, int h, int num_dirs, const float* xproj,
                        const float* w_hh_f, const float* w_hh_r, const float* b_hh_f,
                        const float* b_hh_r, const int* lens, float* h_all, float* gates,
-                       float* ring, unsigned* xl, unsigned* err, unsigned long long* stamps,
-                       size_t lds_pad, hipStream_t st) {
+                       float* ring, unsigned* ctrs, size_t ctr_bytes, unsigned* xl, unsigned* err,
+                       unsigned* err_out, unsigned long long* stamps, size_t lds_pad,
+                       hipStream_t st) {
   if (gru_xl_groups(n, h, num_dirs) == 0 || env_off("DS2_GRU_H3")) return false;
   apply_spin_limit_env();
   apply_rnn_tune_env();
   const int UBX = h / LU, BTX = (n + LB - 1) / LB;
   const void* fn = fwd_xl_fn(UBX);
   if (fn == nullptr) return false;
+  if (!xl_prepare(ctrs, ctr_bytes, nullptr, 0, ring, gru_xl_ring_bytes(n, h, num_dirs, false), st))
+    return false;
   int T_ = t_max, N_ = n, H_ = h, D_ = num_dirs, UB_ = UBX, BT_ = BTX, FG_ = xl_force_global();
   void* args[] = {&T_, &N_, &H_, &D_, &UB_, &BT_, &xproj, &w_hh_f, &w_hh_r, &b_hh_f,
-                  &b_hh_r, &lens, &h_all, &gates, &ring, &xl, &err, &stamps, &FG_};
+                  &b_hh_r, &lens, &h_all, &gates, &ring, &xl, &err, &err_out, &stamps, &FG_};
   return rnn_launch(fn, dim3(8 * UBX), dim3(LT), args, lds_pad, st) == hipSuccess;
 }
 
 bool launch_gru_bwd_xl(int t_max, int n, int h, int num_dirs, const float* dy, int dy_dirs,
                        const float* w_hh_f, const float* w_hh_r, const float* h_all,
                        const float* gates, const int* lens, float* dgates_x, float* dgates_h,
-                       float* ring, unsigned* xl, unsigned* err, unsigned long long* stamps,
-                       double* dbp, size_t lds_pad, hipStream_t st, unsigned* camax) {
+                       float* ring, unsigned* ctrs, size_t ctr_bytes, unsigned* xl, unsigned* err,
+                       unsigned* err_out, unsigned long long* stamps, double* dbp, size_t lds_pad,
+                       hipStream_t st, unsigned* camax, float* rowp) {
   if (gru_xl_groups(n, h, num_dirs) == 0 || env_off("DS2_GRU_H3_BWD")) return false;
   apply_spin_limit_env();
   apply_rnn_tune_env();
   const int UBX = h / LU, BTX = (n + LB - 1) / LB;
-  const void* fn = bwd_xl_fn(UBX);
+  const void* fn = bwd_xl_fn(UBX, rowp != nullptr);
   if (fn == nullptr) return false;
+  if (!xl_prepare(ctrs, ctr_bytes, camax, camax != nullptr ? (size_t)2 * num_dirs * 3 * h : 0,
+                  nullptr, 0, st))
+    return false;
   int T_ = t_max, N_ = n, H_ = h, D_ = num_dirs, UB_ = UBX, BT_ = BTX, DYD_ = dy_dirs;
   int FG_ = xl_force_global();
   void* args[] = {&T_, &N_, &H_, &D_, &UB_, &BT_, &dy, &DYD_, &w_hh_f, &w_hh_r, &h_all,
-                  &gates, &lens, &dgates_x, &dgates_h, &ring, &xl, &err, &stamps, &dbp, &camax,
-                  &FG_};
+                  &gates, &lens, &dgates_x, &dgates_h, &ring, &xl, &err, &err_out, &stamps, &dbp,
+                  &camax, &rowp, &FG_};
   return rnn_launch(fn, dim3(8 * UBX), dim3(LT), args, lds_pad, st) == hipSuccess;
 }
 
-}
+size_t gru_xl_rowp_bytes(int t_max, int n, int h, int num_dirs) {
+  return (size_t)t_max * n * num_dirs * (h / LU) * sizeof(float);
+}
+
+void launch_gru_xl_row_amax(int t_max, int n, int h, int num_dirs, const float* rowp,
+                            unsigned* out, hipStream_t st) {
+  const int rows = t_max * n;
+  hipLaunchKernelGGL(gru_xl_row_amax_kernel, dim3((rows * 8 + 255) / 256), dim3(256), 0, st, rowp,
+                     rows, num_dirs * (h / LU), out);
+}
+
+}
diff --git a/deepspeech.pytorch_amd/csrc/rnn_common.h b/deepspeech.pytorch_amd/csrc/rnn_common.h
--- a/deepspeech.pytorch_amd/csrc/rnn_common.h
+++ b/deepspeech.pytorch_amd/csrc/rnn_common.h
@@ -160,6 +160,12 @@
 
 static inline void fold_err(const unsigned* err, unsigned* err_out, hipStream_t st) {
   if (err_out != nullptr) hipLaunchKernelGGL(err_fold_kernel, dim3(1), dim3(64), 0, st, err, err_out);
+}
+
+__device__ __forceinline__ void raise_err(unsigned* err, unsigned* err_out) {
+  __hip_atomic_fetch_or(err, 1u, __ATOMIC_RELAXED, __HIP_MEMORY_SCOPE_AGENT);
+  if (err_out != nullptr)
+    __hip_atomic_fetch_or(err_out, 1u, __ATOMIC_RELAXED, __HIP_MEMORY_SCOPE_AGENT);
 }
 
 __device__ __forceinline__ void st_sc1(float* p, float v) {
diff --git a/deepspeech.pytorch_amd/ds2amd/_lib.py b/deepspeech.pytorch_amd/ds2amd/_lib.py
--- a/deepspeech.pytorch_amd/ds2amd/_lib.py
+++ b/deepspeech.pytorch_amd/ds2amd/_lib.py
@@ -94,6 +94,8 @@
     "ds2_gru_bwd_bias_amax": (_c_int, [_c_int, _c_int, _c_int, _c_int, _vp, _c_int, _vp, _vp,
                                        _vp, _vp, _vp, _vp, _vp, _vp, _vp, _vp, _vp, _vp, _vp, _vp,
                                        _sz, _vp]),
+    "ds2_gru_row_amax_workspace_size": (_sz, [_c_int, _c_int, _c_int, _c_int]),
+    "ds2_gru_row_amax": (_c_int, [_c_int, _c_int, _c_int, _c_int, _vp, _sz, _vp, _vp]),
     "ds2_lstm_fwd_workspace_size": (_sz, [_c_int, _c_int, _c_int]),
     "ds2_lstm_fwd": (_c_int, [_c_int, _c_int, _c_int, _c_int, _vp, _vp, _vp, _vp, _vp, _vp, _vp,
                               _vp, _vp, _vp, _vp, _sz, _vp]),
@@ -190,5 +192,16 @@
     check(getattr(lib, name)(*args), name)
 
 
+UNSUPPORTED_SHAPE = 2
+
+
+def call_or_unsupported(name: str, *args) -> bool:
+    status = getattr(load(), name)(*args)
+    if status == UNSUPPORTED_SHAPE:
+        return False
+    check(status, name)
+    return True
+
+
 def size(name: str, *args) -> int:
     return int(getattr(load(), name)(*args))
diff --git a/deepspeech.pytorch_amd/ds2amd/ops.py b/deepspeech.pytorch_amd/ds2amd/ops.py
--- a/deepspeech.pytorch_amd/ds2amd/ops.py
+++ b/deepspeech.pytorch_amd/ds2amd/ops.py
@@ -777,7 +777,7 @@
 
 
 def _rnn_param_grads(x, h_all, dgx, dgh, weights, nd, g, need_dx, bf16=False, pre=None,
-                     dbias=None, shared_bf16=True, col_amax=None):
+                     dbias=None, shared_bf16=True, col_amax=None, row_amax=None):
     t, n, inp = x.shape
     h = h_all.shape[-1]
     dev = x.device
@@ -798,7 +798,8 @@
             am["dgx_c"] = col_amax[:ld]
             am["dgh_c"] = col_amax[ld:] if col_amax.numel() == 2 * ld else am["dgx_c"]
             if need_dx:
-                am["dgx_r"] = amax(dgx, tn, ld, ld, want_cols=False)[0]
+                am["dgx_r"] = (row_amax if row_amax is not None
+                               else amax(dgx, tn, ld, ld, want_cols=False)[0])
         else:
             am["dgx_r"], am["dgx_c"] = amax(dgx, tn, ld, ld, want_rows=need_dx)
             am["dgh_c"] = am["dgx_c"] if dgh is dgx else amax(dgh, tn, ld, ld, want_rows=False)[1]
@@ -921,24 +922,33 @@
         dgh = torch.empty(t, n, nd, h3, device=dev, dtype=_F32)
         w_hh_f = weights[1]
         w_hh_r = weights[5] if nd == 2 else None
-        ws = _ws(_lib.size("ds2_gru_bwd_workspace_size", n, h, nd), dev)
+        h3_scales = h3_enabled() and not bf16
+        want_rows = h3_scales and ctx.needs_input_grad[0]
+        ws = _ws(_lib.size("ds2_gru_row_amax_workspace_size", t, n, h, nd) if want_rows
+                 else _lib.size("ds2_gru_bwd_workspace_size", n, h, nd), dev)
         _guard_cooperative("gru", n, h, nd)
         dbias = [grad_like(weights[4 * d + k]) for d in range(nd) for k in (2, 3)]
         common = (t, n, h, nd, dy.data_ptr(), dy_dirs, w_hh_f.data_ptr(), _p(w_hh_r),
                   h_all.data_ptr(), gates.data_ptr(), lens.data_ptr(), dgx.data_ptr(),
                   dgh.data_ptr(), dbias[0].data_ptr(), dbias[1].data_ptr(),
                   _p(dbias[2] if nd == 2 else None), _p(dbias[3] if nd == 2 else None))
-        col_amax = None
-        if h3_enabled() and not bf16:
+        col_amax = row_amax = None
+        if h3_scales:
             col_amax = torch.empty(2 * nd * h3, dtype=_I32, device=dev)
             _lib.call("ds2_gru_bwd_bias_amax", *common, col_amax.data_ptr(),
                       rnn_status_word(dev).data_ptr(), ws.data_ptr(), ws.numel(), _stream())
+            if want_rows and t * n > 0:
+                row_amax = torch.empty(t * n, dtype=_I32, device=dev)
+                if not _lib.call_or_unsupported("ds2_gru_row_amax", t, n, h, nd,
+                                                ws.data_ptr(), ws.numel(), row_amax.data_ptr(),
+                                                _stream()):
+                    row_amax = None
         else:
             _lib.call("ds2_gru_bwd_bias", *common, rnn_status_word(dev).data_ptr(),
                       ws.data_ptr(), ws.numel(), _stream())
         dx, grads = _rnn_param_grads(x, h_all, dgx, dgh, weights, nd, h3,
                                      ctx.needs_input_grad[0], bf16, ctx.pre, dbias=dbias,
-                                     col_amax=col_amax)
+                                     col_amax=col_amax, row_amax=row_amax)
         return (dx, None, None, None, *grads)
 
 
diff --git a/include/ds2hip.h b/include/ds2hip.h
--- a/include/ds2hip.h
+++ b/include/ds2hip.h
@@ -150,6 +150,9 @@
                                    float* db_hh_f, float* db_ih_r, float* db_hh_r,
                                    unsigned* col_amax, unsigned* err_out, void* ws,
                                    size_t ws_bytes, ds2_stream_t stream);
+size_t ds2_gru_row_amax_workspace_size(int t_max, int n, int h, int num_dirs);
+ds2_status_t ds2_gru_row_amax(int t_max, int n, int h, int num_dirs, const void* ws,
+                                  size_t ws_bytes, unsigned* row_amax, ds2_stream_t stream);
 
 size_t ds2_lstm_fwd_workspace_size(int n, int h, int num_dirs);
 ds2_status_t ds2_lstm_fwd(int t_max, int n, int h, int num_dirs, const float* xproj,
```

Measured after the change: 9455 (median of 6 runs). +3.2%, better.
